# darshangm/dynamics-aware-diffusion

Measured on AMD Instinct MI355X. Metric: trajectory plans/sec (H=32, T=100), higher is better.
Workload: dtype f32; 1 GPU; PointMaze umaze-v2 guided policy, H=32 dim=128 mults(1,2,4) T=100 batch=256/GPU; arch=pointmaze, batch_per_gpu=256, global_batch=256, horizon=32, denoise_steps=100, rng=in-kernel philox, conv_arithmetic=fp32 (exact fp32 MFMA), hipgraph=False, loops_in_flight=1

## Files before the change

### dynamics_aware_diffusion_amd/_engine.py

```python
from __future__ import annotations

import ctypes as C
import math
import os
from typing import Dict, Mapping, Optional, Sequence

import torch

_HERE = os.path.dirname(os.path.abspath(__file__))
LIB_PATH = os.environ.get("DAD_LIB") or os.path.join(_HERE, "libdad_hip.so")

DAD_MAX_LEVELS = 8


class DadCfg(C.Structure):
    _fields_ = [
        ("transition_dim", C.c_int32), ("dim", C.c_int32), ("time_dim", C.c_int32),
        ("n_levels", C.c_int32), ("channels", C.c_int32 * DAD_MAX_LEVELS),
        ("kernel_size", C.c_int32), ("horizon", C.c_int32), ("n_timesteps", C.c_int32),
        ("predict_epsilon", C.c_int32), ("clip_denoised", C.c_int32),
    ]


class DadStepArgs(C.Structure):
    _fields_ = [
        ("noise", C.c_void_p), ("seed", C.c_uint64), ("row_offset", C.c_uint64),
        ("draw", C.c_uint64), ("cond0", C.c_void_p), ("cond_per_row", C.c_int32),
        ("guide_grad", C.c_void_p), ("guide_weight", C.c_float),
        ("mean_out", C.c_void_p), ("eps_out", C.c_void_p),
    ]


class DadProjectArgs(C.Structure):
    _fields_ = [
        ("P", C.c_void_p), ("obs_mean", C.c_void_p), ("obs_std", C.c_void_p),
        ("act_mean", C.c_void_p), ("act_std", C.c_void_p),
        ("state_dim", C.c_int32), ("observation_dim", C.c_int32), ("action_dim", C.c_int32),
        ("scratch", C.c_void_p), ("scratch_bytes", C.c_size_t),
    ]


ABI = {
    "dad_last_error": (C.c_char_p, []),
    "dad_version": (C.c_char_p, []),
    "dad_model_create": (C.c_int, [C.POINTER(DadCfg), C.POINTER(C.c_void_p)]),
    "dad_model_destroy": (None, [C.c_void_p]),
    "dad_model_load_weight": (C.c_int, [C.c_void_p, C.c_char_p, C.c_void_p,
                                        C.POINTER(C.c_int64), C.c_int32]),
    "dad_model_load_schedule": (C.c_int, [C.c_void_p] + [C.c_void_p] * 5),
    "dad_model_load_time_embedding": (C.c_int, [C.c_void_p, C.c_void_p, C.c_int32, C.c_int32]),
    "dad_model_set_precision": (C.c_int, [C.c_void_p, C.c_int32]),
    "dad_model_set_group_channels": (C.c_int, [C.c_void_p, C.POINTER(C.c_int32), C.c_int32]),
    "dad_model_set_horizon": (C.c_int, [C.c_void_p, C.c_int32]),
    "dad_model_finalize": (C.c_int, [C.c_void_p, C.c_void_p]),
    "dad_workspace_bytes": (C.c_int, [C.c_void_p, C.c_int32, C.POINTER(C.c_size_t)]),
    "dad_unet_forward": (C.c_int, [C.c_void_p, C.c_void_p, C.c_int32, C.c_void_p, C.c_int32,
                                   C.c_void_p, C.c_size_t, C.c_void_p]),
    "dad_unet_forward_rows": (C.c_int, [C.c_void_p, C.c_void_p, C.c_void_p, C.c_void_p, C.c_int32,
                                        C.c_void_p, C.c_size_t, C.c_void_p]),
    "dad_projection_violation": (C.c_int, [C.POINTER(DadProjectArgs), C.c_void_p, C.c_void_p, C.c_int32,
                                           C.c_int32, C.c_void_p]),
    "dad_denoise_step": (C.c_int, [C.c_void_p, C.c_void_p, C.c_int32, C.c_int32,
                                   C.POINTER(DadStepArgs), C.c_int32, C.c_void_p, C.c_size_t,
                                   C.c_void_p]),
    "dad_sample_loop": (C.c_int, [C.c_void_p, C.c_void_p, C.c_int32, C.c_int32, C.c_void_p,
                                  C.c_uint64, C.c_uint64, C.c_void_p, C.c_int32,
                                  C.POINTER(DadProjectArgs), C.c_void_p, C.c_int32, C.c_void_p,
                                  C.c_size_t, C.c_void_p]),
    "dad_project": (C.c_int, [C.POINTER(DadProjectArgs), C.c_float, C.c_void_p, C.c_int32,
                              C.c_int32, C.c_void_p]),
    "dad_fill_normal": (C.c_int, [C.c_void_p, C.c_int32, C.c_int32, C.c_uint64, C.c_uint64,
                                  C.c_uint64, C.c_void_p]),
    "dad_debug_set_tile": (C.c_int, [C.c_void_p, C.c_int32]),
    "dad_debug_set_option": (C.c_int, [C.c_void_p, C.c_char_p, C.c_int32]),
    "dad_debug_read_table": (C.c_int, [C.c_void_p, C.c_int32, C.c_int32, C.c_void_p, C.c_int32,
                                       C.POINTER(C.c_int32)]),
    "dad_debug_mish": (C.c_int, [C.c_void_p, C.c_void_p, C.c_int64, C.c_void_p]),
    "dad_debug_kernel_table_consistent": (C.c_int, []),
    "dad_debug_small_batch_plan": (C.c_int, [C.c_void_p, C.c_int32, C.POINTER(C.c_int32),
                                             C.POINTER(C.c_int32)]),
    "dad_debug_backward_plan": (C.c_int, [C.c_void_p, C.c_int32, C.POINTER(C.c_int32), C.c_int32,
                                          C.POINTER(C.c_int32)]),
    "dad_model_set_training": (C.c_int, [C.c_void_p, C.c_int32]),
    "dad_model_refresh_weights": (C.c_int, [C.c_void_p, C.c_int32, C.POINTER(C.c_char_p), C.POINTER(C.c_void_p),
                                            C.c_void_p]),
    "dad_train_grad_count": (C.c_int, [C.c_void_p, C.POINTER(C.c_int32), C.POINTER(C.c_int64)]),
    "dad_train_grad_info": (C.c_int, [C.c_void_p, C.c_int32, C.POINTER(C.c_char_p), C.POINTER(C.c_int64),
                                      C.POINTER(C.c_int64)]),
    "dad_train_workspace_bytes": (C.c_int, [C.c_void_p, C.c_int32, C.POINTER(C.c_size_t),
                                            C.POINTER(C.c_size_t)]),
    "dad_unet_forward_train": (C.c_int, [C.c_void_p, C.c_void_p, C.c_void_p, C.c_void_p, C.c_void_p,
                                         C.c_int32, C.c_void_p, C.c_size_t, C.c_void_p]),
    "dad_unet_backward": (C.c_int, [C.c_void_p, C.c_void_p, C.c_void_p, C.c_void_p, C.c_void_p,
                                    C.POINTER(C.c_void_p), C.c_int32,
                                    C.c_int32, C.c_void_p, C.c_size_t, C.c_void_p, C.c_size_t, C.c_void_p]),
    "dad_profile_enable": (C.c_int, [C.c_void_p, C.c_int32]),
    "dad_profile_read": (C.c_int, [C.c_void_p, C.POINTER(C.c_double), C.POINTER(C.c_int64),
                                   C.POINTER(C.c_double)]),
}

_lib = None


def load_library() -> C.CDLL:
    global _lib
    if _lib is not None:
        return _lib
    if not os.path.exists(LIB_PATH):
        raise RuntimeError(
            f"{LIB_PATH} not found: build it with dynamics_aware_diffusion_amd/csrc/build.sh "
            "(or __graft_entry__.build()).  There is no CPU fallback.")
    lib = C.CDLL(LIB_PATH)
    for name, (restype, argtypes) in ABI.items():
        if os.environ.get("DAD_LIB") and not hasattr(lib, name):
            continue
        fn = getattr(lib, name)
        fn.restype = restype
        fn.argtypes = argtypes
    _lib = lib
    return lib


class DadError(RuntimeError):
    def __init__(self, code: int, message: str):
        super().__init__(f"libdad_hip error {code}: {message}")
        self.code = code


def _check(lib, rc: int) -> None:
    if rc != 0:
        raise DadError(rc, lib.dad_last_error().decode("utf-8", "replace"))


def _ptr(t: Optional[torch.Tensor]) -> Optional[int]:
    return None if t is None else t.data_ptr()


def _require_device(t: torch.Tensor, name: str) -> None:
    if not t.is_cuda:
        raise RuntimeError(f"{name} must live on a ROCm device (got {t.device}); the HIP engine "
                           "has no CPU path")
    if t.dtype != torch.float32 or not t.is_contiguous():
        raise RuntimeError(f"{name} must be contiguous float32 (got {t.dtype}, "
                           f"contiguous={t.is_contiguous()})")


PRECISIONS = {"fp32": 0, "f16x3": 1}
TABLES = {"sinusoid": 0, "time_mlp": 1, "blocks": 2}


def sinusoid_table(n_timesteps: int, dim: int) -> torch.Tensor:
    half = dim // 2
    scale = math.log(10000) / (half - 1)
    freqs = torch.exp(torch.arange(half) * -scale)
    arg = torch.arange(n_timesteps)[:, None] * freqs[None, :]
    return torch.cat((arg.sin(), arg.cos()), dim=-1).contiguous()

SCHEDULE_KEYS = ("sqrt_recip_alphas_cumprod", "sqrt_recipm1_alphas_cumprod",
                 "posterior_mean_coef1", "posterior_mean_coef2",
                 "posterior_log_variance_clipped")


class HipEngine:

    def __init__(self, *, transition_dim: int, dim: int, channels: Sequence[int], horizon: int,
                 n_timesteps: int, time_dim: Optional[int] = None, kernel_size: int = 5,
                 predict_epsilon: bool = True, clip_denoised: bool = True,
                 device: torch.device | str = "cuda", precision: str = "fp32", training: bool = False):
        if precision not in PRECISIONS:
            raise ValueError(f"precision must be one of {sorted(PRECISIONS)}, got {precision!r}")
        self.precision = precision
        self.lib = load_library()
        self.device = torch.device(device)
        if self.device.type != "cuda":
            raise RuntimeError("HipEngine needs a ROCm device; there is no CPU path")
        from .utils import padding
        self.real_dim, self.real_channels = int(dim), [int(c) for c in channels]
        padded = [padding.padded_width(c) for c in self.real_channels]
        self.padded = padded != self.real_channels
        if self.padded:
            if self.real_channels[0] != self.real_dim:
                raise NotImplementedError("zero-padded widths need dim_mults[0] == 1")
            if transition_dim == self.real_dim:
                raise NotImplementedError(
                    f"transition_dim == dim == {dim} makes the first block's residual the trajectory itself; "
                    "with zero-padded GroupNorm groups that identity has no kernel")
        horizon = int(horizon)
        levels = len(self.real_channels)
        self.padded_horizon = max(1 << max(horizon - 1, 0).bit_length(), 4 << (levels - 1))
        self.rows_padded = self.padded_horizon != horizon
        if self.rows_padded:
            if horizon % (1 << (levels - 1)) != 0:
                raise ValueError(f"horizon {horizon} cannot be halved {levels - 1} times (the reference's U-Net needs "
                                 f"H % 2^(levels-1) == 0, temporal_unet.py:35-54)")
            if transition_dim == self.real_dim:
                raise NotImplementedError("transition_dim == dim with a zero-padded horizon has no kernel")
        self.padded = self.padded or self.rows_padded
        cfg = DadCfg()
        cfg.transition_dim = transition_dim
        cfg.dim = padded[0] if padded != self.real_channels else dim
        cfg.time_dim = time_dim or dim
        cfg.n_levels = len(channels)
        for i, ch in enumerate(padded):
            cfg.channels[i] = int(ch)
        cfg.kernel_size = kernel_size
        cfg.horizon = self.padded_horizon
        cfg.n_timesteps = n_timesteps
        cfg.predict_epsilon = int(predict_epsilon)
        cfg.clip_denoised = int(clip_denoised)
        self.cfg = cfg
        self.horizon = horizon
        self.transition_dim = transition_dim
        self.n_timesteps = n_timesteps
        handle = C.c_void_p()
        _check(self.lib, self.lib.dad_model_create(C.byref(cfg), C.byref(handle)))
        self._h = handle
        _check(self.lib, self.lib.dad_model_set_precision(self._h, PRECISIONS[precision]))
        self.widths_padded = padded != self.real_channels
        if self.widths_padded:
            real = (C.c_int32 * len(self.real_channels))(*self.real_channels)
            _check(self.lib, self.lib.dad_model_set_group_channels(self._h, real, len(self.real_channels)))
        if self.rows_padded:
            _check(self.lib, self.lib.dad_model_set_horizon(self._h, horizon))
        self.training = bool(training)
        if self.training:
            _check(self.lib, self.lib.dad_model_set_training(self._h, 1))
        self._ws: Dict[int, torch.Tensor] = {}
        self._pinned: Dict[tuple, torch.Tensor] = {}
        self.ready = False

    def __del__(self):
        h = getattr(self, "_h", None)
        if h:
# ... 138 lines not shown
            projection._check_x(x)
            pa = C.byref(projection.args)
            alphas = (C.c_float * self.n_timesteps)(*[float(a) for a in proj_alphas])
        ws = self.workspace(B)
        with torch.cuda.device(self.device):
            _check(self.lib, self.lib.dad_sample_loop(
                self._h, x.data_ptr(), int(n_steps), B, _ptr(noise_stack), int(seed),
                int(row_offset), cond_ptr, per_row, pa, alphas, int(use_graph), ws.data_ptr(),
                ws.numel() * 4, self._stream()))

    def fill_normal(self, x: torch.Tensor, seed: int, row_offset: int = 0, draw: int = 0) -> None:
        _require_device(x, "x")
        B = int(x.shape[0])
        with torch.cuda.device(self.device):
            _check(self.lib, self.lib.dad_fill_normal(
                x.data_ptr(), B, x.numel() // B, int(seed), int(row_offset), int(draw),
                self._stream()))

    def refresh(self, unet_state: Mapping[str, torch.Tensor]) -> None:
        keys, ptrs, keep = [], [], []
        if self.widths_padded:
            with torch.no_grad():
                names = list(unet_state.keys())
                fp = self.flat_padding(names, [tuple(unet_state[k].shape) for k in names])
                wide = fp.pad_flat([unet_state[k].detach().to(self.device) for k in names])
            base, n = wide.data_ptr(), len(names)
            with torch.cuda.device(self.device):
                _check(self.lib, self.lib.dad_model_refresh_weights(
                    self._h, n, (C.c_char_p * n)(*[k.encode() for k in names]),
                    (C.c_void_p * n)(*[base + 4 * o for o in fp.offsets]), self._stream()))
            self._refresh_keep = [wide]
            return
        for key, t in unet_state.items():
            d = t.detach()
            if d.device != self.device or d.dtype != torch.float32 or not d.is_contiguous():
                d = d.to(self.device, torch.float32).contiguous()
            keep.append(d)
            keys.append(key.encode())
            ptrs.append(d.data_ptr())
        n = len(keys)
        with torch.cuda.device(self.device):
            _check(self.lib, self.lib.dad_model_refresh_weights(
                self._h, n, (C.c_char_p * n)(*keys), (C.c_void_p * n)(*ptrs), self._stream()))
        self._refresh_keep = keep

    def flat_padding(self, keys, shapes, offsets=None, total=None):
        from .utils import padding
        cache = self.__dict__.setdefault("_flat_paddings", {})
        sig = (tuple(keys), None if offsets is None else tuple(offsets))
        if sig not in cache:
            cache[sig] = padding.FlatPadding(keys, shapes, self._pad_plan, offsets, total)
        return cache[sig]

    def time_projection_index(self) -> torch.Tensor:
        from .utils import padding
        cached = getattr(self, "_temb_index", None)
        if cached is None:
            n = len(self.real_channels)
            widths = [c for c in self.real_channels for _ in (0, 1)] + [self.real_channels[-1]] * 2
            for j in range(n - 1):
                widths += [self.real_channels[n - 2 - j]] * 2
            index, off = [], 0
            for c in widths:
                index.append(padding.channel_index(c) + off)
                off += padding.padded_width(c)
            cached = self._temb_index = (torch.cat(index).to(self.device), off)
        return cached

    def grad_layout(self):
        cached = getattr(self, "_grad_layout", None)
        if cached is not None:
            return cached
        n, total = C.c_int32(), C.c_int64()
        _check(self.lib, self.lib.dad_train_grad_count(self._h, C.byref(n), C.byref(total)))
        out = []
        for i in range(n.value):
            key, off, numel = C.c_char_p(), C.c_int64(), C.c_int64()
            _check(self.lib, self.lib.dad_train_grad_info(self._h, i, C.byref(key), C.byref(off), C.byref(numel)))
            out.append((key.value.decode(), off.value, numel.value))
        self._grad_layout = (out, total.value)
        return self._grad_layout

    def train_forward(self, x: torch.Tensor, temb_rows: torch.Tensor):
        B = self._traj(x)
        _require_device(temb_rows, "temb_rows")
        if temb_rows.dim() != 2 or temb_rows.shape[0] != B:
            raise RuntimeError(f"temb_rows must be (B, temb_width), got {tuple(temb_rows.shape)}")
        sv, sc = C.c_size_t(), C.c_size_t()
        _check(self.lib, self.lib.dad_train_workspace_bytes(self._h, B, C.byref(sv), C.byref(sc)))
        saved = torch.empty(max(sv.value, 4) // 4 + 4, dtype=torch.float32, device=self.device)
        rows = torch.arange(B, dtype=torch.int32, device=self.device)
        out = torch.empty_like(x)
        with torch.cuda.device(self.device):
            _check(self.lib, self.lib.dad_unet_forward_train(
                self._h, x.data_ptr(), rows.data_ptr(), temb_rows.data_ptr(), out.data_ptr(), B,
                saved.data_ptr(), saved.numel() * 4, self._stream()))
        return out, saved

    def train_backward(self, x: torch.Tensor, d_out: torch.Tensor, saved: torch.Tensor, temb_width: int, shapes):
        B = self._traj(x)
        if self._traj(d_out, "d_out") != B:
            raise RuntimeError("d_out batch mismatch")
        sv, sc = C.c_size_t(), C.c_size_t()
        _check(self.lib, self.lib.dad_train_workspace_bytes(self._h, B, C.byref(sv), C.byref(sc)))
        scratch = torch.empty(max(sc.value, 4) // 4 + 4, dtype=torch.float32, device=self.device)
        layout, total = self.grad_layout()
        if len(shapes) != len(layout):
            raise RuntimeError(f"{len(shapes)} parameter shapes for {len(layout)} gradient tensors")
        real = None
        if self.widths_padded:
            real = self.flat_padding([k for k, _, _ in layout], shapes, [o for _, o, _ in layout], total)
            shapes = real.padded_shapes
            for (key, _, numel), n in zip(layout, real.sizes):
                if n != numel:
                    raise RuntimeError(f"{key}: {n} padded elements, the library expects {numel}")
        flat = torch.empty(total, dtype=torch.float32, device=self.device)
        base = flat.data_ptr()
        spans = [layout[i + 1][1] - layout[i][1] for i in range(len(layout) - 1)] + [total - layout[-1][1]]
        pieces = flat.split_with_sizes(spans)
        grads = [(pc if pc.numel() == numel else pc[:numel]).view(tuple(shape))
                 for pc, (_, _, numel), shape in zip(pieces, layout, shapes)]
        ptrs = (C.c_void_p * len(grads))(*[base + 4 * offset for _, offset, _ in layout])
        d_x = torch.empty_like(x)
        d_temb = torch.empty(B, temb_width, dtype=torch.float32, device=self.device)
        with torch.cuda.device(self.device):
            _check(self.lib, self.lib.dad_unet_backward(
                self._h, x.data_ptr(), d_out.data_ptr(), d_x.data_ptr(), d_temb.data_ptr(), ptrs, len(grads), B,
                saved.data_ptr(), saved.numel() * 4, scratch.data_ptr(), scratch.numel() * 4, self._stream()))
        if real is not None:
            grads = real.gather(flat)
        return d_x, d_temb, grads

    def debug_set_tile(self, cfg: int) -> None:
        with torch.cuda.device(self.device):
            _check(self.lib, self.lib.dad_debug_set_tile(self._h, int(cfg)))

    def debug_set_option(self, name: str, value: int) -> None:
        with torch.cuda.device(self.device):
            _check(self.lib, self.lib.dad_debug_set_option(self._h, name.encode(), int(value)))

    def read_table(self, which: str, t: int) -> torch.Tensor:
        out = torch.empty(1 << 16, dtype=torch.float32)
        width = C.c_int32()
        with torch.cuda.device(self.device):
            _check(self.lib, self.lib.dad_debug_read_table(self._h, TABLES[which], int(t),
                                                           out.data_ptr(), out.numel(), C.byref(width)))
        return out[:width.value].clone()

    def small_batch_plan(self, batch: int):
        n, w = C.c_int32(), C.c_int32()
        _check(self.lib, self.lib.dad_debug_small_batch_plan(self._h, int(batch), C.byref(n), C.byref(w)))
        return n.value, w.value

    def backward_plan(self, batch: int) -> dict:
        need = C.c_int32()
        _check(self.lib, self.lib.dad_debug_backward_plan(self._h, int(batch), None, 0, C.byref(need)))
        buf = (C.c_int32 * need.value)()
        _check(self.lib, self.lib.dad_debug_backward_plan(self._h, int(batch), buf, need.value, C.byref(need)))
        r = list(buf)
        fields = ("taps", "tile", "windowed", "samples", "spc", "sps", "ksplit", "chunks", "last_chunks")
        assert r[71] == len(fields) and (len(r) - 72) == r[0] * r[71]
        hist = lambda at: {(cfg, bool(s)): r[at + 2 * cfg + s] for cfg in range(10) for s in (0, 1) if r[at + 2 * cfg + s]}
        return {
            "wgrads": r[0], "multi": r[1], "max_chunks": r[2], "max_ksplit": r[3], "part": r[4], "part_multi": r[5],
            "windowed": r[6], "tile": r[7:11],
            "taps_tile": {(taps, tile): r[11 + 4 * i + tile] for i, taps in enumerate((1, 3, 4, 5, 7)) for tile in range(4)
                          if r[11 + 4 * i + tile]},
            "fwd": hist(31), "dgrad": hist(51),
            "launches": [dict(zip(fields, r[at:at + len(fields)])) for at in range(72, len(r), len(fields))],
        }

    def mish(self, x: torch.Tensor) -> torch.Tensor:
        _require_device(x, "x")
        out = torch.empty_like(x)
        with torch.cuda.device(self.device):
            _check(self.lib, self.lib.dad_debug_mish(x.data_ptr(), out.data_ptr(), x.numel(),
                                                     self._stream()))
        return out

    def profile_enable(self, on: bool) -> None:
        _check(self.lib, self.lib.dad_profile_enable(self._h, int(on)))

    def profile_read(self):
        ms, n, fl = C.c_double(), C.c_int64(), C.c_double()
        _check(self.lib, self.lib.dad_profile_read(self._h, C.byref(ms), C.byref(n), C.byref(fl)))
        return ms.value, n.value, fl.value


class ProjectionState:

    def __init__(self, P: torch.Tensor, obs_mean, obs_std, act_mean, act_std, state_dim: int,
                 observation_dim: int, action_dim: int, device):
        dev = torch.device(device)
        if dev.type != "cuda":
            raise RuntimeError("projection kernel needs a ROCm device; there is no CPU path")

        def put(v):
            return torch.as_tensor(v, dtype=torch.float32).contiguous().to(dev)

        self.P = put(P)
        self.obs_mean, self.obs_std = put(obs_mean), put(obs_std)
        self.act_mean, self.act_std = put(act_mean), put(act_std)
        a = DadProjectArgs()
        a.P = self.P.data_ptr()
        a.obs_mean, a.obs_std = self.obs_mean.data_ptr(), self.obs_std.data_ptr()
        a.act_mean, a.act_std = self.act_mean.data_ptr(), self.act_std.data_ptr()
        a.state_dim, a.observation_dim, a.action_dim = state_dim, observation_dim, action_dim
        self.args = a
        self.device = dev
        self._scratch = None
        self.gemm = True
        self.D = int(self.P.shape[0])
        if self.P.dim() != 2 or self.P.shape[1] != self.D:
            raise ValueError(f"projection matrix must be square, got {tuple(self.P.shape)}")
        if self.obs_mean.numel() != observation_dim or self.obs_std.numel() != observation_dim \
                or self.act_mean.numel() != action_dim or self.act_std.numel() != action_dim:
            raise ValueError("normaliser statistics do not match observation_dim / action_dim")

    def _check_x(self, x: torch.Tensor) -> None:
        _require_device(x, "x")
        a = self.args
        if x.dim() != 3 or x.shape[2] != a.observation_dim + a.action_dim:
            raise RuntimeError(f"x must be (B, H, {a.observation_dim + a.action_dim}), got {tuple(x.shape)}")
        D = (int(x.shape[1]) + 1) * a.state_dim + int(x.shape[1]) * a.action_dim
        if D != self.D:
            raise RuntimeError(f"mat1 and mat2 shapes cannot be multiplied ({x.shape[0]}x{D} and "
                               f"{self.D}x{self.D}): the projector was built for another horizon")
        if x.device != self.P.device:
            raise RuntimeError(f"x is on {x.device}, the projector on {self.P.device}")
        if self.gemm and (self._scratch is None or self._scratch.numel() < x.numel()):
            self._scratch = torch.empty(x.numel(), dtype=torch.float32, device=self.device)
            self.args.scratch = self._scratch.data_ptr()
            self.args.scratch_bytes = self._scratch.numel() * 4

    def violation(self, x: torch.Tensor) -> torch.Tensor:
        self._check_x(x)
        out = torch.empty(int(x.shape[0]), dtype=torch.float32, device=x.device)
        lib = load_library()
        with torch.cuda.device(self.device):
            _check(lib, lib.dad_projection_violation(C.byref(self.args), x.data_ptr(), out.data_ptr(),
                                                     int(x.shape[0]), int(x.shape[1]),
                                                     torch.cuda.current_stream(self.device).cuda_stream))
        return out

    def apply(self, x: torch.Tensor, alpha: float) -> None:
        self._check_x(x)
        lib = load_library()
        with torch.cuda.device(self.device):
            _check(lib, lib.dad_project(C.byref(self.args), float(alpha), x.data_ptr(),
                                        int(x.shape[0]), int(x.shape[1]),
                                        torch.cuda.current_stream(self.device).cuda_stream))
```

### dynamics_aware_diffusion_amd/csrc/conv_gemm.hpp

```cpp
#pragma once
#include <hip/hip_runtime.h>
#include <stdint.h>

#include "conv_shapes.hpp"

namespace dad {

#define DAD_LBID (blockIdx.x + gridDim.x * (blockIdx.y + gridDim.y * blockIdx.z))
#ifdef DAD_STAMPS
#define DAD_STAMP(i) do { if (p.stamps != nullptr && threadIdx.x == 0 && DAD_LBID < 4096) p.stamps[DAD_LBID * 8 + (i)] = __builtin_amdgcn_s_memrealtime(); } while (0)
#else
#define DAD_STAMP(i) do {} while (0)
#endif
#ifdef DAD_STAMPS
#define DAD_CLOCK(i) do { if (p.stamps != nullptr && threadIdx.x == 0 && DAD_LBID < 4096) p.stamps[DAD_LBID * 8 + (i)] = __builtin_amdgcn_s_memtime(); } while (0)
#else
#define DAD_CLOCK(i) do {} while (0)
#endif
#ifdef DAD_STAMPS_PROLOGUE
#define DAD_PSTAMP(i) do { if (p.stamps != nullptr && threadIdx.x == 0 && DAD_LBID < 4096) p.stamps[DAD_LBID * 8 + (i)] = __builtin_amdgcn_s_memrealtime(); } while (0)
#undef DAD_STAMP
#define DAD_STAMP(i) do { if ((i) == 0) DAD_PSTAMP(0); } while (0)
#undef DAD_CLOCK
#define DAD_CLOCK(i) do {} while (0)
#else
#define DAD_PSTAMP(i) do {} while (0)
#endif

typedef float f32x16 __attribute__((ext_vector_type(16)));
typedef _Float16 f16x8 __attribute__((ext_vector_type(8)));

__device__ __forceinline__ void split_f16(float v, _Float16& hi, _Float16& lo) {
    const float c = __builtin_fminf(__builtin_fmaxf(v, -65504.0f), 65504.0f);
    hi = (_Float16)c;
    lo = (_Float16)((c - (float)hi) * 2048.0f);
}
__device__ __forceinline__ void split_f16x4(const float4 v, float2& hi, float2& lo) {
    typedef _Float16 f16x4 __attribute__((ext_vector_type(4)));
    f16x4 h, l;
    _Float16 a, b;
    split_f16(v.x, a, b); h[0] = a; l[0] = b;
    split_f16(v.y, a, b); h[1] = a; l[1] = b;
    split_f16(v.z, a, b); h[2] = a; l[2] = b;
    split_f16(v.w, a, b); h[3] = a; l[3] = b;
    hi = __builtin_bit_cast(float2, h);
    lo = __builtin_bit_cast(float2, l);
}

struct ConvParams {
    const float* src0;
    const float* src1;
    const float* w;
    const float* bias;
    const float* gamma;
    const float* beta;
    const float* temb;
    const int32_t* trow;
    int32_t temb_stride;
    const float* res;
    float* dst;
    int32_t cin0, cin1;
    int32_t cin_pad;
    int32_t M;
    int32_t cpg;
    int32_t lreal;
    int32_t src_len;
    int32_t cpg_real;
    int32_t B;
    int32_t Lin, Lout;
    int32_t lshift;
    int32_t lshift_in;
    int32_t interleave;
    int32_t ntiles_n;
    int32_t xcd_gn;
    int32_t xcd_mts;
    int32_t xcd_ntn;
    int32_t kslices;
    int32_t chunks_per_slice;
    float c1, c2;
    uint64_t xswz;
    int32_t wtaps;
    const float* rbias;
    float* rdst;
    float* pre;
    float* stats;
    float* slab;
    unsigned* counters;
#ifdef DAD_STAMPS
    unsigned long long* stamps;
#endif
};

__device__ __forceinline__ float mish_f32(float y) {
    if (y > 20.0f) return y;
    const float n = expf(y);
    const float w = n * (n + 2.0f);
    return y * (w / (w + 2.0f));
}

__device__ __forceinline__ float mish_fast_f32(float y) {
    if (y > 20.0f) return y;
    const float L2E_HI = 1.44269502162933349609375f;
    const float L2E_LO = 1.92596299112661746e-08f;
    const float t = y * L2E_HI;
    const float tl = fmaf(y, L2E_HI, -t) + y * L2E_LO;
    const float n = __builtin_amdgcn_exp2f(t) * (1.0f + 0.693147180559945f * tl);
    const float w = n * (n + 2.0f);
    return y * (w * __builtin_amdgcn_rcpf(w + 2.0f));
}

template <int CTRL>
__device__ __forceinline__ float dpp_f32(float v) {
    return __builtin_bit_cast(float, __builtin_amdgcn_update_dpp(0, __builtin_bit_cast(int, v), CTRL,
                                                                 0xF, 0xF, true));
}
__device__ __forceinline__ float rows_sum(float v, int width, int lane) {
    const int iv = __builtin_bit_cast(int, v);
    const float r0 = __builtin_bit_cast(float, __builtin_amdgcn_readlane(iv, 0));
    const float r1 = __builtin_bit_cast(float, __builtin_amdgcn_readlane(iv, 16));
    const float r2 = __builtin_bit_cast(float, __builtin_amdgcn_readlane(iv, 32));
    const float r3 = __builtin_bit_cast(float, __builtin_amdgcn_readlane(iv, 48));
    const float lo = r0 + r1, hi = r2 + r3;
    if (width >= 64) return lo + hi;
    return lane < 32 ? lo : hi;
}

__device__ __forceinline__ float4 ldg4(const float* p) {
    typedef float __attribute__((ext_vector_type(4))) f4;
    const f4 v = *reinterpret_cast<const __attribute__((address_space(1))) f4*>(
        (const __attribute__((address_space(1))) float*)p);
    return make_float4(v.x, v.y, v.z, v.w);
}

__device__ __forceinline__ void store_f4_sc1(float* p, const float4 v) {
    typedef float __attribute__((ext_vector_type(4))) f4;
    const f4 x = {v.x, v.y, v.z, v.w};
    asm volatile("global_store_dwordx4 %0, %1, off sc1" ::"v"(p), "v"(x) : "memory");
}

template <int BM, int BN, int SK, int KC, int TAPS, int STRIDE, bool RAGGED, bool X3 = false, bool BDIR = false,
          bool RES = false, bool PADDED = false, bool WIN = false>
__global__ __launch_bounds__(64 * (BM / 32) * (BN / 32) * SK) void conv_gemm_f32(const ConvParams p) {
    constexpr int TMW = BM / 32;
    constexpr int TNW = BN / 32;
    constexpr int WT = TMW * TNW;
    constexpr int NT = 64 * WT * SK;
    constexpr int PAD = TAPS / 2;
    constexpr int WTAPS = TAPS + (RES ? 1 : 0);
    constexpr int KP = KC + 4;
    constexpr int KU = X3 ? 16 : 8;
    constexpr int G = KC / KU;
    constexpr int GW = G / SK;
    constexpr int KG = KC < 16 ? KC : 16;
    constexpr int NSUB = KC / KG;
    static_assert(KC % KU == 0 && G % SK == 0 && GW >= 1, "K chunk must split evenly over the SK waves");
    static_assert(!BDIR || (BN == 32 && SK == 1 && !RAGGED && KC >= 16), "direct-B tiles");
    static_assert(!RES || (!X3 && !BDIR && (TAPS & 1) == 1 && TAPS >= 3 && STRIDE == 1), "the residual ride exists for fp32 stride-1 convs of the net's kernel size");
    static_assert(!WIN || (PADDED && !X3 && !BDIR && !RES), "windowed tiles: fp32, LDS-staged, no ride");
    constexpr int BN_SH = BN == 32 ? 5 : BN == 64 ? 6 : 7;
    static_assert((1 << BN_SH) == BN, "BN is 32, 64 or 128");

    extern __shared__ __attribute__((aligned(16))) float smem[];
    float4* const smem4 = reinterpret_cast<float4*>(smem);
    float2* const smem2 = reinterpret_cast<float2*>(smem);
#ifdef DAD_ABLATE_NULL
    if (p.B > 0) return;
#endif

    DAD_STAMP(0);
    const int tid = threadIdx.x;
    const int lane = tid & 63;
    const int wave = __builtin_amdgcn_readfirstlane(tid >> 6);
    const int wt = wave % WT;
    const int ks = wave / WT;
    const int tn = wt / TMW;
    const int tm = wt % TMW;
    const int l32 = lane & 31;
    const int h = lane >> 5;

    const int kb = blockIdx.x;
    int mt = blockIdx.y;
    int nt = blockIdx.z;
    if (p.xcd_gn > 0) {
        const int wg = blockIdx.y, c = wg & 7, j = wg >> 3;
        const int im = c / p.xcd_gn, in = c - im * p.xcd_gn;
        mt = (im << p.xcd_mts) + (j & ((1 << p.xcd_mts) - 1));
        nt = in * p.xcd_ntn + (j >> p.xcd_mts);
    }
    const int tile = mt * p.ntiles_n + nt;

    const int Lin = p.Lin, Lout = p.Lout;
    const int SPT = WIN ? 1 : BN >> p.lshift;
    const int SEG = WIN ? BN * STRIDE + 2 * PAD : Lin + 2 * PAD;
    const int XROWS = SPT * SEG;
    const int wsh = WIN ? p.lshift - BN_SH : 0;
    const int s0 = WIN ? nt >> wsh : nt * SPT;
    const int w0 = WIN ? (nt & ((1 << wsh) - 1)) << BN_SH : 0;
    const int m0 = mt * BM;
    const int M = p.M;
    const int nvalid = min(SPT, p.B - s0);

    const int XF = XROWS * KP + kXSwzPad;
    const int STAGE = XF + (BDIR ? 0 : WTAPS * BM * KP);
    const int STAGE4 = STAGE >> 2;


    const int n_loc = tn * 32 + l32;
    const int phase_shift = (TAPS == 2 && p.interleave && m0 >= (p.M >> 1)) ? 1 : 0;
    const int arow = WIN ? (n_loc * STRIDE + phase_shift) * KP + 4 * h
                         : ((n_loc >> p.lshift) * SEG + (n_loc & (Lout - 1)) * STRIDE + phase_shift) * KP + 4 * h +
                               (int)((p.xswz >> (4 * (n_loc >> p.lshift))) & 15) * 4;
    const int brow = XF + (tm * 32 + l32) * KP + 4 * h;

    f32x16 acc, acc2, acc3, acc4;
    f32x16 accr, accr2;
#pragma unroll
    for (int r = 0; r < 16; ++r) { acc[r] = 0.0f; acc2[r] = 0.0f; acc3[r] = 0.0f; acc4[r] = 0.0f; accr[r] = 0.0f; accr2[r] = 0.0f; }

    const int cin = p.cin0 + p.cin1;
    const int c_begin = kb * p.chunks_per_slice;
#ifdef DAD_ABLATE_NOLOOP
    const int nchunks = c_begin + 1;
#else
    const int nchunks = min((p.cin0 + p.cin1 + KC - 1) / KC, c_begin + p.chunks_per_slice);
#endif

    constexpr int W_F4 = WTAPS * BM * KC / 4;
    constexpr int W_PER_T = BDIR ? 0 : (W_F4 + NT - 1) / NT;
    constexpr int W_ARR = W_PER_T ? W_PER_T : 1;
    constexpr int KQ = KC / 4;
    constexpr int X_F4_MAX = (BN * STRIDE + (WIN ? 2 * PAD : 0)) * KQ;
    constexpr int X_PER_T = (X_F4_MAX + NT - 1) / NT;
    const int xrows_real = WIN ? SEG : SPT * Lin;
    float4 wreg[W_ARR];
    float4 xreg[X_PER_T];
    int w_goff[W_ARR], w_loff[W_ARR];
    int x_grow[X_PER_T], x_q4[X_PER_T], x_loff[X_PER_T];
    constexpr int GQ = KG / 4;
#pragma unroll
    for (int i = 0; i < W_PER_T; ++i) {
        const int e = tid + i * NT;
        const int row = e / KQ;
        const int q = e - row * KQ;
        const int tap = row / BM;
        const int mm = row - tap * BM;
        const int sub = q / GQ;
        w_goff[i] = ((sub * p.wtaps + tap) * M + m0 + mm) * KG + (q - sub * GQ) * 4;
        w_loff[i] = (XF + row * KP + q * 4) >> 2;
    }
#pragma unroll
    for (int i = 0; i < X_PER_T; ++i) {
        const int e = tid + i * NT;
        const int row = e / KQ;
        const int q = e - row * KQ;
        const int s = WIN ? 0 : row >> p.lshift_in;
        int l = row - (s << p.lshift_in);
        if constexpr (WIN) l = w0 * STRIDE - PAD + row;
        const bool ok = e < xrows_real * KQ && s < nvalid && (!WIN || (l >= 0 && l < Lin));
        x_grow[i] = ok ? (WIN ? s0 * Lin + l : s0 * Lin + row) : -1;
        if constexpr (PADDED)
            if (p.src_len > 0)
                x_grow[i] = (ok && l < p.src_len) ? (s0 + s) * p.src_len + l : -1;
        x_q4[i] = q * 4;
        const int qoff = X3 ? (q >> 2) * 16 + (q & 3) * 2 : q * 4;
        const int xo = WIN ? row * KP + qoff : (s * SEG + PAD + l) * KP + qoff + (int)((p.xswz >> (4 * s)) & 15) * 4;
        x_loff[i] = e < xrows_real * KQ ? (X3 ? xo >> 1 : xo >> 2) : -1;
    }
    DAD_PSTAMP(6);
    const long w_chunk_stride = (long)NSUB * p.wtaps * M * KG;
    constexpr int NLD = W_PER_T + X_PER_T;
    auto item_store = [&](int k, int stage) {
        const int base4 = stage * STAGE4;
        if (k < W_PER_T) {
            if (W_F4 % NT == 0 || tid + k * NT < W_F4)
                smem4[base4 + w_loff[k]] = wreg[k];
        } else {
            const int i = k - W_PER_T;
            if (x_loff[i] >= 0) {
                float4 v = xreg[i];
                if (!RAGGED && x_grow[i] < 0) v = make_float4(0.f, 0.f, 0.f, 0.f);
                if constexpr (X3) {
                    float2 hi, lo;
                    split_f16x4(v, hi, lo);
                    smem2[base4 * 2 + x_loff[i]] = hi;
                    smem2[base4 * 2 + x_loff[i] + 4] = lo;
                } else {
                    smem4[base4 + x_loff[i]] = v;
                }
            }
        }
    };
    auto item_load = [&](int k, int chunk) {
        if (k < W_PER_T) {
            float4 v = make_float4(0.f, 0.f, 0.f, 0.f);
            if (W_F4 % NT == 0 || tid + k * NT < W_F4)
                v = *reinterpret_cast<const float4*>(p.w + chunk * w_chunk_stride + w_goff[k]);
            wreg[k] = v;
        } else {
            const int i = k - W_PER_T;
            const int c0 = chunk * KC;
            float4 v = make_float4(0.f, 0.f, 0.f, 0.f);
            if constexpr (!RAGGED) {
                const bool second = c0 >= p.cin0;
                const float* xsrc = second ? p.src1 : p.src0;
                const int cs = second ? p.cin1 : p.cin0;
                const int cb = second ? c0 - p.cin0 : c0;
                v = *reinterpret_cast<const float4*>(xsrc + (long)max(x_grow[i], 0) * cs + cb + x_q4[i]);
            } else {
                const int cc = c0 + x_q4[i];
                if (x_grow[i] >= 0 && cc < cin) {
                    const bool second = cc >= p.cin0;
                    const int cs = second ? p.cin1 : p.cin0;
                    const int cl = second ? cc - p.cin0 : cc;
                    const float* g = (second ? p.src1 : p.src0) + (long)x_grow[i] * cs + cl;
                    const int left = cs - cl;
                    if ((cs & 3) == 0) {
                        v = *reinterpret_cast<const float4*>(g);
                    } else {
                        if (left > 0) v.x = g[0];
                        if (left > 1) v.y = g[1];
                        if (left > 2) v.z = g[2];
                        if (left > 3) v.w = g[3];
                    }
                }
            }
            xreg[i] = v;
        }
    };

    constexpr int UW = WTAPS * GW;
    const int koff = ks * (GW * KU);
    const int afrag4 = (arow + koff) >> 2;
    const int bfrag4 = (brow + koff) >> 2;
    auto frag_a = [&](int stage, int u, int lo) -> float4 {
        const int wtap = u / GW, gw = u - wtap * GW;
        const int tap = (RES && wtap == TAPS) ? PAD : wtap;
        return smem4[stage * STAGE4 + afrag4 + tap * (KP / 4) + gw * (KU / 4) + lo / 4];
    };
    auto frag_b = [&](int stage, int u, int lo) -> float4 {
        const int tap = u / GW, gw = u - tap * GW;
        return smem4[stage * STAGE4 + bfrag4 + tap * (BM * KP / 4) + gw * (KU / 4) + lo / 4];
    };
    constexpr int BPU = X3 ? 2 : 1;
    float4 breg[BDIR ? BPU * UW : 1];
    const float* bsrc = p.w + ((long)(m0 + tm * 32 + l32) * 16 + 4 * h);
    auto bload = [&](int u, int chunk) {
        const int tap = u / GW, gw = u - tap * GW;
        if constexpr (X3) {
            const float* q = bsrc + (long)chunk * w_chunk_stride + (long)((gw * p.wtaps + tap) * M) * 16;
            breg[2 * u] = ldg4(q);
            breg[2 * u + 1] = ldg4(q + 8);
        } else {
            const float* q = bsrc + (long)chunk * w_chunk_stride +
                             (long)(((gw >> 1) * p.wtaps + tap) * M) * 16 + (gw & 1) * 8;
            breg[u] = ldg4(q);
        }
    };

#pragma unroll
    for (int k = 0; k < NLD; ++k) item_load(k, c_begin);
    if constexpr (BDIR) {
#pragma unroll
        for (int u = 0; u < UW; ++u) bload(u, c_begin);
    }

    constexpr int ES = BM + 4;
    constexpr int ECOPY = BN * ES;
    constexpr int F4PL = (BN * BM / 4) / NT;
    static_assert(F4PL >= 1 && (BN * BM / 4) % NT == 0, "epilogue mapping");
#ifdef DAD_ABLATE_GN
    const bool has_gn = false;
#else
    const bool has_gn = !WIN && p.gamma != nullptr;
#endif
    const int cpg = has_gn ? p.cpg : BM;
    const int cq = cpg >> 2;
    const int cnt4 = has_gn ? (Lout * cq) : (BN * cq);
    static_assert((F4PL & (F4PL - 1)) == 0, "F4PL is a power of two");
    const int lpp = cnt4 >> (F4PL == 1 ? 0 : F4PL == 2 ? 1 : F4PL == 4 ? 2 : 3);
    const int lpp_sh = 31 - __clz(lpp);
    const int cq_sh = 31 - __clz(cq);
    const int gpt_sh = 31 - __clz(BM) - (31 - __clz(cpg));
    const int pr = tid >> lpp_sh;
    const int lp = tid & (lpp - 1);
    const int ps = has_gn ? pr >> gpt_sh : 0;
    const int pg = has_gn ? pr & ((1 << gpt_sh) - 1) : 0;
    int erow[F4PL], ecol[F4PL];
    int eoff[F4PL];
    float4 bias4[F4PL], gam4[F4PL], bet4[F4PL], temb4[F4PL], res4[F4PL];
#pragma unroll
    for (int k = 0; k < F4PL; ++k) {
        const int j = lp + k * lpp;
        const int r = j >> cq_sh;
        erow[k] = ps * Lout + r;
        ecol[k] = pg * cpg + (j & (cq - 1)) * 4;
        const int s = erow[k] >> p.lshift;
        const int l = w0 + (erow[k] & (Lout - 1));
        const int em = m0 + ecol[k];
        if (!p.interleave) {
            eoff[k] = ((s0 + s) * Lout + l) * M + em;
        } else {
            const int half = M >> 1;
            const int phase = em >= half;
            eoff[k] = ((s0 + s) * (2 * Lout) + 2 * l + phase) * half + (em - phase * half);
        }
        if (s >= nvalid) eoff[k] = -1;
    }
    constexpr bool EARLY_PARAMS = F4PL <= 2;
#define DAD_FETCH_PARAMS()                                                                       \
    _Pragma("unroll") for (int k = 0; k < F4PL; ++k) {                                           \
        const int em = m0 + ecol[k];                                                             \
        long toff = 0;                                                                           \
        if (p.trow != nullptr)            \
            toff = (long)p.trow[min(s0 + (erow[k] >> p.lshift), p.B - 1)] * p.temb_stride;       \
        bias4[k] = ldg4(p.bias + em);                                                            \
        gam4[k] = ldg4(gptr + em);                                                               \
        bet4[k] = ldg4(bptr + em);                                                               \
        temb4[k] = ldg4(tptr + toff + em);                                                       \
        res4[k] = ldg4(has_res ? p.res + max(eoff[k], 0) : p.bias + em);                         \
    }
    const float* const gptr = has_gn ? p.gamma : p.bias;
    const float* const bptr = has_gn ? p.beta : p.bias;
    const float* const tptr = p.temb != nullptr ? p.temb : p.bias;
    const bool has_res = p.res != nullptr && !p.interleave;
    const bool has_temb = p.temb != nullptr;
    DAD_PSTAMP(7);
    if (EARLY_PARAMS) { DAD_FETCH_PARAMS() }
    DAD_PSTAMP(1);
    if constexpr (PAD > 0 && !WIN) {
        constexpr int KP4 = KP / 4;
        const int nz = SPT * (2 * PAD) * KP4;
        for (int i = tid; i < nz; i += NT) {
            const int hr = i / KP4, c4 = i - hr * KP4;
            const int s = hr / (2 * PAD), j = hr - s * (2 * PAD);
            const int row = s * SEG + (j < PAD ? j : Lin + j);
            const int at = row * KP + c4 * 4 + (int)((p.xswz >> (4 * s)) & 15) * 4;
            smem4[at >> 2] = make_float4(0.f, 0.f, 0.f, 0.f);
            smem4[STAGE4 + (at >> 2)] = make_float4(0.f, 0.f, 0.f, 0.f);
        }
    }
    DAD_PSTAMP(2);
#pragma unroll
    for (int k = 0; k < NLD; ++k) item_store(k, 0);
    DAD_PSTAMP(3);
    if (c_begin + 1 < nchunks) {
#pragma unroll
        for (int k = 0; k < NLD; ++k) item_load(k, c_begin + 1);
    }
    DAD_PSTAMP(4);
    __syncthreads();
    DAD_PSTAMP(5);

    float4 ah = frag_a(0, 0, 0), bh = ah;
    if constexpr (!BDIR) bh = frag_b(0, 0, 0);
    float4 al = ah, bl = bh;
    if constexpr (X3) {
        al = frag_a(0, 0, 8);
        if constexpr (!BDIR) bl = frag_b(0, 0, 8);
    }
    DAD_STAMP(1);
    DAD_CLOCK(6);
#ifndef DAD_ABLATE_STAGE
#define DAD_ROLL(STORE, LOAD)                                                                    \
    _Pragma("unroll") for (int k = 0; k < NLD; ++k) {                                            \
        if ((BDIR ? UW - 1 : (k * UW) / NLD) != u) continue;       \
        if (STORE) item_store(k, cur ^ 1);                                                       \
        if (LOAD) item_load(k, ch + 2);                                                          \
    }
#else
#define DAD_ROLL(STORE, LOAD)
#endif
#ifndef DAD_ABLATE_BARRIER
#define DAD_SYNC() __syncthreads();
#else
#define DAD_SYNC()
#endif
#ifndef DAD_ABLATE_LDSREAD
#define DAD_READ(ST, U)                                                                          \
    nah = frag_a(ST, U, 0);                                                                      \
    if constexpr (X3) nal = frag_a(ST, U, 8);                                                    \
    if constexpr (!BDIR) {                                                                       \
        nbh = frag_b(ST, U, 0);                                                                  \
        if constexpr (X3) nbl = frag_b(ST, U, 8);                                                \
    }
#else
#define DAD_READ(ST, U)
#endif
#ifndef DAD_ABLATE_MFMA
#define DAD_MFMA()                                                                               \
    if constexpr (BDIR && X3) { bh = breg[2 * u]; bl = breg[2 * u + 1]; }                        \
    if constexpr (BDIR && !X3) bh = breg[u];                                                     \
    if constexpr (X3) {                                                                          \
        acc = __builtin_amdgcn_mfma_f32_32x32x16_f16(__builtin_bit_cast(f16x8, ah),              \
                                                     __builtin_bit_cast(f16x8, bh), acc, 0, 0, 0);  \
        acc2 = __builtin_amdgcn_mfma_f32_32x32x16_f16(__builtin_bit_cast(f16x8, ah),             \
                                                      __builtin_bit_cast(f16x8, bl), acc2, 0, 0, 0); \
        acc3 = __builtin_amdgcn_mfma_f32_32x32x16_f16(__builtin_bit_cast(f16x8, al),             \
                                                      __builtin_bit_cast(f16x8, bh), acc3, 0, 0, 0); \
    } else if (RES && u / GW == TAPS) {                                                          \
        accr = __builtin_amdgcn_mfma_f32_32x32x2f32(ah.x, bh.x, accr, 0, 0, 0);                  \
        accr2 = __builtin_amdgcn_mfma_f32_32x32x2f32(ah.y, bh.y, accr2, 0, 0, 0);                \
        accr = __builtin_amdgcn_mfma_f32_32x32x2f32(ah.z, bh.z, accr, 0, 0, 0);                  \
        accr2 = __builtin_amdgcn_mfma_f32_32x32x2f32(ah.w, bh.w, accr2, 0, 0, 0);                \
    } else {                                                                                     \
        acc = __builtin_amdgcn_mfma_f32_32x32x2f32(ah.x, bh.x, acc, 0, 0, 0);                    \
        acc2 = __builtin_amdgcn_mfma_f32_32x32x2f32(ah.y, bh.y, acc2, 0, 0, 0);                  \
        acc3 = __builtin_amdgcn_mfma_f32_32x32x2f32(ah.z, bh.z, acc3, 0, 0, 0);                  \
        acc4 = __builtin_amdgcn_mfma_f32_32x32x2f32(ah.w, bh.w, acc4, 0, 0, 0);                  \
    }
#else
#define DAD_MFMA() acc[0] += ah.x * bh.x + al.y * bl.y;
#endif
#define DAD_CHUNK(STORE, LOAD)                                                                   \
    {                                                                                            \
        const int cur = (ch - c_begin) & 1;                                                      \
        _Pragma("unroll") for (int u = 0; u < UW; ++u) {                                         \
            float4 nah = ah, nal = al, nbh = bh, nbl = bl;                                       \
            DAD_ROLL(STORE, LOAD)                                                                \
            if (u + 1 < UW) {                                                                    \
                DAD_READ(cur, u + 1)                                                             \
            } else {                                                                             \
                DAD_SYNC()                                                                       \
                if (STORE) { DAD_READ(cur ^ 1, 0) }                                              \
            }                                                                                    \
            __builtin_amdgcn_sched_barrier(0);                                                   \
            DAD_MFMA()                                                                           \
            __builtin_amdgcn_sched_barrier(0);                                                   \
            if constexpr (BDIR) { if (STORE) bload(u, ch + 1); }                                 \
            ah = nah; al = nal; bh = nbh; bl = nbl;                                              \
        }                                                                                        \
    }
    int ch = c_begin;
    for (; ch + 2 < nchunks; ++ch) DAD_CHUNK(true, true)
    if (ch + 1 < nchunks) { DAD_CHUNK(true, false) ++ch; }
    if (ch < nchunks) DAD_CHUNK(false, false)
#undef DAD_CHUNK
#undef DAD_ROLL
#undef DAD_SYNC
#undef DAD_READ
#undef DAD_MFMA
#pragma unroll
    for (int r = 0; r < 16; ++r) {
        if constexpr (X3) acc[r] = acc[r] * p.c1 + (acc2[r] + acc3[r]) * p.c2;
        else acc[r] = (acc[r] + acc2[r]) + (acc3[r] + acc4[r]);
    }
    __syncthreads();
    DAD_STAMP(2);
    DAD_CLOCK(7);

    float* E = smem;
    float* red = smem + SK * ECOPY;
#ifdef DAD_ABLATE_NOEPI
    if (p.B > 0) { if (acc[0] == 123.456f) p.dst[0] = acc[1]; return; }
#endif
#pragma unroll
    for (int r = 0; r < 16; ++r) {
        const int row = tn * 32 + (r & 3) + 8 * (r >> 2) + 4 * h;
        const int col = tm * 32 + l32;
        E[ks * ECOPY + row * ES + col] = acc[r];
    }
    __syncthreads();
    DAD_STAMP(3);
    if (!EARLY_PARAMS) { DAD_FETCH_PARAMS() }
#undef DAD_FETCH_PARAMS

    float y[F4PL][4];
#pragma unroll
    for (int k = 0; k < F4PL; ++k) {
        const float* q = E + erow[k] * ES + ecol[k];
        float4 v = *reinterpret_cast<const float4*>(q);
#pragma unroll
        for (int c = 1; c < SK; ++c) {
            const float4 u = *reinterpret_cast<const float4*>(q + c * ECOPY);
            v.x += u.x; v.y += u.y; v.z += u.z; v.w += u.w;
        }
        y[k][0] = v.x; y[k][1] = v.y; y[k][2] = v.z; y[k][3] = v.w;
    }

    if constexpr (RES) {
        __syncthreads();
#pragma unroll
        for (int r = 0; r < 16; ++r) {
            const int row = tn * 32 + (r & 3) + 8 * (r >> 2) + 4 * h;
            const int col = tm * 32 + l32;
            E[ks * ECOPY + row * ES + col] = accr[r] + accr2[r];
        }
        __syncthreads();
#pragma unroll
        for (int k = 0; k < F4PL; ++k) {
            const float* q = E + erow[k] * ES + ecol[k];
            float4 v = *reinterpret_cast<const float4*>(q);
#pragma unroll
            for (int c = 1; c < SK; ++c) {
                const float4 u = *reinterpret_cast<const float4*>(q + c * ECOPY);
                v.x += u.x; v.y += u.y; v.z += u.z; v.w += u.w;
            }
            const float4 rb = ldg4(p.rbias + m0 + ecol[k]);
            if (eoff[k] >= 0)
                store_f4_sc1(p.rdst + eoff[k], make_float4(v.x + rb.x, v.y + rb.y, v.z + rb.z, v.w + rb.w));
        }
    }

    if (p.kslices > 1) {
        const int KS = p.kslices;
        float* mine = p.slab + ((long)tile * KS + kb) * (BN * BM);
#pragma unroll
        for (int k = 0; k < F4PL; ++k)
            if (eoff[k] >= 0)
                store_f4_sc1(mine + erow[k] * BM + ecol[k], make_float4(y[k][0], y[k][1], y[k][2], y[k][3]));
        asm volatile("s_waitcnt vmcnt(0)" ::: "memory");
        __syncthreads();
        unsigned* flag = reinterpret_cast<unsigned*>(smem + SK * ECOPY + 32);
        if (tid == 0) {
            const unsigned ticket = __hip_atomic_fetch_add(p.counters + tile, 1u, __ATOMIC_RELAXED,
                                                           __HIP_MEMORY_SCOPE_AGENT);
            const unsigned last = ticket == (unsigned)(KS - 1);
            if (last) {
                __builtin_amdgcn_fence(__ATOMIC_ACQUIRE, "agent");
                asm volatile("s_waitcnt vmcnt(0)" ::: "memory");
// ... 118 lines not shown
```

### dynamics_aware_diffusion_amd/csrc/dad_lib.hip

```cpp
#include <hip/hip_runtime.h>

#include <algorithm>
#include <cmath>
#include <cstdarg>
#include <cstdio>
#include <cstring>
#include <cstdlib>
#include <functional>
#include <map>
#include <memory>
#include <string>
#include <vector>

#include <mutex>
#include <set>
#include <tuple>
#include <utility>

#include "../../include/dad.h"
#include "host_plan.hpp"
#include "conv_gemm.hpp"
#include "conv_gn_pass.hpp"
#include "pointwise.hpp"
#include "conv_cc.hpp"
#include "conv_ccw.hpp"
#include "train_bwd.hpp"

using namespace dadhost;

namespace {

#ifdef DAD_STAMPS
unsigned long long* g_stamps = nullptr;
#endif

#define HIP_TRY(expr)                                                                   \
    do {                                                                                \
        hipError_t e_ = (expr);                                                         \
        if (e_ != hipSuccess)                                                           \
            return fail(DAD_E_HIP, "%s failed: %s (%s:%d)", #expr, hipGetErrorString(e_), \
                        __FILE__, __LINE__);                                            \
    } while (0)

struct GraphKey {
    const void* x; const void* noise; const void* cond; const void* ws;
    const void* P; const void* obs_mean; const void* obs_std; const void* act_mean; const void* act_std;
    const void* proj_scratch;
    int n_steps, batch, cond_per_row, state_dim, observation_dim, action_dim;
    int force_tile, flags;
    uint64_t row_offset;
    uint64_t alpha_hash;
    bool operator<(const GraphKey& o) const {
        return std::memcmp(this, &o, sizeof(GraphKey)) < 0;
    }
};

}

struct dad_model : HostModel {
    bool finalized = false;
    int device = -1;
    std::vector<float> sched[5];
    bool have_sched = false;
    std::vector<float> emb_override;
    float* d_emb = nullptr;
    float* d_temb = nullptr;
    float* d_temb_table = nullptr;
    float* d_final_w = nullptr;
    float* d_final_b = nullptr;
    uint64_t* d_rng = nullptr;
    unsigned* d_counters = nullptr;
    float* d_zero = nullptr;
    std::map<std::string, float*> d_time;
    std::vector<WeightEntry> weights;
    float* d_h1 = nullptr;
    std::vector<void*> owned;
    void* d_repack = nullptr;
    size_t repack_cap = 0;
    std::vector<char> repack_host;
    bool tables_stale = false;
    char* arena = nullptr;
    size_t arena_cap = 0, arena_used = 0;
    bool profile = false;
    std::vector<std::pair<hipEvent_t, hipEvent_t>> ev_pool;
    size_t ev_used = 0;
    double prof_flops = 0;
    int64_t prof_launches = 0;
    std::map<GraphKey, hipGraphExec_t> graphs;
    hipStream_t cap_stream = nullptr;
};

namespace {

using dad::ConvParams;

int arena_alloc(dad_model* m, size_t bytes, void** out) {
    const size_t aligned = (bytes + 255) / 256 * 256;
    if (m->arena_used + aligned > m->arena_cap)
        return fail(DAD_E_STATE, "parameter arena exhausted (%zu + %zu > %zu)", m->arena_used, aligned,
                    m->arena_cap);
    *out = m->arena + m->arena_used;
    m->arena_used += aligned;
    return DAD_OK;
}

int upload(dad_model* m, const std::vector<float>& host, float** dev) {
    void* p = nullptr;
    const int rc = arena_alloc(m, std::max<size_t>(host.size(), 1) * sizeof(float), &p);
    if (rc != DAD_OK) return rc;
    HIP_TRY(hipMemcpy(p, host.data(), host.size() * sizeof(float), hipMemcpyHostToDevice));
    *dev = (float*)p;
    return DAD_OK;
}

float*& weight_ptr(dad_model* m, const WeightEntry& e) {
    switch (e.to) {
        case WT_W: return m->plan.convs[e.conv].d_w;
        case WT_BIAS: return m->plan.convs[e.conv].d_bias;
        case WT_RBIAS: return m->plan.convs[e.conv].d_rbias;
        case WT_GAMMA: return m->plan.convs[e.conv].d_gamma;
        case WT_BETA: return m->plan.convs[e.conv].d_beta;
        case WT_BWD_W: return m->bconvs[e.conv].op[e.sub].d_w;
        case WT_BFINAL_W: return m->bfinal.d_w;
        case WT_FINAL_W: return m->d_final_w;
        case WT_FINAL_B: return m->d_final_b;
        case WT_TIME: break;
    }
    return m->d_time[e.key];
}

void free_device(dad_model* m) {
    for (auto& kv : m->graphs) (void)hipGraphExecDestroy(kv.second);
    m->graphs.clear();
    for (void* p : m->owned) (void)hipFree(p);
    m->owned.clear();
    m->d_repack = nullptr; m->repack_cap = 0; m->repack_host.clear(); m->tables_stale = false;
    m->arena = nullptr;
    m->arena_cap = m->arena_used = 0;
    m->d_emb = m->d_temb = m->d_temb_table = nullptr;
    m->d_final_w = m->d_final_b = nullptr;
    m->d_rng = nullptr;
    m->d_counters = nullptr;
    m->d_zero = nullptr;
    m->weights.clear(); m->d_time.clear();
    for (Plan* plan : {&m->plan, &m->tplan})
        for (auto& op : plan->convs) op.d_w = op.d_bias = op.d_gamma = op.d_beta = op.d_rbias = nullptr;
    for (auto& b : m->bconvs) for (int k = 0; k < b.n; ++k) b.op[k].d_w = b.op[k].d_bias = nullptr;
    m->bfinal.d_w = m->bfinal.d_bias = nullptr;
}

using KernFn = void (*)(const ConvParams);
using KernKey = std::tuple<int, int, int, bool, bool, bool, bool, bool, bool>;
using KernTable = std::map<KernKey, KernFn>;

template <int CFG, int TAPS, int STRIDE, int F>
void reg_kernel(KernTable& t) {
    if constexpr (kernel_registered_f(CFG, TAPS, STRIDE, F)) {
        constexpr TileCfg T = kTiles[CFG];
        constexpr bool X3 = F & 1, BDIR = F & 2, RAGGED = F & 4, RES = F & 8, PADDED = F & 16, WIN = F & 32;
        t[KernKey(CFG, TAPS, STRIDE, X3, BDIR, RAGGED, RES, PADDED, WIN)] =
            dad::conv_gemm_f32<T.BM, T.BN, T.SK, tile_kc(CFG, TAPS, X3, BDIR), TAPS, STRIDE, RAGGED, X3, BDIR, RES, PADDED, WIN>;
    }
}
template <int CFG, int TAPS, size_t... F>
void reg_flags(KernTable& t, std::index_sequence<F...>) {
    (reg_kernel<CFG, TAPS, 1, (int)F>(t), ...);
    (reg_kernel<CFG, TAPS, 2, (int)F>(t), ...);
}
template <int CFG, size_t... TAPS>
void reg_taps(KernTable& t, std::index_sequence<TAPS...>) {
    (reg_flags<CFG, (int)TAPS + 1>(t, std::make_index_sequence<(1 << kRegFlags)>()), ...);
}
template <size_t... CFG>
void reg_tiles(KernTable& t, std::index_sequence<CFG...>) {
    (reg_taps<(int)CFG>(t, std::make_index_sequence<kRegMaxTaps>()), ...);
}
const KernTable& kernel_table() {
    static const KernTable table = [] {
        KernTable t;
        reg_tiles(t, std::make_index_sequence<kNumTiles>());
        return t;
    }();
    return table;
}

struct FamilyKernel { int key[5]; const void* fn; };
using FamilyList = std::vector<FamilyKernel>;
const void* find_kernel(const FamilyList& list, int k0, int k1, int k2, int k3 = 0, int k4 = 0) {
    for (const FamilyKernel& k : list)
        if (k.key[0] == k0 && k.key[1] == k1 && k.key[2] == k2 && k.key[3] == k3 && k.key[4] == k4) return k.fn;
    return nullptr;
}

template <bool BIG, int NR>
void add_cc(FamilyList& v) {
    v.push_back({{5, 0, BIG, NR, 0}, (const void*)dad::conv_cc<5, 1, false, BIG, NR>});
    v.push_back({{5, 1, BIG, NR, 0}, (const void*)dad::conv_cc<5, 1, true, BIG, NR>});
    v.push_back({{3, 0, BIG, NR, 0}, (const void*)dad::conv_cc<3, 2, false, BIG, NR>});
    v.push_back({{2, 0, BIG, NR, 0}, (const void*)dad::conv_cc<2, 1, false, BIG, NR>});
}
const FamilyList& cc_kernels() {
    static const FamilyList list = [] {
        FamilyList v;
        add_cc<false, 16>(v); add_cc<false, 32>(v); add_cc<true, 16>(v); add_cc<true, 32>(v);
        v.push_back({{5, 0, 0, 32, 1}, (const void*)dad::conv_cc<5, 1, false, false, 32, 6, true>});
        v.push_back({{5, 1, 0, 32, 1}, (const void*)dad::conv_cc<5, 1, true, false, 32, 6, true>});
        return v;
    }();
    return list;
}
const void* cc_kernel(int taps, bool ride, bool big, int rows, bool windowed) {
    return find_kernel(cc_kernels(), taps, ride, big, rows, windowed);
}

template <bool RIDE, int NR>
void add_ccw(FamilyList& v) {
    v.push_back({{5, 0, RIDE, NR}, (const void*)dad::conv_ccw<5, 1, false, RIDE, NR>});
    v.push_back({{5, 1, RIDE, NR}, (const void*)dad::conv_ccw<5, 1, true, RIDE, NR>});
    v.push_back({{3, 0, RIDE, NR}, (const void*)dad::conv_ccw<3, 2, false, RIDE, NR>});
    v.push_back({{2, 0, RIDE, NR}, (const void*)dad::conv_ccw<2, 1, false, RIDE, NR>});
    v.push_back({{1, 0, RIDE, NR}, (const void*)dad::conv_ccw<1, 1, false, RIDE, NR>});
}
const FamilyList& ccw_kernels() {
    static const FamilyList list = [] {
        FamilyList v;
        add_ccw<false, 16>(v); add_ccw<false, 32>(v); add_ccw<true, 16>(v); add_ccw<true, 32>(v);
        return v;
    }();
    return list;
}
const void* ccw_kernel(int taps, bool res, bool ride_in, int rows) {
    return find_kernel(ccw_kernels(), taps, res, ride_in, rows);
}

template <int TAPS, bool WIN>
void add_wgrad(FamilyList& v) {
    v.push_back({{TAPS, 0, WIN}, (const void*)dad::conv_wgrad<TAPS, 2, 2, true, WIN>});
    v.push_back({{TAPS, 1, WIN}, (const void*)dad::conv_wgrad<TAPS, 2, 1, true, WIN>});
    v.push_back({{TAPS, 2, WIN}, (const void*)dad::conv_wgrad<TAPS, 1, 1, true, WIN>});
    v.push_back({{TAPS, 3, WIN}, (const void*)dad::conv_wgrad<TAPS, 1, 1, false, WIN>});
}
template <size_t... I>
void add_wgrad_taps(FamilyList& v, std::index_sequence<I...>) {
    ((add_wgrad<kWgradTaps[I], false>(v), add_wgrad<kWgradTaps[I], true>(v)), ...);
}
const FamilyList& wgrad_kernels() {
    static const FamilyList list = [] {
        FamilyList v;
        add_wgrad_taps(v, std::make_index_sequence<std::size(kWgradTaps)>());
        return v;
    }();
    return list;
}
const void* wgrad_kernel(int taps, int tile, bool win) { return find_kernel(wgrad_kernels(), taps, tile, win); }

int configure_kernels() {
    static std::mutex lock;
    static std::set<int> done;
    int dev = -1;
    HIP_TRY(hipGetDevice(&dev));
    std::lock_guard<std::mutex> hold(lock);
    if (done.count(dev)) return DAD_OK;
    std::vector<const void*> fns = {(const void*)dad::final_posterior_kernel, (const void*)dad::final_cc_kernel,
                                    (const void*)dad::project_kernel<4, 16>, (const void*)dad::project_kernel<1, 16>};
    for (const auto& kv : kernel_table()) fns.push_back((const void*)kv.second);
    for (const FamilyList* list : {&cc_kernels(), &ccw_kernels(), &wgrad_kernels()})
        for (const FamilyKernel& k : *list) fns.push_back(k.fn);
    for (const void* fn : fns)
        HIP_TRY(hipFuncSetAttribute(fn, hipFuncAttributeMaxDynamicSharedMemorySize, (int)dad::kLdsBytes));
    done.insert(dev);
    return DAD_OK;
}

struct ConvIO {
    const float* src0 = nullptr; const float* src1 = nullptr;
    float* dst = nullptr; const float* res = nullptr; float* rdst = nullptr;
    const float* temb = nullptr; const int32_t* trow = nullptr;
    float* pre = nullptr; float* stats = nullptr;
    float* slab = nullptr;
};
int launch_conv(dad_model* m, const ConvOp& op, const LaunchGeom& g, int batch, const ConvIO& io, hipStream_t st);

int run_conv(dad_model* m, const FwdPlan& f, const FwdLaunch& l, const float* xext, float* ws, int t, hipStream_t st,
             const int32_t* trow, const float* temb_rows) {
    const Plan& plan = f.train ? m->tplan : m->plan;
    const ConvOp& op = plan.convs[l.conv];
    const int batch = f.batch;
    auto buf = [&](int id) -> float* {
        return id >= 0 ? ws + plan.bufs[id].offset * (long)batch : nullptr;
    };
    if (op.cat0 >= 0) {
        const long rows = (long)batch * op.Lout;
        const long n4 = rows * ((op.cat_c0 + op.cat_c1) / 4);
        hipLaunchKernelGGL(dad::concat_rows_kernel, dim3((unsigned)((n4 + 255) / 256)), dim3(256), 0, st,
                           buf(op.res), buf(op.cat0), buf(op.cat1), rows, op.cat_c0, op.cat_c1);
        HIP_TRY(hipGetLastError());
    }
    ConvIO io;
    io.src0 = op.src0 == -2 ? xext : buf(op.src0);
    io.src1 = buf(op.src1);
    if (op.temb_off >= 0)
        io.temb = temb_rows != nullptr ? temb_rows + op.temb_off
                                       : m->d_temb_table + (trow ? 0L : (long)t * m->plan.temb_width) + op.temb_off;
    io.trow = io.temb != nullptr ? trow : nullptr;
    io.res = op.res == -2 ? xext : buf(op.res);
    io.dst = buf(op.dst);
    io.rdst = buf(op.rdst);
    io.pre = buf(op.pre); io.stats = buf(op.stats);
    io.slab = ws + plan.floats_per_sample * (long)batch;
    return launch_conv(m, op, l.g, batch, io, st);
}

int launch_gn_pass(dad_model* m, const ConvOp& op, int npt, int batch, const ConvIO& io, hipStream_t st) {
    dad::GnPassParams q{};
    q.src = io.pre != nullptr ? io.pre : io.dst;
    q.dst = io.dst;
    q.gamma = op.d_gamma; q.beta = op.d_beta;
    q.temb = io.temb; q.trow = io.trow; q.temb_stride = m->plan.temb_width;
    q.res = io.res; q.stats = io.stats;
    q.C = op.cout; q.L = op.Lout; q.cpg = op.cout / 8; q.lreal = op.lreal; q.cpg_real = op.gn_real;
    const dim3 grid(8, (unsigned)batch), block(dad::GNP_THREADS);
    static_assert(dad::kGnPassMaxNpt == 32, "one case per power of two up to kGnPassMaxNpt");
    switch (npt) {
        case 1: hipLaunchKernelGGL(dad::gn_pass_kernel<1>, grid, block, 0, st, q); break;
        case 2: hipLaunchKernelGGL(dad::gn_pass_kernel<2>, grid, block, 0, st, q); break;
        case 4: hipLaunchKernelGGL(dad::gn_pass_kernel<4>, grid, block, 0, st, q); break;
        case 8: hipLaunchKernelGGL(dad::gn_pass_kernel<8>, grid, block, 0, st, q); break;
        case 16: hipLaunchKernelGGL(dad::gn_pass_kernel<16>, grid, block, 0, st, q); break;
        default: hipLaunchKernelGGL(dad::gn_pass_kernel<32>, grid, block, 0, st, q);
    }
    HIP_TRY(hipGetLastError());
    return DAD_OK;
}

int launch_conv(dad_model* m, const ConvOp& op, const LaunchGeom& g, int batch, const ConvIO& io, hipStream_t st) {
    const bool gn_pass = g.gn_npt > 0;
    ConvParams p{};
    p.src0 = io.src0;
    p.src1 = io.src1;
    p.w = op.d_w; p.bias = op.d_bias; p.gamma = op.d_gamma; p.beta = op.d_beta;
    p.temb = io.temb;
    p.trow = io.trow; p.temb_stride = m->plan.temb_width;
    p.res = io.res;
    p.dst = io.dst;
    p.pre = io.pre; p.stats = io.stats;
    if (gn_pass) {
        p.gamma = p.beta = p.temb = p.res = nullptr;
        p.trow = nullptr;
        p.pre = nullptr; p.stats = nullptr;
        if (io.pre != nullptr) p.dst = io.pre;
    }
    p.cin0 = op.cin0; p.cin1 = op.cin1; p.cin_pad = op.cin_pad;
    p.M = op.M; p.cpg = op.norm.empty() ? 0 : op.cout / 8; p.cpg_real = op.gn_real;
    p.lreal = op.lreal; p.src_len = op.src_len;
    p.B = batch; p.Lin = op.Lin; p.Lout = op.Lout; p.lshift = ilog2(op.Lout);
    p.lshift_in = ilog2(op.Lin);
    p.interleave = op.kind == CONV_UP;
    p.ntiles_n = g.ntiles_n;
    p.xcd_gn = g.xcd_gn; p.xcd_mts = g.xcd_mts; p.xcd_ntn = g.xcd_ntn;
    p.kslices = g.split.kslices;
    p.chunks_per_slice = g.split.chunks_per_slice;
    p.slab = io.slab;
    p.counters = m->d_counters;
    p.c1 = op.c1; p.c2 = op.c2;
    p.xswz = g.xswz;
    p.wtaps = op.wtaps();
    p.rbias = g.fused ? op.d_rbias : nullptr;
    p.rdst = g.fused ? io.rdst : nullptr;
    if (g.split.kslices > 1 && io.slab == nullptr)
        return fail(DAD_E_WORKSPACE, "%s: split-K launch without scratch", op.name.c_str());
    static const bool trace = getenv("DAD_TRACE_TILES") != nullptr;
    if (trace)
        fprintf(stderr, "[dad] %-34s B=%d M=%d K=%dx%d L=%d tile=%d (%dx%d SK%d) kslices=%d%s\n", op.name.c_str(),
                batch, op.M, op.taps, op.cin0 + op.cin1, op.Lout, g.cfg, kTiles[g.cfg].BM, kTiles[g.cfg].BN,
                kTiles[g.cfg].SK, g.split.kslices, g.fused ? " +res1x1" : "");
#ifdef DAD_STAMPS
    p.stamps = (g_stamps && &op >= &m->plan.convs[0] && &op < &m->plan.convs[0] + m->plan.convs.size())
                   ? g_stamps + (size_t)(&op - &m->plan.convs[0]) * 4096 * 8 : nullptr;
#endif
    const auto& table = kernel_table();
    const auto it = table.find(KernKey(g.cfg, op.taps, op.stride, op.x3, op.bdir, g.ragged, g.fused, g.padded, g.windowed));
    if (it == table.end())
        return fail(DAD_E_INVALID, "no kernel for %s (tile %d taps=%d stride=%d x3=%d bdir=%d ragged=%d res=%d)",
                    op.name.c_str(), g.cfg, op.taps, op.stride, (int)op.x3, (int)op.bdir, (int)g.ragged, (int)g.fused);
    void* args[] = {&p};
    HIP_TRY(hipLaunchKernel((const void*)it->second, dim3(g.gx, g.gy, g.gz), dim3(g.threads), args,
                            g.lds_bytes, st));
    if (gn_pass) return launch_gn_pass(m, op, g.gn_npt, batch, io, st);
    return DAD_OK;
}

int build_time_tables(dad_model* m, hipStream_t st);
int ensure_tables(dad_model* m, hipStream_t st) {
    if (!m->tables_stale) return DAD_OK;
    const int rc = build_time_tables(m, st);
    if (rc == DAD_OK) m->tables_stale = false;
    return rc;
}

int check_ready(const dad_model* m, int batch, int t, size_t ws_bytes, bool small_ok, FwdPlan& f) {
    if (!m) return fail(DAD_E_INVALID, "null model");
    if (!m->finalized) return fail(DAD_E_STATE, "dad_model_finalize has not been called");
    if (batch <= 0) return fail(DAD_E_INVALID, "batch must be positive (got %d)", batch);
    if (t < 0 || t >= m->cfg.n_timesteps)
        return fail(DAD_E_RANGE, "index %d is out of bounds for the schedule of size %d", t,
                    m->cfg.n_timesteps);
    const int rc = plan_forward(*m, false, batch, small_ok, f);
    if (ws_bytes < f.bytes)
        return fail(DAD_E_WORKSPACE, "workspace has %zu bytes, batch %d needs %zu", ws_bytes, batch,
                    f.bytes);
    return rc;
}

dad::CcSrc cc_source(dad_model* m, const CcPlan& cc, const CcInput& in, int channels, const float* xext,
                     float* ws, int batch, int t) {
    dad::CcSrc s{};
    auto buf = [&](int id) -> float* { return ws + m->plan.bufs[id].offset * (long)batch; };
    float* slabs = ws + m->plan.floats_per_sample * (long)batch;
    s.C = channels;
    if (in.kind == 1) { s.data = xext; s.rows = batch * m->cfg.horizon; return s; }
    if (in.kind == 2) { s.data = buf(in.buf); return s; }
    const ConvOp& q = m->plan.convs[in.producer];
    const CcOp& qo = cc.ops[in.producer];
    s.data = slabs + qo.oslab;
    s.nsl = qo.kslices;
    s.C = qo.out_cols;
    s.rows = qo.out_rows;
    s.bias = q.d_bias;
    if (!q.norm.empty()) { s.gamma = q.d_gamma; s.beta = q.d_beta; s.cpg = q.cout / 8; }
    if (q.temb_off >= 0) s.temb = m->d_temb_table + (long)t * m->plan.temb_width + q.temb_off;
    if (qo.res_kind == 1) s.res = xext;
    else if (qo.res_kind == 2) s.res = buf(qo.res_buf);
    else if (qo.res_kind == 3) {
        const CcOp& r = cc.ops[qo.res_ride];
        s.rslab = slabs + r.orslab; s.nrs = r.kslices; s.rbias = m->plan.convs[qo.res_ride].d_rbias;
    } else if (qo.res_kind == 4) {
        const CcOp& r = cc.ops[qo.res_ride];
        s.rslab = slabs + r.oslab; s.nrs = r.kslices; s.rbias = m->plan.convs[qo.res_ride].d_bias;
    }
    s.mat = buf(in.buf);
    return s;
}

int run_conv_cc(dad_model* m, const CcPlan& cc, int i, const float* xext, float* ws, int batch, int t,
                hipStream_t st) {
    const ConvOp& op = m->plan.convs[i];
    const CcOp& o = cc.ops[i];
    dad::CcParams p{};
    p.src0 = cc_source(m, cc, o.in0, op.cin0, xext, ws, batch, t);
    if (o.in1.kind != 0) p.src1 = cc_source(m, cc, o.in1, op.cin1, xext, ws, batch, t);
    p.w = op.d_w; p.wtaps = op.wtaps();
    p.cin0 = op.cin0; p.cin1 = op.cin1; p.M = op.M;
    p.B = batch; p.Lin = op.Lin; p.Lout = op.Lout;
    p.lshift = ilog2(op.Lout); p.lshift_in = ilog2(op.Lin);
    p.interleave = op.kind == CONV_UP;
    p.slice_ch = o.slice_ch;
    float* slabs = ws + m->plan.floats_per_sample * (long)batch;
    p.oslab = slabs + o.oslab;
    p.orslab = o.orslab >= 0 ? slabs + o.orslab : nullptr;
    p.out_rows = o.out_rows;
    const void* kern = o.wide ? ccw_kernel(op.taps, op.ride, o.ride_in, o.tile_rows)
                              : cc_kernel(op.taps, op.ride, o.big, o.tile_rows, op.Lout > 32);
    if (!kern) return fail(DAD_E_INVALID, "no small-batch kernel for %s (taps=%d stride=%d)", op.name.c_str(), op.taps, op.stride);
    static const bool trace = getenv("DAD_TRACE_TILES") != nullptr;
    if (trace)
        fprintf(stderr, "[dad] %-34s B=%d M=%d K=%dx%d L=%d cc slice=%d kslices=%d ntiles=%d%s\n", op.name.c_str(), batch,
                op.M, op.taps, op.cin0 + op.cin1, op.Lout, o.slice_ch, o.kslices, o.ntiles, op.ride ? " +res1x1" : "");
    if (trace && o.wide) fprintf(stderr, "[dad]   (wide: %d-row tiles, %zu B LDS)\n", o.tile_rows, o.lds_bytes);
#ifdef DAD_STAMPS
    p.stamps = g_stamps ? g_stamps + (size_t)i * 16 : nullptr;
#endif
    void* args[] = {&p};
    HIP_TRY(hipLaunchKernel(kern, dim3(o.kslices, op.M / 32, o.ntiles), dim3(dad::CC_THREADS), args, o.lds_bytes, st));
    return DAD_OK;
}

int run_unet(dad_model* m, const FwdPlan& f, const float* x, int t, float* ws, hipStream_t st,
             const int32_t* trow = nullptr, const float* temb_rows = nullptr) {
    hipEvent_t e0 = nullptr, e1 = nullptr;
    if (m->profile) {
        if (m->ev_used == m->ev_pool.size()) {
            hipEvent_t a, b;
            HIP_TRY(hipEventCreate(&a));
            HIP_TRY(hipEventCreate(&b));
            m->ev_pool.push_back({a, b});
        }
        e0 = m->ev_pool[m->ev_used].first;
        e1 = m->ev_pool[m->ev_used].second;
        ++m->ev_used;
        HIP_TRY(hipEventRecord(e0, st));
    }
    for (size_t i = 0; f.cc.ok && i < f.cc.ops.size(); ++i) {
        if (!f.cc.ops[i].launched) continue;
        const int rc = run_conv_cc(m, f.cc, (int)i, x, ws, f.batch, t, st);
        if (rc != DAD_OK) return rc;
    }
    for (const FwdLaunch& l : f.launches) {
        const int rc = run_conv(m, f, l, x, ws, t, st, trow, temb_rows);
        if (rc != DAD_OK) return rc;
    }
    if (m->profile) {
        for (const ConvOp& op : m->plan.convs) m->prof_flops += op.flops_per_sample * f.batch;
        for (const CcOp& o : f.cc.ops) m->prof_launches += o.launched;
        m->prof_launches += (int64_t)f.launches.size();
        HIP_TRY(hipEventRecord(e1, st));
    }
    return DAD_OK;
}

int run_final(dad_model* m, const FwdPlan& f, float* x, const float* x_ro, int t, const dad_step_args* a,
              int x_out_disabled, float* eps_only, float* ws, hipStream_t st, bool seed_from_device = false) {
    const dad_cfg& c = m->cfg;
    const int batch = f.batch;
    dad::FinalParams p{};
    const Plan& plan = f.train ? m->tplan : m->plan;
    p.act = ws + plan.bufs[plan.final_act].offset * (long)batch;
    p.w = m->d_final_w; p.bias = m->d_final_b;
    p.dim = c.dim; p.td = c.transition_dim; p.B = batch; p.H = traj_horizon(*m); p.Hact = c.horizon;
    p.predict_epsilon = c.predict_epsilon; p.clip_denoised = c.clip_denoised;
    if (eps_only) {
        p.x = const_cast<float*>(x_ro);
        p.eps_out = eps_only;
        p.x_out_disabled = 1;
    } else {
        p.x = x;
        p.noise = a->noise; p.cond0 = a->cond0; p.cond_per_row = a->cond_per_row;
        p.guide = (a->guide_grad && a->guide_weight > 0.0f) ? a->guide_grad : nullptr;
        p.mean_out = a->mean_out; p.eps_out = a->eps_out;
        p.x_out_disabled = x_out_disabled;
        const float lv = m->sched[4][t];
        p.c_recip = m->sched[0][t]; p.c_recipm1 = m->sched[1][t];
        p.coef1 = m->sched[2][t]; p.coef2 = m->sched[3][t];
        p.sigma = t == 0 ? 0.0f : expf(0.5f * lv);
        p.guide_scale = a->guide_weight * expf(lv);
        p.seed = a->seed;
        p.elem_offset = a->row_offset * (uint64_t)traj_horizon(*m) * (uint64_t)c.transition_dim;
        p.draw = a->draw;
// ... 589 lines not shown
                      int32_t batch, void* saved_v, size_t saved_bytes, void* scratch_v, size_t scratch_bytes,
                      dad_stream_t stream) {
    int rc = check_train(m, batch);
    if (rc != DAD_OK) return rc;
    if (!x || !d_out || !d_temb_rows || !grad_tensors || !saved_v || !scratch_v) return fail(DAD_E_INVALID, "null pointer");
    if (n_grad_tensors != (int32_t)m->grad_slots.size())
        return fail(DAD_E_INVALID, "%d gradient tensors passed, the model has %zu (dad_train_grad_count)", n_grad_tensors,
                    m->grad_slots.size());
    for (int32_t i = 0; i < n_grad_tensors; ++i)
        if (!grad_tensors[i]) return fail(DAD_E_INVALID, "gradient tensor %d ('%s') is null", i, m->grad_slots[i].key.c_str());
    const int B = batch;
    FwdPlan fwd;
    plan_forward(*m, true, B, false, fwd);
    TrainScratch ts;
    const int geom_rc = train_scratch(*m, B, ts);
    if (saved_bytes < fwd.bytes || scratch_bytes < (size_t)ts.total * sizeof(float))
        return fail(DAD_E_WORKSPACE, "backward workspaces too small (saved %zu / %zu, scratch %zu / %zu bytes)", saved_bytes,
                    fwd.bytes, scratch_bytes, (size_t)ts.total * sizeof(float));
    if (m->bwd_rc != DAD_OK) return fail(m->bwd_rc, "%s", m->bwd_err.c_str());
    if (geom_rc != DAD_OK) return geom_rc;
    if (d_x != nullptr && !m->bdx) return fail(DAD_E_STATE, "backward: no gradient reached the trajectory");

    hipStream_t st = (hipStream_t)stream;
    const Plan& P = m->tplan;
    const int H = m->cfg.horizon, td = m->cfg.transition_dim, tdp = round_up(td, 32);
    float* const saved = (float*)saved_v;
    float* const mirror = (float*)scratch_v;
    float* const part = mirror + ts.mirror;
    float* const wslab = part + ts.part;
    float* const dxpad = wslab + ts.wslab;
    float* const tmp = dxpad + ts.dxpad;
    float* const bslab = tmp + ts.tmp;
    const int Hr = traj_horizon(*m);
    if (Hr != H) {
        float* const xpad = dxpad + (long)B * H * tdp;
        float* const dopad = xpad + (long)B * H * round_up(td, 4);
        const long n = (long)B * H * td;
        hipLaunchKernelGGL(dad::pad_rows_kernel, dim3((unsigned)((n + 255) / 256)), dim3(256), 0, st, xpad, x, (long)B, H, Hr, td);
        hipLaunchKernelGGL(dad::pad_rows_kernel, dim3((unsigned)((n + 255) / 256)), dim3(256), 0, st, dopad, d_out, (long)B, H, Hr, td);
        HIP_TRY(hipGetLastError());
        x = xpad; d_out = dopad;
    }
    auto ptr = [&](const BwdRef& r) -> float* {
        switch (r.sp) {
            case BSP_ACT: return saved + P.bufs[r.buf].offset * (long)B;
            case BSP_GRAD: return mirror + P.bufs[r.buf].offset * (long)B;
            case BSP_X: return const_cast<float*>(x);
            case BSP_DOUT: return const_cast<float*>(d_out);
            case BSP_DX: return dxpad;
            default: return nullptr;
        }
    };

    size_t nw = 0, nd = 0;
    for (const BwdStep& s : m->bsteps) {
        switch (s.kind) {
            case BK_BIAS:
                hipLaunchKernelGGL(dad::row_partial_sums_kernel, dim3(B), dim3(256), 0, st, part + s.part * B, ptr(s.in),
                                   s.rows, s.C, s.C);
                HIP_TRY(hipGetLastError());
                break;
            case BK_WGRAD:
                if ((rc = launch_wgrad(m, s, ts.wgrads[nw++], ptr(s.in), ptr(s.z0), ptr(s.z1), grad_tensors[s.slot], wslab, st)) != DAD_OK)
                    return rc;
                break;
            case BK_DGRAD: {
                ConvIO io;
                io.src0 = ptr(s.in); io.slab = bslab;
                io.dst = s.write == BW_STAGE ? tmp : ptr(s.out);
                io.res = s.write == BW_ADD ? io.dst : nullptr;
                if ((rc = launch_conv(m, bwd_op(*m, s), ts.dgrads[nd++].g, B, io, st)) != DAD_OK) return rc;
                if (s.write == BW_STAGE && (rc = accumulate(ptr(s.out), tmp, s.n * B, BW_ADD, st)) != DAD_OK) return rc;
                break;
            }
            case BK_GN: {
                const ConvOp& f = P.convs[s.conv];
                const long c4 = round_up(f.cout, 4);
                dad::GnBwdParams gp{};
                gp.dA = ptr(s.in); gp.h = saved + P.bufs[f.pre].offset * (long)B; gp.stats = saved + P.bufs[f.stats].offset * (long)B;
                gp.gamma = f.d_gamma; gp.beta = f.d_beta;
                gp.dH = ptr(s.out);
                gp.part_dgamma = part + s.part * B; gp.part_dbeta = gp.part_dgamma + c4 * B; gp.part_dbias = gp.part_dbeta + c4 * B;
                gp.dtemb = f.temb_off >= 0 ? d_temb_rows + f.temb_off : nullptr;
                gp.temb_stride = P.temb_width;
                gp.C = f.cout; gp.L = f.Lout; gp.cpg = f.cout / 8; gp.lreal = f.lreal; gp.cpg_real = f.gn_real;
                gp.B = B;
                const dim3 wgrid((unsigned)((B * 8 + 3) / 4));
                switch (s.nv) {
                    case 1: hipLaunchKernelGGL(dad::gn_mish_bwd_wave_kernel<1>, wgrid, dim3(256), 0, st, gp); break;
                    case 2: hipLaunchKernelGGL(dad::gn_mish_bwd_wave_kernel<2>, wgrid, dim3(256), 0, st, gp); break;
                    case 4: hipLaunchKernelGGL(dad::gn_mish_bwd_wave_kernel<4>, wgrid, dim3(256), 0, st, gp); break;
                    case 8: hipLaunchKernelGGL(dad::gn_mish_bwd_wave_kernel<8>, wgrid, dim3(256), 0, st, gp); break;
                    case 16: hipLaunchKernelGGL(dad::gn_mish_bwd_wave_kernel<16>, wgrid, dim3(256), 0, st, gp); break;
                    default: hipLaunchKernelGGL(dad::gn_mish_bwd_kernel, dim3(B, 8), dim3(dad::GNB_THREADS), 0, st, gp);
                }
                HIP_TRY(hipGetLastError());
                break;
            }
            case BK_RESID:
                if ((rc = accumulate(ptr(s.out), ptr(s.in), s.n * B, s.write, st)) != DAD_OK) return rc;
                break;
            case BK_COLS: {
                const long rows = (long)B * s.rows, n4 = rows * (s.C / 4);
                hipLaunchKernelGGL(dad::take_cols_kernel, dim3((unsigned)((n4 + 255) / 256)), dim3(256), 0, st,
                                   ptr(s.out), ptr(s.in), rows, s.C, s.ld, s.off, (int)(s.write == BW_ADD));
                HIP_TRY(hipGetLastError());
                break;
            }
        }
    }
    for (size_t at = 0; at < m->bsums.size(); at += dad::COLS_MAX) {
        dad::ColSumsMany cs{};
        const int n = (int)std::min<size_t>(dad::COLS_MAX, m->bsums.size() - at);
        int widest = 0;
        for (int k = 0; k < n; ++k) {
            const BwdSum& q = m->bsums[at + k];
            cs.out[k] = grad_tensors[q.slot]; cs.part[k] = part + q.part * B; cs.C[k] = q.C;
            widest = std::max(widest, q.C);
        }
        hipLaunchKernelGGL(dad::col_sums_many_kernel, dim3((unsigned)((widest + 31) / 32), (unsigned)n), dim3(256), 0, st, cs, B);
        HIP_TRY(hipGetLastError());
    }
    if (d_x != nullptr) {
        const long n = (long)B * Hr * td;
        if (Hr != H)
            hipLaunchKernelGGL(dad::slice_rows_cols_kernel, dim3((unsigned)((n + 255) / 256)), dim3(256), 0, st, d_x, dxpad, (long)B, H, Hr, td, tdp);
        else
            hipLaunchKernelGGL(dad::slice_cols_kernel, dim3((unsigned)((n + 255) / 256)), dim3(256), 0, st, d_x, dxpad, (long)B * H, td, tdp);
        HIP_TRY(hipGetLastError());
    }
    return DAD_OK;
}

int dad_fill_normal(float* x, int32_t batch, int32_t row_elems, uint64_t seed, uint64_t row_offset,
                    uint64_t draw, dad_stream_t stream) {
    if (!x || batch <= 0 || row_elems <= 0) return fail(DAD_E_INVALID, "bad argument");
    const long n = (long)batch * row_elems;
    hipLaunchKernelGGL(dad::fill_normal_kernel, dim3((unsigned)((n + 255) / 256)), dim3(256), 0,
                       (hipStream_t)stream, x, n, row_offset * (uint64_t)row_elems, draw, seed);
    HIP_TRY(hipGetLastError());
    return DAD_OK;
}

#ifdef DAD_STAMPS
int dad_debug_stamps(void* buf) { g_stamps = (unsigned long long*)buf; return DAD_OK; }
#endif
int dad_debug_kernel_table_consistent(void) {
    const KernTable& t = kernel_table();
    size_t hits = 0;
    for (int cfg = 0; cfg < kNumTiles; ++cfg)
        for (int taps = 1; taps <= kRegMaxTaps; ++taps)
            for (int stride = 1; stride <= 2; ++stride)
                for (int f = 0; f < (1 << kRegFlags); ++f) {
                    const bool x3 = f & 1, bdir = f & 2, ragged = f & 4, res = f & 8, padded = f & 16, win = f & 32;
                    const bool have = t.count(KernKey(cfg, taps, stride, x3, bdir, ragged, res, padded, win)) != 0;
                    if (have != kernel_registered_f(cfg, taps, stride, f)) {
                        fail(DAD_E_INVALID, "kernel table mismatch at tile %d taps=%d stride=%d x3=%d bdir=%d ragged=%d res=%d padded=%d windowed=%d (registry %d)",
                             cfg, taps, stride, (int)x3, (int)bdir, (int)ragged, (int)res, (int)padded, (int)win, (int)have);
                        return 0;
                    }
                    hits += have;
                }
    return hits == t.size() ? 1 : 0;
}

#ifdef DAD_WG_STAMPS
extern "C" int dad_debug_wgrad_stamps(unsigned long long* host32) {
    HIP_TRY(hipDeviceSynchronize());
    HIP_TRY(hipMemcpyFromSymbol(host32, HIP_SYMBOL(dad::g_wg_stamps), 32 * sizeof(unsigned long long)));
    return DAD_OK;
}
#endif

int dad_debug_set_tile(dad_model* m, int32_t cfg) {
    if (!m) return fail(DAD_E_INVALID, "null model");
    m->split_enabled = cfg < 99;
    m->force_tile = cfg >= 99 ? cfg - 100 : cfg;
    return DAD_OK;
}

int dad_debug_set_option(dad_model* m, const char* name, int32_t value) {
    if (!m || !name) return fail(DAD_E_INVALID, "null argument");
    const std::string key(name);
    if (key == "fuse_residual") m->fuse_residual = value != 0;
    else if (key == "xswz") m->xswz_enabled = value != 0;
    else if (key == "xcd_order") m->xcd_order = value != 0;
    else if (key == "split_target") m->split_target = std::max(1, (int)value);
    else if (key == "cc") m->cc_enabled = value != 0;
    else if (key == "cc_max_rows") m->cc_max_rows = std::max(0, (int)value);
    else if (key == "ccw_max_rows") m->ccw_max_rows = std::max(0, (int)value);
    else if (key == "ccw_min_blocks") m->ccw_min_blocks = std::max(1, (int)value);
    else if (key == "ccw_prefer16") m->ccw_prefer16 = value != 0;
    else if (key == "wgrad_blocks") m->wgrad_blocks = std::max(1, (int)value);
    else return fail(DAD_E_INVALID, "unknown option '%s'", name);
    if (!m->graphs.empty()) {
        HIP_TRY(hipDeviceSynchronize());
        for (auto& kv : m->graphs) (void)hipGraphExecDestroy(kv.second);
        m->graphs.clear();
    }
    return DAD_OK;
}

int dad_debug_read_table(dad_model* m, int32_t which, int32_t t, float* host_out, int32_t capacity,
                         int32_t* width_out) {
    if (!m || !host_out) return fail(DAD_E_INVALID, "null argument");
    if (!m->finalized) return fail(DAD_E_STATE, "dad_model_finalize has not been called");
    if (t < 0 || t >= m->cfg.n_timesteps)
        return fail(DAD_E_RANGE, "index %d is out of bounds for the schedule of size %d", t, m->cfg.n_timesteps);
    { const int rc = ensure_tables(m, nullptr); if (rc != DAD_OK) return rc; }
    const float* base = nullptr;
    int width = 0;
    switch (which) {
        case DAD_TABLE_SINUSOID: base = m->d_emb; width = m->cfg.dim; break;
        case DAD_TABLE_TIME_MLP: base = m->d_temb; width = m->cfg.time_dim; break;
        case DAD_TABLE_BLOCKS: base = m->d_temb_table; width = m->plan.temb_width; break;
        default: return fail(DAD_E_INVALID, "unknown table %d", which);
    }
    if (width_out) *width_out = width;
    if (capacity < width)
        return fail(DAD_E_INVALID, "table %d has rows of %d floats, the buffer holds %d", which, width, capacity);
    HIP_TRY(hipDeviceSynchronize());
    HIP_TRY(hipMemcpy(host_out, base + (size_t)t * width, (size_t)width * sizeof(float), hipMemcpyDeviceToHost));
    return DAD_OK;
}

int dad_debug_mish(const float* in, float* out, int64_t n, dad_stream_t stream) {
    if (!in || !out || n <= 0) return fail(DAD_E_INVALID, "bad argument");
    hipLaunchKernelGGL(dad::mish_probe_kernel, dim3((unsigned)((n + 255) / 256)), dim3(256), 0,
                       (hipStream_t)stream, in, out, (long)n);
    HIP_TRY(hipGetLastError());
    return DAD_OK;
}

int dad_debug_small_batch_plan(dad_model* m, int32_t batch, int32_t* launches_out, int32_t* wide_out) {
    if (!m || batch <= 0) return fail(DAD_E_INVALID, "bad argument");
    const CcPlan cc = cc_plan(*m, batch);
    int launches = 0, wide = 0;
    if (cc.ok)
        for (const CcOp& o : cc.ops) {
            launches += o.launched;
            wide += o.launched && o.wide;
        }
    static const bool trace = getenv("DAD_TRACE_TILES") != nullptr;
    if (trace && !cc.ok) fprintf(stderr, "[dad] batch %d: no small-batch plan (%s)\n", batch, cc.why.c_str());
    if (launches_out) *launches_out = launches;
    if (wide_out) *wide_out = wide;
    return DAD_OK;
}

int dad_debug_backward_plan(dad_model* m, int32_t batch, int32_t* out, int32_t capacity, int32_t* needed_out) {
    if (!m || batch <= 0 || capacity < 0 || (capacity > 0 && !out)) return fail(DAD_E_INVALID, "bad argument");
    if (!m->training) return fail(DAD_E_STATE, "dad_model_set_training(m, 1) has not been called");
    if (m->bwd_rc != DAD_OK) return fail(m->bwd_rc, "%s", m->bwd_err.c_str());
    std::vector<int32_t> r;
    const int rc = backward_plan_report(*m, batch, r);
    if (rc != DAD_OK) return rc;
    if (needed_out) *needed_out = (int32_t)r.size();
    std::copy(r.begin(), r.begin() + std::min<size_t>(r.size(), (size_t)capacity), out);
    return DAD_OK;
}

int dad_profile_enable(dad_model* m, int32_t on) {
    if (!m) return fail(DAD_E_INVALID, "null model");
    m->profile = on != 0;
    m->ev_used = 0;
    m->prof_flops = 0;
    m->prof_launches = 0;
    return DAD_OK;
}

int dad_profile_read(dad_model* m, double* conv_ms, int64_t* conv_launches, double* conv_flops) {
    if (!m) return fail(DAD_E_INVALID, "null model");
    double ms = 0;
    for (size_t i = 0; i < m->ev_used; ++i) {
        HIP_TRY(hipEventSynchronize(m->ev_pool[i].second));
        float d = 0;
        HIP_TRY(hipEventElapsedTime(&d, m->ev_pool[i].first, m->ev_pool[i].second));
        ms += d;
    }
    if (conv_ms) *conv_ms = ms;
    if (conv_launches) *conv_launches = m->prof_launches;
    if (conv_flops) *conv_flops = m->prof_flops;
    m->ev_used = 0;
    m->prof_flops = 0;
    m->prof_launches = 0;
    return DAD_OK;
}

}
```

### dynamics_aware_diffusion_amd/csrc/host_plan.hpp

```cpp
#pragma once
#include <algorithm>
#include <array>
#include <cmath>
#include <cstdarg>
#include <cstdint>
#include <cstdio>
#include <cstdlib>
#include <cstring>
#include <functional>
#include <iterator>
#include <map>
#include <string>
#include <vector>

#include "../../include/dad.h"
#include "conv_shapes.hpp"
#include "weight_image.hpp"

namespace dadhost {

inline thread_local char g_err[1024] = "";

inline int fail(int code, const char* fmt, ...) {
    va_list ap;
    va_start(ap, fmt);
    vsnprintf(g_err, sizeof(g_err), fmt, ap);
    va_end(ap);
    return code;
}

struct HostTensor {
    std::vector<float> data;
    std::vector<int64_t> shape;
};

enum ConvKind { CONV_K5 = 0, CONV_1X1 = 1, CONV_DOWN = 2, CONV_UP = 3 };

struct ConvOp {
    std::string name;
    std::string norm;
    ConvKind kind;
    int taps, stride;
    int cin0, cin1, cin_pad;
    int cout;
    int M;
    int Lin, Lout;
    int src0, src1, dst, res;
    int temb_off;
    int kc = 16;
    bool x3 = false;
    bool bdir = false;
    int cat0 = -1, cat1 = -1, cat_c0 = 0, cat_c1 = 0;
    std::string rname;
    int rdst = -1;
    bool ride = false;
    int rider_of = -1;
    float c1 = 1.0f, c2 = 0.0f;
    int pre = -1, stats = -1;
    bool net_padded = false;
    int gn_real = 0;
    int lreal = 0;
    int src_len = 0;
    int real_in = 0, real_out = 0;
    float* d_w = nullptr;
    float* d_bias = nullptr;
    float* d_gamma = nullptr;
    float* d_beta = nullptr;
    float* d_rbias = nullptr;
    double flops_per_sample = 0;
    int wtaps() const { return taps + (ride ? 1 : 0); }
    bool padded() const { return gn_real > 0 || lreal > 0 || src_len > 0; }
};

struct Buf {
    long per_sample;
    long offset;
};

struct Plan {
    std::vector<ConvOp> convs;
    std::vector<Buf> bufs;
    long floats_per_sample = 0;
    int final_act = -1;
    int temb_width = 0;
};

constexpr int kMaxSplitTiles = 4096;
struct TileCfg { int BM, BN, SK, KC; };
constexpr int kNumTiles = 10;
constexpr TileCfg kTiles[kNumTiles] = {
    {32, 64, 4, 32},
    {64, 64, 2, 32},
    {128, 64, 1, 16},
    {256, 32, 1, 8},
    {64, 64, 1, 16},
    {32, 64, 2, 16},
    {32, 64, 1, 16},
    {64, 64, 2, 16},
    {32, 128, 2, 32},
    {64, 128, 1, 16},
};
constexpr int kMaxTileBN = 128;
constexpr bool kWinTiles[kNumTiles] = {true, true, true, false, false, false, false, false, false, false};
constexpr bool kPaddedTiles[kNumTiles] = {true, true, true, true, true, false, false, false, true, true};
constexpr int kGnPassMaxPair = dad::GNP_THREADS * 4 * dad::kGnPassMaxNpt;
inline bool windowed_layer(const ConvOp& op) { return op.Lout > kMaxTileBN; }
inline long tiles_n(const ConvOp& op, int BN, int batch) {
    if (op.Lout > BN) return (long)batch * (op.Lout / BN);
    const int spt = BN / op.Lout;
    return (batch + spt - 1) / spt;
}

constexpr int eff_kc(int cfg_kc, int bm, int taps, int sk = 1, bool x3 = false, bool bd = false, int bn = 64) {
    return bd                          ? 32
           : (taps == 1 && cfg_kc >= 16) ? (bn >= 128 ? 32 : bm >= 128 ? 64 : 128)
           : (x3 && cfg_kc < 16 * sk)  ? 16 * sk
                                       : cfg_kc;
}
constexpr int tile_kc(int cfg, int taps, bool x3, bool bdir) {
    return eff_kc(kTiles[cfg].KC, kTiles[cfg].BM, taps, kTiles[cfg].SK, x3, bdir, kTiles[cfg].BN);
}

enum BwdSpace : int8_t { BSP_NONE, BSP_ACT, BSP_GRAD, BSP_X, BSP_DOUT, BSP_DX };
struct BwdRef { BwdSpace sp = BSP_NONE; int buf = -1; };
enum BwdKind : int8_t {
    BK_BIAS,
    BK_WGRAD,
    BK_DGRAD,
    BK_GN,
    BK_RESID,
    BK_COLS,
};
enum BwdWrite : int8_t { BW_SET, BW_ADD, BW_STAGE };
struct BwdStep {
    BwdKind kind;
    BwdWrite write = BW_SET;
    int conv = -1;
    int sub = 0;
    BwdRef in, out;
    BwdRef z0, z1;
    int slot = -1;
    long part = 0;
    long n = 0;
    int rows = 0, C = 0;
    int off = 0, ld = 0;
    int M = 0, C0 = 0, C1 = 0, taps = 0, stride = 0, pad = 0, Lg = 0, Lz = 0;
    int nv = 0;
};
struct BwdSum { int slot; long part; int C; };

struct HostModel {
    dad_cfg cfg{};
    std::map<std::string, HostTensor> raw;
    std::map<std::string, std::vector<int64_t>> expected;
    Plan plan;
    Plan tplan;
    int precision = DAD_PREC_FP32;
    int force_tile = -1;
    bool split_enabled = true;
    bool fuse_residual = true;
    bool xswz_enabled = true;
    bool xcd_order = true;
    int split_target = 256;
    bool cc_enabled = true;
    int cc_max_rows = 512;
    int ccw_max_rows = 128;
    int ccw_min_blocks = 256;
    int real_channels[DAD_MAX_LEVELS] = {0};
    int real_horizon = 0;
    int wgrad_blocks = 256;
    bool ccw_prefer16 = true;
    mutable std::map<std::array<int, 5>, uint64_t> xswz_cache;
    bool training = false;
    struct BwdConv {
        int n = 0;
        ConvOp op[2];
        int c_lo[2] = {0, 0};
        int c_n[2] = {0, 0};
    };
    std::vector<BwdConv> bconvs;
    ConvOp bfinal;
    struct GradSlot { std::string key; long offset, numel; };
    std::vector<GradSlot> grad_slots;
    long grad_numel = 0;
    std::vector<BwdStep> bsteps;
    std::vector<BwdSum> bsums;
    long bpart = 0;
    bool bdx = false;
    int bwd_rc = DAD_OK;
    std::string bwd_err;
    int max_cout = 0;
    int max_bwd_m = 0;
};

inline int ilog2(int v) { int s = 0; while ((1 << s) < v) ++s; return s; }
inline bool is_pow2(int v) { return v > 0 && (v & (v - 1)) == 0; }

inline int check_cfg(const dad_cfg* cfg) {
    if (!cfg) return fail(DAD_E_INVALID, "null argument");
    if (cfg->kernel_size != 3 && cfg->kernel_size != 5 && cfg->kernel_size != 7)
        return fail(DAD_E_INVALID, "kernel_size %d unsupported (3, 5 or 7)", cfg->kernel_size);
    if (cfg->n_levels < 1 || cfg->n_levels > DAD_MAX_LEVELS)
        return fail(DAD_E_INVALID, "n_levels %d out of range", cfg->n_levels);
    if (cfg->transition_dim < 1 || cfg->dim < 4 || (cfg->dim & 1) || cfg->time_dim < 1)
        return fail(DAD_E_INVALID, "bad transition_dim/dim/time_dim");
    if (!is_pow2(cfg->horizon) || (cfg->horizon >> (cfg->n_levels - 1)) < 4)
        return fail(DAD_E_INVALID, "horizon %d must be a power of two with horizon / 2^(levels-1) >= 4",
                    cfg->horizon);
    if (cfg->n_timesteps < 1) return fail(DAD_E_INVALID, "n_timesteps must be positive");
    for (int i = 0; i < cfg->n_levels; ++i) {
        const int ch = cfg->channels[i];
        if (ch < 32 || ch % 32 != 0 || !is_pow2(ch / 8))
            return fail(DAD_E_INVALID, "level %d has %d channels: need a multiple of 32 with C/8 a power of two",
                        i, ch);
    }
    if (cfg->dim % 32 != 0) return fail(DAD_E_INVALID, "dim %d must be a multiple of 32", cfg->dim);
    return DAD_OK;
}

struct Allocator {
    std::vector<Buf>& bufs;
    std::vector<bool> in_use;
    bool retain;
    explicit Allocator(std::vector<Buf>& b, bool keep = false) : bufs(b), retain(keep) {}
    int get(long per_sample) {
        int best = -1;
        for (size_t i = 0; i < bufs.size() && !retain; ++i)
            if (!in_use[i] && bufs[i].per_sample >= per_sample &&
                (best < 0 || bufs[i].per_sample < bufs[best].per_sample))
                best = (int)i;
        if (best < 0) {
            bufs.push_back({per_sample, 0});
            in_use.push_back(false);
            best = (int)bufs.size() - 1;
        }
        in_use[best] = true;
        return best;
    }
    void put(int id) { if (id >= 0) in_use[id] = false; }
};

inline void expect(HostModel* m, const std::string& key, std::vector<int64_t> shape) {
    m->expected[key] = std::move(shape);
}

inline void decide_kernel_families(HostModel* m) {
    bool padded_net = m->real_horizon > 0 && m->real_horizon != m->cfg.horizon;
    for (int i = 0; i < m->cfg.n_levels; ++i) padded_net = padded_net || (m->real_channels[i] > 0 && m->real_channels[i] != m->cfg.channels[i]);
    for (Plan* plan : {&m->plan, &m->tplan})
    for (ConvOp& op : plan->convs) {
        const int cin_all = op.cin0 + op.cin1;
        op.bdir = op.kc == 8 && op.kind == CONV_K5 &&
                  (op.cin0 % 32) == 0 && (cin_all % 32) == 0 && op.cin_pad == cin_all;
        const bool win = windowed_layer(op);
        op.ride = !op.rname.empty() && !op.bdir && m->precision == DAD_PREC_FP32 && !padded_net && !win;
        op.x3 = !padded_net && !win && ((op.bdir && m->precision == DAD_PREC_F16X3) ||
                (m->precision == DAD_PREC_F16X3 && op.kc == 16 &&
                 ((op.kind == CONV_K5 && op.taps == 5) || op.kind == CONV_1X1 ||
                  ((op.kind == CONV_DOWN || op.kind == CONV_UP) && (op.cin0 & 63) == 0 && (cin_all & 63) == 0))));
        op.net_padded = padded_net;
    }
}

inline int build_plan_into(HostModel* m, Plan& P, bool retain) {
    const dad_cfg& c = m->cfg;
    P = Plan();
    Allocator A(P.bufs, retain);
    const int k = c.kernel_size;
    const int tdm = c.time_dim;
    int temb_off = 0;

    int level_now = 0;
    const bool rows_padded = m->real_horizon > 0 && m->real_horizon != c.horizon;
// ... 200 lines not shown
        const ConvOp& f = convs[i];
        HostModel::BwdConv& b = m->bconvs[i];
        const int cin = f.cin0 + f.cin1;
        switch (f.kind) {
            case CONV_K5: case CONV_1X1:
                b.n = f.cin1 > 0 ? 2 : 1;
                for (int s = 0; s < b.n; ++s) {
                    b.c_lo[s] = s == 0 ? 0 : f.cin0;
                    b.c_n[s] = s == 0 ? f.cin0 : f.cin1;
                    b.op[s] = make_bwd_op(f, s == 0 ? ".dgrad0" : ".dgrad1", f.kind, f.taps, 1, f.cout, b.c_n[s], f.Lin, f.Lin);
                }
                wslot[i] = slot(f.name + ".weight", (long)f.cout * cin * f.taps);
                break;
            case CONV_DOWN:
                b.n = 1; b.c_lo[0] = 0; b.c_n[0] = cin;
                b.op[0] = make_bwd_op(f, ".dgrad0", CONV_UP, 2, 1, f.cout, cin, f.Lout, f.Lout);
                wslot[i] = slot(f.name + ".weight", (long)f.cout * cin * 3);
                break;
            case CONV_UP:
                b.n = 1; b.c_lo[0] = 0; b.c_n[0] = cin;
                b.op[0] = make_bwd_op(f, ".dgrad0", CONV_DOWN, 5, 2, f.cout, cin, 2 * f.Lin, f.Lin);
                wslot[i] = slot(f.name + ".weight", (long)cin * f.cout * 4);
                break;
        }
        for (int s = 0; s < b.n; ++s) {
            const int real_rows = f.kind == CONV_DOWN ? f.real_out : f.real_in;
            const int rows = f.kind == CONV_DOWN ? f.Lout : f.Lin;
            b.op[s].lreal = (real_rows > 0 && real_rows != rows) ? real_rows : 0;
            b.op[s].net_padded = f.net_padded;
        }
        bslot[i] = slot(f.name + ".bias", f.cout);
        if (!f.norm.empty()) { gslot[i] = slot(f.norm + ".weight", f.cout); slot(f.norm + ".bias", f.cout); }
        m->max_cout = std::max(m->max_cout, f.cout);
        for (int s = 0; s < b.n; ++s) m->max_bwd_m = std::max(m->max_bwd_m, b.op[s].M);
    }
    {
        ConvOp f;
        f.name = "final_conv.1";
        m->bfinal = make_bwd_op(f, ".dgrad0", CONV_1X1, 1, 1, c.transition_dim, c.dim, c.horizon, c.horizon);
        if (m->real_horizon > 0 && m->real_horizon != c.horizon) { m->bfinal.lreal = m->real_horizon; m->bfinal.net_padded = true; }
    }
    const int fw = slot("final_conv.1.weight", (long)c.transition_dim * c.dim);
    const int fb = slot("final_conv.1.bias", c.transition_dim);

    std::vector<BwdStep>& S = m->bsteps;
    S.clear(); m->bsums.clear(); m->bpart = 0;
    m->bwd_rc = DAD_OK; m->bwd_err.clear();
    std::vector<int> alias(P.bufs.size(), -1), owner(P.bufs.size(), -1);
    std::vector<char> written(P.bufs.size(), 0);
    char dx = 0;
    for (size_t i = 0; i < convs.size(); ++i) owner[convs[i].dst] = (int)i;
    auto resolve = [&](int id) { while (alias[id] >= 0) id = alias[id]; return id; };
    auto grad = [&](int id) { return BwdRef{BSP_GRAD, resolve(id)}; };
    auto act = [&](int id) { return id == -2 ? BwdRef{BSP_X, -1} : id >= 0 ? BwdRef{BSP_ACT, id} : BwdRef{}; };
    auto write = [&](BwdStep& s, int id) {
        char& w = id == -2 ? dx : written[resolve(id)];
        s.out = id == -2 ? BwdRef{BSP_DX, -1} : grad(id);
        s.write = w ? BW_ADD : BW_SET;
        w = 1;
    };
    auto part_take = [&](int C) { const long q = m->bpart; m->bpart += round_up(C, 4); return q; };
    auto bias = [&](BwdRef in, int rows, int C, int slot_) {
        BwdStep s{BK_BIAS};
        s.in = in; s.rows = rows; s.C = C; s.part = part_take(C);
        S.push_back(s);
        m->bsums.push_back({slot_, s.part, C});
    };
    auto wgrad = [&](BwdRef G, int M, BwdRef z0, int C0, BwdRef z1, int C1, int slot_, int taps, int stride, int pad,
                     int Lg, int Lz) {
        BwdStep s{BK_WGRAD};
        s.in = G; s.M = M; s.z0 = z0; s.C0 = C0; s.z1 = z1; s.C1 = C1; s.slot = slot_;
        s.taps = taps; s.stride = stride; s.pad = pad; s.Lg = Lg; s.Lz = Lz;
        S.push_back(s);
    };
    auto dgrad = [&](int conv, int sub, BwdRef dH, int target, long per_sample) {
        BwdStep s{BK_DGRAD};
        s.conv = conv; s.sub = sub; s.in = dH; s.n = per_sample;
        write(s, target);
        const ConvOp& op = conv < 0 ? m->bfinal : m->bconvs[conv].op[sub];
        if (op.kind == CONV_UP && s.write == BW_ADD) s.write = BW_STAGE;
        S.push_back(s);
    };

    const int H = c.horizon, td = c.transition_dim;
    const BwdRef dout{BSP_DOUT, -1};
    bias(dout, H, td, fb);
    wgrad(dout, td, act(P.final_act), c.dim, BwdRef{}, 0, fw, 1, 1, 0, H, H);
    dgrad(-1, 0, dout, P.final_act, (long)H * c.dim);
    for (int i = (int)convs.size() - 1; i >= 0; --i) {
        const ConvOp& f = convs[i];
        if (!written[resolve(f.dst)] && m->bwd_rc == DAD_OK) {
            m->bwd_rc = fail(DAD_E_STATE, "backward: no gradient reached the output of %s", f.name.c_str());
            m->bwd_err = g_err;
        }
        const BwdRef gout = grad(f.dst);
        const int out_rows = f.kind == CONV_UP ? 2 * f.Lout : f.Lout;
        BwdRef dH = gout;
        if (!f.norm.empty()) {
            auto resid = [&](int target) {
                BwdStep s{BK_RESID};
                s.in = gout; s.n = (long)out_rows * f.cout;
                write(s, target);
                S.push_back(s);
            };
            if (f.res == -2) {
                resid(-2);
            } else if (f.cat0 >= 0) {
                const int ids[2] = {f.cat0, f.cat1}, cs[2] = {f.cat_c0, f.cat_c1};
                for (int k = 0, off = 0; k < 2; off += cs[k], ++k) {
                    BwdStep s{BK_COLS};
                    s.in = gout; s.rows = out_rows; s.C = cs[k]; s.off = off; s.ld = f.cout;
                    write(s, ids[k]);
                    S.push_back(s);
                }
            } else if (f.res >= 0) {
                const int q = owner[f.res];
                if (q >= 0 && convs[q].kind == CONV_1X1 && convs[q].norm.empty()) alias[f.res] = resolve(f.dst);
                else resid(f.res);
            }
            BwdStep s{BK_GN};
            s.conv = i; s.in = gout; s.out = BwdRef{BSP_GRAD, f.pre};
            s.part = part_take(f.cout); part_take(f.cout); part_take(f.cout);
            const int f4 = f.cout / 8 / 4 * f.Lout;
            s.nv = f4 <= 64 ? 1 : f4 <= 128 ? 2 : f4 <= 256 ? 4 : f4 <= 512 ? 8 : f4 <= 1024 ? 16 : 0;
            S.push_back(s);
            const long c4 = round_up(f.cout, 4);
            m->bsums.push_back({gslot[i], s.part, f.cout});
            m->bsums.push_back({gslot[i] + 1, s.part + c4, f.cout});
            m->bsums.push_back({bslot[i], s.part + 2 * c4, f.cout});
            dH = s.out;
        } else {
            bias(dH, out_rows, f.cout, bslot[i]);
        }
        switch (f.kind) {
            case CONV_K5: case CONV_1X1:
                wgrad(dH, f.cout, act(f.src0), f.cin0, act(f.src1), f.cin1, wslot[i], f.taps, 1, f.taps / 2, f.Lin, f.Lin); break;
            case CONV_DOWN:
                wgrad(dH, f.cout, act(f.src0), f.cin0, BwdRef{}, 0, wslot[i], 3, 2, 1, f.Lout, f.Lin); break;
            case CONV_UP:
                wgrad(act(f.src0), f.cin0, dH, f.cout, BwdRef{}, 0, wslot[i], 4, 2, 1, f.Lin, 2 * f.Lin); break;
        }
        const HostModel::BwdConv& b = m->bconvs[i];
        for (int k = 0; k < b.n; ++k) dgrad(i, k, dH, k == 0 ? f.src0 : f.src1, (long)f.Lin * b.c_n[k]);
    }
    m->bdx = dx != 0;
    return DAD_OK;
}
inline const char* training_refusal(const HostModel& m) {
    if (m.precision != DAD_PREC_FP32) return "the backward pass exists for the fp32 arithmetic only";
    return nullptr;
}

inline bool tile_valid(const ConvOp& op, int cfg);
inline int check_tiles(const HostModel& m) {
    for (const ConvOp& op : m.plan.convs) {
        bool any = false;
        for (int cfg = 0; cfg < kNumTiles && !any; ++cfg) any = tile_valid(op, cfg);
        if (!any)
            return fail(DAD_E_INVALID, "no tile configuration for %s (M=%d, C/8=%d, L=%d, %d taps)",
                        op.name.c_str(), op.M, op.cout / 8, op.Lout, op.taps);
    }
    return DAD_OK;
}
inline int build_plan(HostModel* m) {
    m->expected.clear();
    int rc = build_plan_into(m, m->plan, false);
    if (rc == DAD_OK) rc = build_plan_into(m, m->tplan, true);
    if (rc == DAD_OK) decide_kernel_families(m);
    if (rc == DAD_OK) rc = check_tiles(*m);
    if (rc == DAD_OK) rc = build_backward_plan(m);
    return rc;
}

inline uint16_t f16_bits(float v) {
    const _Float16 h = (_Float16)v;
    uint16_t b;
    std::memcpy(&b, &h, 2);
    return b;
}
inline int split_f16_image(std::vector<float>& packed) {
    float amax = 0.0f;
    for (float v : packed) amax = std::max(amax, std::fabs(v));
    int s = 0;
    if (amax > 0.0f && std::isfinite(amax)) {
        int e;
        std::frexp(amax, &e);
        s = 10 - e;
    }
    s = std::max(-100, std::min(100, s));
    const float up = std::ldexp(1.0f, s);
    for (size_t g = 0; g + 16 <= packed.size(); g += 16) {
        uint16_t hi[16], lo[16];
        for (int j = 0; j < 16; ++j) {
            const float v = packed[g + j] * up;
            const _Float16 h = (_Float16)v;
            hi[j] = f16_bits(v);
            lo[j] = f16_bits((v - (float)h) * 2048.0f);
        }
        std::memcpy(&packed[g], hi, 32);
        std::memcpy(&packed[g + 8], lo, 32);
    }
    return s;
}

inline dad::ImageDesc image_desc(const ConvOp& op, int mode, int CO, int CI, int K, int c_lo = 0, int c_n = 0) {
    dad::ImageDesc p{};
    p.mode = mode;
    p.kg = op.bdir ? 16 : op.kc;
    p.wtaps = op.wtaps(); p.M = op.M;
    p.n = (long)op.cin_pad * p.wtaps * op.M;
    p.CO = CO; p.CI = CI; p.K = K; p.c_lo = c_lo; p.c_n = c_n;
    return p;
}
inline dad::ImageDesc fwd_image(const ConvOp& op) {
    const int cin = op.cin0 + op.cin1;
    return op.kind == CONV_UP ? image_desc(op, dad::IMG_FWD_UP, op.cout, cin, 4) : image_desc(op, dad::IMG_FWD, op.cout, cin, op.taps);
}
inline dad::ImageDesc bwd_image(const ConvOp& f, const HostModel::BwdConv& b, int k) {
    const int mode = f.kind == CONV_DOWN ? dad::IMG_BWD_DOWN : f.kind == CONV_UP ? dad::IMG_BWD_UP : dad::IMG_BWD_CONV;
    return image_desc(b.op[k], mode, f.cout, f.cin0 + f.cin1, f.taps, b.c_lo[k], b.c_n[k]);
}
inline dad::ImageDesc bfinal_image(const HostModel& m) {
    return image_desc(m.bfinal, dad::IMG_BWD_FINAL, m.cfg.transition_dim, m.cfg.dim, 1);
}

enum WeightTarget { WT_W, WT_BIAS, WT_RBIAS, WT_GAMMA, WT_BETA, WT_BWD_W, WT_BFINAL_W, WT_FINAL_W, WT_FINAL_B, WT_TIME };
struct WeightEntry {
    WeightTarget to;
    int conv, sub;
    std::string key, key2;
    dad::ImageDesc img;
    long floats = 0;
    int reps = 1;
    float* dev = nullptr;
    size_t size() const { return img.n > 0 ? (size_t)img.n : (size_t)floats * reps; }
};
inline std::vector<WeightEntry> weight_table(const HostModel& m) {
    std::vector<WeightEntry> t;
    auto copy = [&](WeightTarget to, int conv, const std::string& key, long floats, int reps = 1) {
        t.push_back({to, conv, 0, key, "", dad::ImageDesc{}, floats, reps});
    };
    for (const auto& kv : m.expected)
        if (kv.first.find("time_mlp.") != std::string::npos) {
            long n = 1;
            for (int64_t d : kv.second) n *= (long)d;
            copy(WT_TIME, -1, kv.first, n);
        }
    for (int i = 0; i < (int)m.plan.convs.size(); ++i) {
        const ConvOp& op = m.plan.convs[i];
        t.push_back({WT_W, i, 0, op.name + ".weight", op.ride ? op.rname + ".weight" : "", fwd_image(op)});
        for (int k = 0; m.training && k < m.bconvs[i].n; ++k)
            t.push_back({WT_BWD_W, i, k, op.name + ".weight", "", bwd_image(m.tplan.convs[i], m.bconvs[i], k)});
        copy(WT_BIAS, i, op.name + ".bias", op.cout, op.kind == CONV_UP ? 2 : 1);
        if (op.ride) copy(WT_RBIAS, i, op.rname + ".bias", op.cout);
        if (!op.norm.empty()) { copy(WT_GAMMA, i, op.norm + ".weight", op.cout); copy(WT_BETA, i, op.norm + ".bias", op.cout); }
    }
    copy(WT_FINAL_W, -1, "final_conv.1.weight", (long)m.cfg.transition_dim * m.cfg.dim);
    if (m.training) t.push_back({WT_BFINAL_W, -1, 0, "final_conv.1.weight", "", bfinal_image(m)});
    copy(WT_FINAL_B, -1, "final_conv.1.bias", m.cfg.transition_dim);
    return t;
}

inline void pack_image(const dad::ImageDesc& p, float* out) {
    const long chunks = p.n / ((long)p.wtaps * p.M * p.kg);
    for (long c = 0; c < chunks; ++c)
        for (int slot = 0; slot < p.wtaps; ++slot)
            for (int o = 0; o < p.M; ++o)
                for (int j = 0; j < p.kg; ++j) *out++ = dad::image_value(p, (int)c * p.kg + j, slot, o);
}
inline int pack_entry(HostModel* m, const WeightEntry& e, std::vector<float>& out) {
    auto src = [&](const std::string& key) -> const float* {
        auto it = m->raw.find(key);
        return it == m->raw.end() ? nullptr : it->second.data.data();
    };
    const float* w = src(e.key);
    const float* ride = e.key2.empty() ? nullptr : src(e.key2);
    if (!w || (!e.key2.empty() && !ride)) return fail(DAD_E_KEY, "missing key '%s'", (w ? e.key2 : e.key).c_str());
    out.resize(e.size());
    if (e.img.n == 0) {
        for (int r = 0; r < e.reps; ++r) std::copy(w, w + e.floats, out.begin() + r * e.floats);
        return DAD_OK;
    }
    dad::ImageDesc p = e.img;
    p.w = w; p.ride = ride;
    pack_image(p, out.data());
    if (e.to == WT_W) {
        ConvOp& op = m->plan.convs[e.conv];
        op.c1 = 1.0f; op.c2 = 0.0f;
        if (op.x3) {
            const int sh = split_f16_image(out);
            op.c1 = std::ldexp(1.0f, -sh);
            op.c2 = std::ldexp(1.0f, -sh - 11);
        }
    }
    return DAD_OK;
}

inline bool tile_valid(const ConvOp& op, int cfg) {
    const TileCfg& t = kTiles[cfg];
    if (windowed_layer(op)) {
        if (!kWinTiles[cfg] || op.x3 || op.bdir || op.kc != 16 || op.Lout % t.BN != 0) return false;
        if ((op.kind == CONV_UP ? op.M / 2 : op.M) % t.BM != 0) return false;
        if (!op.norm.empty() && (long)(op.cout / 8) * op.Lout > kGnPassMaxPair) return false;
        const int kc = tile_kc(cfg, op.taps, false, false);
        return dad::conv_lds_floats(t.BM, t.BN, kc, op.taps, op.Lin, op.Lout, t.SK, false, op.taps) * sizeof(float) <=
               dad::kLdsBytes;
    }
    if (op.net_padded && !kPaddedTiles[cfg]) return false;
    const int Mrows = op.kind == CONV_UP ? op.M / 2 : op.M;
    const int cpg = op.norm.empty() ? 1 : op.cout / 8;
    if ((t.KC == 8) != (op.kc == 8)) return false;
    if (Mrows % t.BM != 0) return false;
    if (!op.norm.empty() && (t.BM % cpg != 0)) return false;
    if (t.BN % op.Lout != 0) return false;
    const int nthreads = 64 * (t.BM / 32) * (t.BN / 32) * t.SK;
    const int f4pl = t.BM * t.BN / 4 / nthreads;
    if (!op.norm.empty() && op.Lout * cpg / 4 < f4pl) return false;
    const int kc = tile_kc(cfg, op.taps, op.x3, op.bdir);
    if (dad::conv_lds_floats(t.BM, t.BN, kc, op.taps, op.Lin, op.Lout, t.SK, op.bdir, op.taps) * sizeof(float) > dad::kLdsBytes)
        return false;
    return true;
}
inline int choose_tile(const HostModel& m, const ConvOp& op, int batch) {
    auto valid = [&](int cfg) { return tile_valid(op, cfg); };
    auto blocks = [&](int cfg) {
        const TileCfg& t = kTiles[cfg];
        return tiles_n(op, t.BN, batch) * (op.M / t.BM);
    };
    if (op.kc == 8) return valid(3) ? 3 : -1;
    if (m.force_tile >= 0 && m.force_tile < kNumTiles && valid(m.force_tile)) return m.force_tile;
    if (valid(2) && blocks(2) >= 512) return 2;
    if (valid(1) && blocks(1) >= 224) return 1;
    if (valid(0)) return 0;
    if (valid(1)) return 1;
    if (valid(2)) return 2;
    if (valid(4)) return 4;
    if (valid(8)) return 8;
    if (valid(9)) return 9;
    return -1;
}

inline uint64_t find_xswz(const HostModel& m, int L, int stride, int pad, int kp4, int BN) {
    if (L >= 32 || pad == 0 || BN / L > 16) return 0;
    const std::array<int, 5> key{L, stride, pad, kp4, BN};
    auto it = m.xswz_cache.find(key);
    if (it != m.xswz_cache.end()) return it->second;
    static const int groups[2][16] = {{0, 1, 2, 3, 12, 13, 14, 15, 20, 21, 22, 23, 24, 25, 26, 27},
                                      {4, 5, 6, 7, 8, 9, 10, 11, 16, 17, 18, 19, 28, 29, 30, 31}};
    const int S = BN / L, seg = L * stride + 2 * pad, per = 32 / L;
    std::vector<int> d(S, 0);
    auto ok_prefix = [&](int upto) {
        for (int tn = 0; tn * per < upto; ++tn)
            for (const auto& g : groups) {
                unsigned seen = 0;
                for (int lane : g) {
                    const int n = tn * 32 + lane, sm = n / L, l = n % L;
                    if (sm >= upto) continue;
                    const unsigned bit = 1u << (((sm * seg + l * stride) * kp4 + d[sm]) & 15);
                    if (seen & bit) return false;
                    seen |= bit;
                }
            }
        return true;
    };
    long budget = 300000;
    std::function<bool(int)> place = [&](int sm) -> bool {
        if (sm == S) return true;
        for (int v = 0; v < 16; ++v) {
            if (--budget < 0) return false;
            if (sm > 0 && d[sm - 1] - v > pad * kp4) continue;
            d[sm] = v;
            if (ok_prefix(sm + 1) && place(sm + 1)) return true;
        }
        d[sm] = 0;
        return false;
    };
    uint64_t packed = 0;
    if (place(0))
        for (int sm = 0; sm < S; ++sm) packed |= (uint64_t)d[sm] << (4 * sm);
    m.xswz_cache[key] = packed;
    return packed;
}

struct SplitPlan { int kslices, chunks_per_slice; long slab_floats; };
inline SplitPlan plan_split(const HostModel& m, const ConvOp& op, int cfg, int batch) {
    const TileCfg& t = kTiles[cfg];
    const long tiles = tiles_n(op, t.BN, batch) * (op.M / t.BM);
    const int kc = tile_kc(cfg, op.taps, op.x3, op.bdir);
    const int nchunks = (op.cin0 + op.cin1 + kc - 1) / kc;
    SplitPlan sp{1, nchunks, 0};
    if (!m.split_enabled) return sp;
    if (tiles >= 160 || nchunks < 2 || tiles > kMaxSplitTiles) return sp;
    int want = tiles * 2 <= m.split_target ? (int)(m.split_target / tiles) : (int)((m.split_target + tiles - 1) / tiles);
    if (want > nchunks) want = nchunks;
    if (want < 2) return sp;
    sp.chunks_per_slice = (nchunks + want - 1) / want;
    sp.kslices = (nchunks + sp.chunks_per_slice - 1) / sp.chunks_per_slice;
    sp.slab_floats = tiles * sp.kslices * (long)t.BN * t.BM;
    return sp;
}

struct LaunchGeom {
    int cfg = -1;
    int kc = 0;
    bool ragged = false;
    int threads = 0;
    size_t lds_bytes = 0;
    int ntiles_n = 0, mtiles = 0;
    unsigned gx = 1, gy = 1, gz = 1;
    int xcd_gn = 0, xcd_mts = 0, xcd_ntn = 0;
    bool fused = false;
    bool padded = false;
    bool windowed = false;
    int gn_npt = 0;
    SplitPlan split{1, 0, 0};
    uint64_t xswz = 0;
};

inline bool fused_at(const HostModel& m, const ConvOp& op, const LaunchGeom& g) {
    if (!op.ride || !m.fuse_residual || g.cfg < 0) return false;
    const TileCfg& t = kTiles[g.cfg];
    if (t.KC < 16 || g.split.kslices != 1) return false;
    return dad::conv_lds_floats(t.BM, t.BN, g.kc, op.taps, op.Lin, op.Lout, t.SK, false, op.taps + 1) *
               sizeof(float) <= dad::kLdsBytes;
}
inline void choose_launch(const HostModel& m, const ConvOp& op, int batch, LaunchGeom& g) {
    g = LaunchGeom();
    g.cfg = choose_tile(m, op, batch);
    if (g.cfg < 0) return;
    g.kc = tile_kc(g.cfg, op.taps, op.x3, op.bdir);
    g.split = plan_split(m, op, g.cfg, batch);
    g.fused = fused_at(m, op, g);
}

constexpr int kRegMaxTaps = 7;
constexpr int kRegFlags = 6;
constexpr bool kernel_registered(int cfg, int taps, int stride, bool x3, bool bdir, bool ragged, bool res, bool padded = false,
                                 bool windowed = false) {
    if (cfg < 0 || cfg >= kNumTiles) return false;
    if (windowed) {
        if (!kWinTiles[cfg] || !padded || x3 || bdir || res) return false;
        const bool odd = taps == 3 || taps == 5 || taps == 7 || taps == 1;
        if (ragged) return stride == 1 && odd;
        return (stride == 1 && (odd || taps == 2)) || (stride == 2 && (taps == 3 || (taps == 5 && kTiles[cfg].KC >= 16)));
    }
    if (padded && (!kPaddedTiles[cfg] || x3 || res)) return false;
    const bool kc16 = kTiles[cfg].KC >= 16;
    const bool k357 = taps == 3 || taps == 5 || taps == 7;
    if (ragged && !(stride == 1 && (k357 || taps == 1) && !bdir)) return false;
    if (bdir) return !kc16 && !res && !ragged && stride == 1 && k357;
    if (res) return kc16 && !x3 && stride == 1 && k357;
    if (x3) return kc16 && ((taps == 5 && stride == 1) || (taps == 3 && stride == 2) || (taps == 2 && stride == 1) ||
                            (taps == 1 && stride == 1));
    if (stride == 2) return taps == 3 || (taps == 5 && kc16);
    return stride == 1 && (taps == 1 || taps == 2 || k357);
}
constexpr bool kernel_registered_f(int cfg, int taps, int stride, int f) {
    return kernel_registered(cfg, taps, stride, f & 1, f & 2, f & 4, f & 8, f & 16, f & 32);
}
constexpr int count_registered() {
    int n = 0;
    for (int cfg = 0; cfg < kNumTiles; ++cfg)
        for (int taps = 1; taps <= kRegMaxTaps; ++taps)
            for (int stride = 1; stride <= 2; ++stride)
                for (int f = 0; f < (1 << kRegFlags); ++f) n += kernel_registered_f(cfg, taps, stride, f);
    return n;
}
static_assert(count_registered() == 335, "the set of conv-GEMM kernels changed: kernel_registered");

inline int plan_launch(const HostModel& m, const ConvOp& op, int batch, LaunchGeom& g) {
    choose_launch(m, op, batch, g);
    if ((long)batch * op.Lout * op.M >= (1L << 31) ||
        (long)batch * op.Lin * (op.cin0 + op.cin1) >= (1L << 31))
        return fail(DAD_E_INVALID, "batch %d too large: a layer's activation tensor exceeds 2^31 elements", batch);
    if (g.cfg < 0)
        return fail(DAD_E_INVALID, "no tile configuration for %s (M=%d, C/8=%d, L=%d)",
                    op.name.c_str(), op.M, op.cout / 8, op.Lout);
    const TileCfg& t = kTiles[g.cfg];
    const int cin = op.cin0 + op.cin1;
    g.ragged = (op.cin0 & 3) != 0 || (op.cin1 & 3) != 0 || op.cin0 % g.kc != 0 || cin % g.kc != 0;
    if (g.ragged && !(op.stride == 1 && (op.taps & 1) == 1))
        return fail(DAD_E_INVALID, "channel count %d+%d needs the general staging path, which exists "
                    "for stride-1 k-tap and 1x1 convs only", op.cin0, op.cin1);
    if (op.bdir && g.ragged)
        return fail(DAD_E_INVALID, "the direct-B kernel needs whole 32-channel chunks (%d+%d)", op.cin0, op.cin1);
    if (op.bdir && !(t.KC == 8 && op.kind == CONV_K5 && op.stride == 1))
        return fail(DAD_E_INVALID, "no direct-B kernel for tile %d taps=%d stride=%d", g.cfg, op.taps, op.stride);
    if (op.x3 && !op.bdir && t.KC < 16)
        return fail(DAD_E_INVALID, "no split-f16 kernel for tile %d taps=%d stride=%d", g.cfg, op.taps, op.stride);
    if (g.fused && (op.x3 || op.bdir || op.kind != CONV_K5 || op.stride != 1))
        return fail(DAD_E_INVALID, "no fused-residual kernel for %s on tile %d", op.name.c_str(), g.cfg);
    if (op.cin_pad % g.kc != 0 && !g.ragged)
        return fail(DAD_E_INVALID, "%s: padded channel count %d is not a multiple of the K chunk %d",
                    op.name.c_str(), op.cin_pad, g.kc);
    g.windowed = op.Lout > t.BN;
    g.padded = op.net_padded || g.windowed;
    if (!kernel_registered(g.cfg, op.taps, op.stride, op.x3, op.bdir, g.ragged, g.fused, g.padded, g.windowed))
        return fail(DAD_E_INVALID, "no kernel for %s (tile %d taps=%d stride=%d x3=%d bdir=%d ragged=%d res=%d padded=%d windowed=%d)",
                    op.name.c_str(), g.cfg, op.taps, op.stride, (int)op.x3, (int)op.bdir, (int)g.ragged, (int)g.fused, (int)g.padded,
                    (int)g.windowed);
    if (g.windowed && !op.norm.empty() && (long)(op.cout / 8) * op.Lout > kGnPassMaxPair)
        return fail(DAD_E_INVALID, "%s: GroupNorm pair of %ld elements (the pass holds %d)", op.name.c_str(),
                    (long)(op.cout / 8) * op.Lout, kGnPassMaxPair);
    if (g.windowed && !op.norm.empty()) {
        const long elems = (long)(op.cout / 8) * op.Lout, per = dad::GNP_THREADS * 4L;
        if (op.kind != CONV_K5 || (op.cout / 8) % 4 != 0)
            return fail(DAD_E_INVALID, "%s: no GroupNorm pass for %ld-element pairs", op.name.c_str(), elems);
        for (g.gn_npt = 1; elems > g.gn_npt * per; g.gn_npt *= 2) {}
    }
    g.threads = 64 * (t.BM / 32) * (t.BN / 32) * t.SK;
    g.lds_bytes = dad::conv_lds_floats(t.BM, t.BN, g.kc, op.taps, op.Lin, op.Lout, t.SK, op.bdir,
                                       op.taps + (g.fused ? 1 : 0)) * sizeof(float);
    if (g.lds_bytes > dad::kLdsBytes)
        return fail(DAD_E_INVALID, "%s: tile %d needs %zu bytes of LDS", op.name.c_str(), g.cfg, g.lds_bytes);
    const long ntn = tiles_n(op, t.BN, batch);
    if (ntn > 65535) return fail(DAD_E_INVALID, "batch too large for one launch (%ld N tiles)", ntn);
    g.ntiles_n = (int)ntn;
    g.mtiles = op.M / t.BM;
    if (g.split.kslices > 1 && (long)g.mtiles * g.ntiles_n > kMaxSplitTiles)
        return fail(DAD_E_INVALID, "%s: %ld tiles exceed the split-K ticket table", op.name.c_str(),
                    (long)g.mtiles * g.ntiles_n);
    const int MT = g.mtiles, NTn = g.ntiles_n;
    g.gx = (unsigned)g.split.kslices; g.gy = (unsigned)MT; g.gz = (unsigned)NTn;
    g.xcd_gn = 0;
    if (m.xcd_order && g.split.kslices == 1 && (MT & (MT - 1)) == 0 && (long)MT * NTn <= 65535 &&
        ((long)MT * NTn) % 8 == 0) {
        const double wbytes = (double)op.M * op.taps * cin;
        const double xbytes = (double)batch * op.Lin * cin;
        double best = -1;
        for (int gm = 1; gm <= 8; gm *= 2) {
            const int gn = 8 / gm;
            if (MT % gm != 0 || NTn % gn != 0) continue;
            const double cost = gn * wbytes + gm * xbytes;
            if (best < 0 || cost < best) {
                best = cost;
                g.xcd_gn = gn; g.xcd_mts = ilog2(MT / gm); g.xcd_ntn = NTn / gn;
            }
        }
        if (g.xcd_gn > 0) { g.gy = (unsigned)(MT * NTn); g.gz = 1; }
    }
    g.xswz = m.xswz_enabled ? find_xswz(m, op.Lout, op.stride, op.taps / 2, (g.kc + 4) / 4, t.BN) : 0;
    return DAD_OK;
}

constexpr int kCcMaxSlabs = 16;
constexpr int kCcMaxSlice = 64;
constexpr int kCcwMaxSlabs = 8;
using dad::kCcwMaxPairs;
constexpr int kCcwMaxPair = 8192;
struct CcInput {
    int kind = 0;
    int buf = -1;
    int producer = -1;
};
struct CcOp {
    bool launched = false;
    bool wide = false;
    int slice_ch = 0, kslices = 0, ntiles = 0;
    int tile_rows = 32;
    bool big = false;
    bool ride_in = false;
    long oslab = 0, orslab = -1;
    int out_rows = 0, out_cols = 0;
    size_t lds_bytes = 0;
    CcInput in0, in1;
    int res_kind = 0;
    int res_buf = -1, res_ride = -1;
};
struct CcPlan {
    bool ok = false;
    std::vector<CcOp> ops;
    long slab_floats = 0;
    int final_producer = -1;
    std::string why;
};
inline CcPlan& refuse(CcPlan& P, const char* why) { P.why = why; return P; }
constexpr bool cc_kernel_exists(int taps, int stride, bool ride, bool wide, bool big, int rows, bool windowed) {
    if ((rows != 16 && rows != 32) || (ride && !(taps == 5 && stride == 1))) return false;
    const bool shape_ok = (taps == 5 && stride == 1) || (taps == 3 && stride == 2) || (taps == 2 && stride == 1);
    if (wide) return !big && !windowed && (shape_ok || (taps == 1 && stride == 1));
    if (windowed) return taps == 5 && stride == 1 && !big && rows == 32;
    return shape_ok;
}

inline CcPlan cc_plan(const HostModel& m, int batch) {
    CcPlan P;
    const dad_cfg& c = m.cfg;
    const std::vector<ConvOp>& convs = m.plan.convs;
    if (m.precision != DAD_PREC_FP32 || !m.cc_enabled || c.horizon > 128 || c.kernel_size != 5 ||
        (long)batch * c.horizon > m.cc_max_rows)
        return refuse(P, "disabled, split-f16 arithmetic, horizon > 128, kernel_size != 5 or more than cc_max_rows rows");
    if (c.horizon > 32 && (long)batch * c.horizon > 256)
        return refuse(P, "horizon > 32 and more than 256 rows");
    for (const ConvOp& op : convs)
        if (op.gn_real > 0) return refuse(P, "zero-padded GroupNorm groups (dad_model_set_group_channels): batch kernels only");
    if (m.real_horizon > 0 && m.real_horizon != c.horizon) return refuse(P, "zero-padded horizon (dad_model_set_horizon): batch kernels only");
    for (const ConvOp& op : convs)
        if ((op.kc != 16 && !op.bdir) || op.cat0 >= 0 || op.x3 || (!op.rname.empty() && !op.ride)) return refuse(P, "a weight image not in 16-channel granules, or an identity residual over a concat");
    P.ops.resize(convs.size());
    std::vector<int> owner(m.plan.bufs.size(), -1);
    std::vector<char> materialised(convs.size(), 0);
    long off = 0;
    for (size_t i = 0; i < convs.size(); ++i) {
        const ConvOp& op = convs[i];
        CcOp& o = P.ops[i];
        if (op.rider_of >= 0) { owner[op.dst] = -2 - op.rider_of; continue; }
        o.launched = true;
        auto input = [&](int buf, CcInput& in) -> bool {
            if (buf == -1) { in.kind = 0; return true; }
            if (buf == -2) { in.kind = 1; return true; }
            const int q = owner[buf];
            if (q < 0) return false;
            in.buf = buf;
            if (materialised[q]) { in.kind = 2; return true; }
            in.kind = 3; in.producer = q; materialised[q] = 1;
            return true;
        };
        if (!input(op.src0, o.in0) || !input(op.src1, o.in1)) return refuse(P, "input with no known producer");
        const bool windowed = op.Lout > 32;
        if (op.M % 32 != 0 || (!windowed && 32 % op.Lout != 0) || (windowed && (op.Lout % 32 != 0 || op.kind != CONV_K5)))
            return refuse(P, "output columns not a multiple of 32, a length that does not divide 32, or a long layer that is not a stride-1 conv");
        const int cin = op.cin0 + op.cin1;
        int need = 32, max_slabs_in = 0;
        long max_pair = 0;
        for (const CcInput* in : {&o.in0, &o.in1})
            if (in->kind == 3) {
                const ConvOp& q = convs[in->producer];
                const CcOp& qo = P.ops[in->producer];
                max_slabs_in = std::max(max_slabs_in, qo.kslices);
                if (qo.res_kind >= 3) max_slabs_in = std::max(max_slabs_in, P.ops[qo.res_ride].kslices);
                o.ride_in = o.ride_in || qo.res_kind >= 3;
                if (!q.norm.empty()) {
                    need = std::max(need, q.cout / 8);
                    max_pair = std::max(max_pair, (long)(q.cout / 8) * op.Lin);
                    if (need % (q.cout / 8) != 0) return refuse(P, "inputs whose GroupNorm widths do not nest");
                }
            }
        int slice = need;
        while ((cin + slice - 1) / slice > 8 && slice < kCcMaxSlice) slice *= 2;
        while ((cin + slice - 1) / slice > kCcMaxSlabs) slice *= 2;
        o.wide = slice > kCcMaxSlice || max_pair > 1024 || op.bdir || op.kind == CONV_1X1;
        if (o.wide && (windowed || op.Lin > 32)) return refuse(P, "a wide layer (conv_ccw) of more than 32 positions");
        if (windowed && max_slabs_in > 8) return refuse(P, "a windowed layer fed more than 8 slabs");
        if (!o.wide) {
            if (slice % 32 != 0) return refuse(P, "K slice not a multiple of 32 channels");
            o.tile_rows = 32;
            if (op.Lout <= 16) {
                const int ks = (cin + slice - 1) / slice;
                const long blocks16 = (long)((batch + 16 / op.Lout - 1) / (16 / op.Lout)) * (op.M / 32) * ks;
                if (blocks16 <= 256) o.tile_rows = 16;
// ... 294 lines not shown
```

### dynamics_aware_diffusion_amd/csrc/pointwise.hpp

```cpp
#pragma once
#include <hip/hip_runtime.h>
#include <stdint.h>

#include "conv_gemm.hpp"

namespace dad {

__host__ __device__ inline void philox4x32_10(uint32_t c0, uint32_t c1, uint32_t c2, uint32_t c3,
                                              uint32_t k0, uint32_t k1, uint32_t out[4]) {
    const uint32_t M0 = 0xD2511F53u, M1 = 0xCD9E8D57u, W0 = 0x9E3779B9u, W1 = 0xBB67AE85u;
#pragma unroll
    for (int r = 0; r < 10; ++r) {
        const uint64_t p0 = (uint64_t)M0 * c0;
        const uint64_t p1 = (uint64_t)M1 * c2;
        const uint32_t n0 = (uint32_t)(p1 >> 32) ^ c1 ^ k0;
        const uint32_t n1 = (uint32_t)p1;
        const uint32_t n2 = (uint32_t)(p0 >> 32) ^ c3 ^ k1;
        const uint32_t n3 = (uint32_t)p0;
        c0 = n0; c1 = n1; c2 = n2; c3 = n3;
        k0 += W0; k1 += W1;
    }
    out[0] = c0; out[1] = c1; out[2] = c2; out[3] = c3;
}

__device__ __forceinline__ float philox_normal(uint64_t e, uint64_t draw, uint64_t seed) {
    uint32_t r[4];
    const uint64_t q = e >> 2;
    philox4x32_10((uint32_t)q, (uint32_t)(q >> 32), (uint32_t)draw, (uint32_t)(draw >> 32),
                  (uint32_t)seed, (uint32_t)(seed >> 32), r);
    const int pair = (int)((e >> 1) & 1);
    const uint32_t ra = r[2 * pair], rb = r[2 * pair + 1];
    const float u1 = ((float)(ra >> 9) + 0.5f) * (1.0f / 8388608.0f);
    const float u2 = (float)(rb >> 8) * (1.0f / 16777216.0f);
    const float rad = sqrtf(-2.0f * logf(u1));
    const float ang = 6.28318530717958647692f * u2;
    return (e & 1) ? rad * sinf(ang) : rad * cosf(ang);
}

__global__ void set_u64_kernel(unsigned long long* dst, unsigned long long v) { *dst = v; }

__global__ void fill_normal_kernel(float* x, long n_elems, uint64_t elem_offset, uint64_t draw,
                                   uint64_t seed) {
    const long i = (long)blockIdx.x * blockDim.x + threadIdx.x;
    if (i < n_elems) x[i] = philox_normal(elem_offset + (uint64_t)i, draw, seed);
}

__global__ void concat_rows_kernel(float* dst, const float* a, const float* b, long rows, int c0, int c1) {
    const int q = (c0 + c1) >> 2;
    const long i = (long)blockIdx.x * blockDim.x + threadIdx.x;
    if (i >= rows * q) return;
    const long r = i / q;
    const int c = (int)(i - r * q) * 4;
    const float4 v = c < c0 ? *reinterpret_cast<const float4*>(a + r * c0 + c)
                            : *reinterpret_cast<const float4*>(b + r * c1 + (c - c0));
    *reinterpret_cast<float4*>(dst + r * (c0 + c1) + c) = v;
}

struct FinalParams {
    const float* act;
    const float* w;
    const float* bias;
    float* x;
    const float* noise;
    const float* cond0;
    const float* guide;
    float* mean_out;
    float* eps_out;
    int32_t dim, td, B, H;
    int32_t Hact;
    int32_t cond_per_row;
    int32_t predict_epsilon, clip_denoised;
    int32_t x_out_disabled;
    float c_recip, c_recipm1, coef1, coef2;
    float sigma;
    float guide_scale;
    uint64_t seed, elem_offset, draw;
    const unsigned long long* seed_dev;
};


template <int K>
__device__ __forceinline__ void final_dots(const float* wrow0, const float* arow, int dim, int rstep, float* acc) {
    const float* wr[K];
    float a[K][4];
#pragma unroll
    for (int k = 0; k < K; ++k) {
        wr[k] = wrow0 + (long)k * rstep;
        a[k][0] = a[k][1] = a[k][2] = a[k][3] = 0.0f;
    }
    for (int c = 0; c < dim; c += 4) {
        const float4 av = *reinterpret_cast<const float4*>(arow + c);
#pragma unroll
        for (int k = 0; k < K; ++k) {
            const float4 wv = *reinterpret_cast<const float4*>(wr[k] + c);
            a[k][0] = fmaf(wv.x, av.x, a[k][0]); a[k][1] = fmaf(wv.y, av.y, a[k][1]);
            a[k][2] = fmaf(wv.z, av.z, a[k][2]); a[k][3] = fmaf(wv.w, av.w, a[k][3]);
        }
    }
#pragma unroll
    for (int k = 0; k < K; ++k) acc[k] = (a[k][0] + a[k][1]) + (a[k][2] + a[k][3]);
}

__global__ __launch_bounds__(256) void final_posterior_kernel(const FinalParams p) {
    extern __shared__ __attribute__((aligned(16))) float ws[];
    const int td = p.td, dim = p.dim;
    const int rs = dim + 4;
    constexpr int JG = 256 / FINAL_COLS;
    const int rows_local = final_rows_local(td, (int)gridDim.y);
    float* wl = ws;
    float* bl = wl + rows_local * dim;
    float* tile = bl + ((td + 3) & ~3);
    const long N = (long)p.B * p.H;
    const long n0 = (long)blockIdx.x * FINAL_COLS;
    const int dq = dim >> 2;
    for (int e = threadIdx.x; e < FINAL_COLS * dq; e += blockDim.x) {
        const int row = e / dq, q = e - row * dq;
        float4 v = make_float4(0.f, 0.f, 0.f, 0.f);
        if (n0 + row < N) {
            long ar = n0 + row;
            if (p.Hact != p.H) { const long sb = ar / p.H; ar = sb * p.Hact + (ar - sb * p.H); }
            v = *reinterpret_cast<const float4*>(p.act + ar * dim + q * 4);
        }
        *reinterpret_cast<float4*>(tile + row * rs + q * 4) = v;
    }
    for (int i = threadIdx.x; i < rows_local * dq; i += blockDim.x) {
        const int lr = i / dq, q = i - lr * dq;
        const int j = ((lr / JG) * (int)gridDim.y + (int)blockIdx.y) * JG + lr % JG;
        float4 v = make_float4(0.f, 0.f, 0.f, 0.f);
        if (j < td) v = *reinterpret_cast<const float4*>(p.w + (long)j * dim + q * 4);
        *reinterpret_cast<float4*>(wl + i * 4) = v;
    }
    for (int i = threadIdx.x; i < td; i += blockDim.x) bl[i] = p.bias[i];
    __syncthreads();

    const int col = threadIdx.x & (FINAL_COLS - 1);
    const int jg = threadIdx.x / FINAL_COLS;
    const long n = n0 + col;
    if (n >= N) return;
    const int b = (int)(n / p.H);
    const int l = (int)(n - (long)b * p.H);
    const float* arow = tile + col * rs;
    auto finish = [&](int j, float acc, float xv) {
        const long idx = n * td + j;
        const float out = acc + bl[j];
        if (p.eps_out != nullptr) p.eps_out[idx] = out;
        if (p.x_out_disabled && p.mean_out == nullptr) return;
        float x0 = p.predict_epsilon ? p.c_recip * xv - p.c_recipm1 * out : out;
        if (p.clip_denoised) x0 = fminf(fmaxf(x0, -1.0f), 1.0f);
        float mean = p.coef1 * x0 + p.coef2 * xv;
        if (p.guide != nullptr) mean = mean + p.guide_scale * p.guide[idx];
        if (p.mean_out != nullptr) p.mean_out[idx] = mean;
        if (p.x_out_disabled) return;
        const float z = (p.noise != nullptr)
                            ? p.noise[idx]
                            : philox_normal(p.elem_offset + (uint64_t)idx, p.draw,
                                            p.seed_dev != nullptr ? (uint64_t)*p.seed_dev : p.seed);
        float xn = mean + p.sigma * z;
        if (l == 0 && p.cond0 != nullptr) xn = p.cond0[(p.cond_per_row ? (long)b * td : 0) + j];
        p.x[idx] = xn;
    };
    constexpr int JB = 4;
    const int jstep = JG * (int)gridDim.y;
    for (int jb = (int)blockIdx.y * JG; jb < td; jb += JB * jstep) {
        const int j0 = jb + jg;
        const int live = min(JB, (td - 1 - jb) / jstep + 1);
        float acc[JB], xv[JB];
#pragma unroll
        for (int k = 0; k < JB; ++k) xv[k] = p.x[n * td + min(j0 + k * jstep, td - 1)];
        const float* wrow0 = wl + (long)(((jb / JG) / (int)gridDim.y) * JG + jg) * dim;
        switch (live) {
            case 1: final_dots<1>(wrow0, arow, dim, JG * dim, acc); break;
            case 2: final_dots<2>(wrow0, arow, dim, JG * dim, acc); break;
            case 3: final_dots<3>(wrow0, arow, dim, JG * dim, acc); break;
            default: final_dots<4>(wrow0, arow, dim, JG * dim, acc); break;
        }
#pragma unroll
        for (int k = 0; k < JB; ++k)
            if (k < live && j0 + k * jstep < td) finish(j0 + k * jstep, acc[k], xv[k]);
    }
}

struct ProjParams {
    const float* P;
    const float* obs_mean; const float* obs_std; const float* act_mean; const float* act_std;
    float* x;
    float* xout;
    int32_t B, H, n, od, m, D;
    float alpha, one_minus_alpha;
    float* violation;
};

template <int RB, int KP>
__global__ __launch_bounds__(64 * KP) void project_kernel(const ProjParams p) {
    extern __shared__ __attribute__((aligned(16))) float v[];
    const int D = p.D, H = p.H, n = p.n, m = p.m, td = p.od + p.m;
    float* part = v + RB * D;
    const int b0 = blockIdx.x * RB;
    const int nstate = (H + 1) * n;
    for (int e = threadIdx.x; e < RB * D; e += blockDim.x) {
        const int r = e / D, d = e - r * D;
        const int b = b0 + r;
        float val = 0.0f;
        if (b < p.B) {
            const float* xb = p.x + (long)b * H * td;
            if (d < nstate) {
                const int ts = d / n, k = d - ts * n;
                const int tsrc = ts < H ? ts : H - 1;
                val = xb[tsrc * td + k] * p.obs_std[k] + p.obs_mean[k];
            } else {
                const int dd = d - nstate;
                const int ts = dd / m, k = dd - ts * m;
                val = xb[ts * td + p.od + k] * p.act_std[k] + p.act_mean[k];
            }
        }
        v[e] = val;
    }
    __syncthreads();
    const int dl = threadIdx.x & 63, kp = threadIdx.x >> 6;
    const int kq = (D + KP - 1) / KP;
    const int k0 = kp * kq, k1 = min(D, k0 + kq);
    for (int d = dl; d < D; d += 64) {
        float acc[RB];
#pragma unroll
        for (int r = 0; r < RB; ++r) acc[r] = 0.0f;
        const float* pc = p.P + d;
#pragma unroll 8
        for (int k = k0; k < k1; ++k) {
            const float pk = pc[(long)k * D];
#pragma unroll
            for (int r = 0; r < RB; ++r) acc[r] = fmaf(v[r * D + k], pk, acc[r]);
        }
#pragma unroll
        for (int r = 0; r < RB; ++r) part[(kp * RB + r) * D + d] = acc[r];
    }
    __syncthreads();
    if (p.violation != nullptr) {
        if (threadIdx.x < 64) {
            for (int r = 0; r < RB; ++r) {
                float acc = 0.0f;
                for (int d = threadIdx.x; d < D; d += 64) {
                    float proj = 0.0f;
#pragma unroll
                    for (int q = 0; q < KP; ++q) proj += part[(q * RB + r) * D + d];
                    const float diff = v[r * D + d] - proj;
                    acc = fmaf(diff, diff, acc);
                }
                for (int o = 32; o > 0; o >>= 1) acc += __shfl_xor(acc, o, 64);
                if (threadIdx.x == 0 && b0 + r < p.B) p.violation[b0 + r] = acc;
            }
        }
        return;
    }
    for (int e = threadIdx.x; e < RB * D; e += blockDim.x) {
        const int r = e / D, d = e - r * D;
        const int b = b0 + r;
        if (b >= p.B) continue;
        float proj = 0.0f;
#pragma unroll
        for (int q = 0; q < KP; ++q) proj += part[(q * RB + r) * D + d];
        const float blended = p.alpha * proj + p.one_minus_alpha * v[r * D + d];
        float* xb = p.x + (long)b * H * td;
        if (d < nstate) {
            const int ts = d / n, k = d - ts * n;
            if (ts < H) xb[ts * td + k] = (blended - p.obs_mean[k]) / p.obs_std[k];
        } else {
            const int dd = d - nstate;
            const int ts = dd / m, k = dd - ts * m;
            xb[ts * td + p.od + k] = (blended - p.act_mean[k]) / p.act_std[k];
        }
    }
    if (p.od > n) {
        const int extra = p.od - n;
        for (int e = threadIdx.x; e < RB * H * extra; e += blockDim.x) {
            const int r = e / (H * extra);
            const int rem = e - r * H * extra;
            const int ts = rem / extra, k = rem - ts * extra;
            const int b = b0 + r;
            if (b < p.B) p.x[((long)b * H + ts) * td + n + k] = 0.0f;
        }
    }
}

constexpr int PG_THREADS = 256;
constexpr int PG_KC = 64;
constexpr int PG_AS = 33;
__host__ __device__ inline size_t project_gemm_lds_floats() { return (size_t)4 * PG_KC * PG_AS + 64; }

__device__ __forceinline__ float proj_gather(const ProjParams& p, const float* xb, int d, int nstate, int td) {
    if (d < nstate) {
        const int ts = d / p.n, k = d - ts * p.n;
        const int tsrc = ts < p.H ? ts : p.H - 1;
        return xb[tsrc * td + k] * p.obs_std[k] + p.obs_mean[k];
    }
    const int dd = d - nstate;
    const int ts = dd / p.m, k = dd - ts * p.m;
    return xb[ts * td + p.od + k] * p.act_std[k] + p.act_mean[k];
}

__global__ __launch_bounds__(PG_THREADS) void project_gemm_kernel(const ProjParams p) {
    extern __shared__ __attribute__((aligned(16))) float sm[];
    const int tid = threadIdx.x, lane = tid & 63;
    const int wave = __builtin_amdgcn_readfirstlane(tid >> 6);
    const int l32 = lane & 31, h = lane >> 5;
    const int D = p.D, H = p.H, td = p.od + p.m;
    const int nstate = (H + 1) * p.n;
    const int b0 = blockIdx.x * 32, d0 = blockIdx.y * 32;
    float* const As = sm + wave * (PG_KC * PG_AS);
    f32x16 acc;
#pragma unroll
    for (int r = 0; r < 16; ++r) acc[r] = 0.0f;
    const int nchunks = (D + PG_KC - 1) / PG_KC;
    const int dcol = min(d0 + l32, D - 1);
    for (int ch = wave; ch < nchunks; ch += 4) {
        const int k0 = ch * PG_KC;
        float bv[PG_KC / 2];
#pragma unroll
        for (int j = 0; j < PG_KC / 2; ++j) {
            const int k = min(k0 + 2 * j + h, D - 1);
            bv[j] = p.P[(long)k * D + dcol];
        }
        {
            const int k = k0 + lane;
            for (int r = 0; r < 32; ++r) {
                const int b = b0 + r;
                float v = 0.0f;
                if (k < D && b < p.B) v = proj_gather(p, p.x + (long)b * H * td, k, nstate, td);
                As[lane * PG_AS + r] = v;
            }
        }
        __builtin_amdgcn_fence(__ATOMIC_RELEASE, "wavefront");
#pragma unroll
// ... 62 lines not shown
```

### include/dad.h

```cpp
#ifndef DAD_H
#define DAD_H

#include <stddef.h>
#include <stdint.h>

#ifdef __cplusplus
extern "C" {
#endif

#define DAD_OK 0
#define DAD_E_INVALID (-1)
#define DAD_E_STATE (-2)
#define DAD_E_KEY (-3)
#define DAD_E_HIP (-4)
#define DAD_E_RANGE (-5)
#define DAD_E_WORKSPACE (-6)

#define DAD_MAX_LEVELS 8

#define DAD_PREC_FP32 0
#define DAD_PREC_F16X3 1

typedef struct dad_model dad_model;
typedef void* dad_stream_t;

typedef struct dad_cfg {
    int32_t transition_dim;
    int32_t dim;
    int32_t time_dim;
    int32_t n_levels;
    int32_t channels[DAD_MAX_LEVELS];
    int32_t kernel_size;
    int32_t horizon;
    int32_t n_timesteps;
    int32_t predict_epsilon;
    int32_t clip_denoised;
} dad_cfg;

const char* dad_last_error(void);
const char* dad_version(void);

int dad_model_create(const dad_cfg* cfg, dad_model** out);
void dad_model_destroy(dad_model* m);

int dad_model_load_weight(dad_model* m, const char* key, const float* data,
                          const int64_t* shape, int32_t ndim);

int dad_model_load_schedule(dad_model* m, const float* sqrt_recip, const float* sqrt_recipm1,
                            const float* coef1, const float* coef2, const float* log_var);

int dad_model_load_time_embedding(dad_model* m, const float* emb, int32_t n_timesteps, int32_t dim);

int dad_model_set_precision(dad_model* m, int32_t precision);

int dad_model_set_group_channels(dad_model* m, const int32_t* real_channels, int32_t n_levels);

int dad_model_set_horizon(dad_model* m, int32_t real_horizon);
int dad_model_finalize(dad_model* m, dad_stream_t stream);

int dad_workspace_bytes(const dad_model* m, int32_t batch, size_t* bytes);

int dad_unet_forward(dad_model* m, const float* x, int32_t t, float* out, int32_t batch,
                     void* workspace, size_t workspace_bytes, dad_stream_t stream);

int dad_unet_forward_rows(dad_model* m, const float* x, const int32_t* t_rows, float* out, int32_t batch,
                          void* workspace, size_t workspace_bytes, dad_stream_t stream);

int dad_model_set_training(dad_model* m, int32_t on);
int dad_model_refresh_weights(dad_model* m, int32_t n, const char* const* keys, const float* const* tensors,
                              dad_stream_t stream);
int dad_train_grad_count(const dad_model* m, int32_t* count, int64_t* total_floats);
int dad_train_grad_info(const dad_model* m, int32_t i, const char** key, int64_t* offset, int64_t* numel);
int dad_train_workspace_bytes(const dad_model* m, int32_t batch, size_t* saved_bytes, size_t* scratch_bytes);
int dad_unet_forward_train(dad_model* m, const float* x, const int32_t* row_index, const float* temb_rows,
                           float* out, int32_t batch, void* saved, size_t saved_bytes, dad_stream_t stream);
int dad_unet_backward(dad_model* m, const float* x, const float* d_out, float* d_x, float* d_temb_rows,
                      float* const* grad_tensors, int32_t n_grad_tensors, int32_t batch, void* saved,
                      size_t saved_bytes, void* scratch, size_t scratch_bytes, dad_stream_t stream);

typedef struct dad_step_args {
    const float* noise;
    uint64_t seed;
    uint64_t row_offset;
    uint64_t draw;
    const float* cond0;
    int32_t cond_per_row;
    const float* guide_grad;
    float guide_weight;
    float* mean_out;
    float* eps_out;
} dad_step_args;

int dad_denoise_step(dad_model* m, float* x, int32_t t, int32_t batch, const dad_step_args* args,
                     int32_t x_out_disabled, void* workspace, size_t workspace_bytes,
                     dad_stream_t stream);

typedef struct dad_project_args {
    const float* P;
    const float* obs_mean;
    const float* obs_std;
    const float* act_mean;
    const float* act_std;
    int32_t state_dim;
    int32_t observation_dim;
    int32_t action_dim;
    float* scratch;
    size_t scratch_bytes;
} dad_project_args;

int dad_sample_loop(dad_model* m, float* x, int32_t n_steps, int32_t batch,
                    const float* noise_stack, uint64_t seed, uint64_t row_offset,
                    const float* cond0, int32_t cond_per_row,
                    const dad_project_args* proj, const float* proj_alphas_host,
                    int32_t use_graph, void* workspace, size_t workspace_bytes,
                    dad_stream_t stream);

int dad_project(const dad_project_args* p, float alpha, float* x, int32_t batch,
                int32_t horizon, dad_stream_t stream);

int dad_projection_violation(const dad_project_args* p, const float* x, float* violation, int32_t batch,
                             int32_t horizon, dad_stream_t stream);

int dad_fill_normal(float* x, int32_t batch, int32_t row_elems, uint64_t seed,
                    uint64_t row_offset, uint64_t draw, dad_stream_t stream);

int dad_profile_enable(dad_model* m, int32_t on);
int dad_profile_read(dad_model* m, double* conv_ms, int64_t* conv_launches, double* conv_flops);

int dad_debug_set_tile(dad_model* m, int32_t cfg);
int dad_debug_set_option(dad_model* m, const char* name, int32_t value);

#define DAD_TABLE_SINUSOID 0
#define DAD_TABLE_TIME_MLP 1
#define DAD_TABLE_BLOCKS 2
int dad_debug_read_table(dad_model* m, int32_t which, int32_t t, float* host_out, int32_t capacity,
                         int32_t* width_out);
int dad_debug_mish(const float* in, float* out, int64_t n, dad_stream_t stream);
int dad_debug_kernel_table_consistent(void);
int dad_debug_small_batch_plan(dad_model* m, int32_t batch, int32_t* launches_out, int32_t* wide_out);
#define DAD_BP_WGRADS 0
#define DAD_BP_MULTI 1
#define DAD_BP_MAX_CHUNKS 2
#define DAD_BP_MAX_KSPLIT 3
#define DAD_BP_PART 4
#define DAD_BP_PART_MULTI 5
#define DAD_BP_WINDOWED 6
#define DAD_BP_TILE 7
#define DAD_BP_TAPS_TILE 11
#define DAD_BP_FWD 31
#define DAD_BP_DGRAD 51
#define DAD_BP_RECORD_INTS 71
#define DAD_BP_HEADER 72
#define DAD_BP_REC_TAPS 0
#define DAD_BP_REC_TILE 1
#define DAD_BP_REC_WINDOWED 2
#define DAD_BP_REC_SAMPLES 3
#define DAD_BP_REC_SPC 4
#define DAD_BP_REC_SPS 5
#define DAD_BP_REC_KSPLIT 6
#define DAD_BP_REC_CHUNKS 7
#define DAD_BP_REC_LAST_CHUNKS 8
#define DAD_BP_REC_INTS 9
int dad_debug_backward_plan(dad_model* m, int32_t batch, int32_t* out, int32_t capacity, int32_t* needed_out);

#ifdef __cplusplus
}
#endif
#endif
```

Baseline: 3454 plans/s.

## Add narrow-channel conv tile path and split final projection dot over K slices

```diff
diff --git a/dynamics_aware_diffusion_amd/_engine.py b/dynamics_aware_diffusion_amd/_engine.py
--- a/dynamics_aware_diffusion_amd/_engine.py
+++ b/dynamics_aware_diffusion_amd/_engine.py
@@ -79,6 +79,8 @@
     "dad_debug_kernel_table_consistent": (C.c_int, []),
     "dad_debug_small_batch_plan": (C.c_int, [C.c_void_p, C.c_int32, C.POINTER(C.c_int32),
                                              C.POINTER(C.c_int32)]),
+    "dad_debug_forward_plan": (C.c_int, [C.c_void_p, C.c_int32, C.POINTER(C.c_int32), C.c_int32,
+                                         C.POINTER(C.c_int32)]),
     "dad_debug_backward_plan": (C.c_int, [C.c_void_p, C.c_int32, C.POINTER(C.c_int32), C.c_int32,
                                           C.POINTER(C.c_int32)]),
     "dad_model_set_training": (C.c_int, [C.c_void_p, C.c_int32]),
@@ -523,6 +525,16 @@
         _check(self.lib, self.lib.dad_debug_small_batch_plan(self._h, int(batch), C.byref(n), C.byref(w)))
         return n.value, w.value
 
+    def forward_plan(self, batch: int) -> list:
+        need = C.c_int32()
+        _check(self.lib, self.lib.dad_debug_forward_plan(self._h, int(batch), None, 0, C.byref(need)))
+        buf = (C.c_int32 * need.value)()
+        _check(self.lib, self.lib.dad_debug_forward_plan(self._h, int(batch), buf, need.value, C.byref(need)))
+        r = list(buf)
+        fields = ("conv", "tile", "kc", "kslices", "fused", "ragged", "narrow", "blocks")
+        assert r[1] == len(fields) and len(r) == 2 + r[0] * r[1]
+        return [dict(zip(fields, r[at:at + len(fields)])) for at in range(2, len(r), len(fields))]
+
     def backward_plan(self, batch: int) -> dict:
         need = C.c_int32()
         _check(self.lib, self.lib.dad_debug_backward_plan(self._h, int(batch), None, 0, C.byref(need)))
diff --git a/dynamics_aware_diffusion_amd/csrc/conv_gemm.hpp b/dynamics_aware_diffusion_amd/csrc/conv_gemm.hpp
--- a/dynamics_aware_diffusion_amd/csrc/conv_gemm.hpp
+++ b/dynamics_aware_diffusion_amd/csrc/conv_gemm.hpp
@@ -132,6 +132,13 @@
     return make_float4(v.x, v.y, v.z, v.w);
 }
 
+__device__ __forceinline__ float4 ldg4u(const float* p) {
+    typedef float __attribute__((ext_vector_type(4), aligned(4))) f4u;
+    const f4u v = *reinterpret_cast<const __attribute__((address_space(1))) f4u*>(
+        (const __attribute__((address_space(1))) float*)p);
+    return make_float4(v.x, v.y, v.z, v.w);
+}
+
 __device__ __forceinline__ void store_f4_sc1(float* p, const float4 v) {
     typedef float __attribute__((ext_vector_type(4))) f4;
     const f4 x = {v.x, v.y, v.z, v.w};
@@ -151,10 +158,12 @@
     constexpr int KU = X3 ? 16 : 8;
     constexpr int G = KC / KU;
     constexpr int GW = G / SK;
-    constexpr int KG = KC < 16 ? KC : 16;
-    constexpr int NSUB = KC / KG;
+    constexpr int KG = (KC < 16 && BM == 256) ? KC : 16;
+    constexpr bool HALFG = KC < KG;
+    constexpr int NSUB = HALFG ? 1 : KC / KG;
     static_assert(KC % KU == 0 && G % SK == 0 && GW >= 1, "K chunk must split evenly over the SK waves");
     static_assert(!BDIR || (BN == 32 && SK == 1 && !RAGGED && KC >= 16), "direct-B tiles");
+    static_assert(!HALFG || (RAGGED && !X3 && !BDIR && !WIN && KC == 8), "half-granule chunks: narrow first layers");
     static_assert(!RES || (!X3 && !BDIR && (TAPS & 1) == 1 && TAPS >= 3 && STRIDE == 1), "the residual ride exists for fp32 stride-1 convs of the net's kernel size");
     static_assert(!WIN || (PADDED && !X3 && !BDIR && !RES), "windowed tiles: fp32, LDS-staged, no ride");
     constexpr int BN_SH = BN == 32 ? 5 : BN == 64 ? 6 : 7;
@@ -269,7 +278,20 @@
     DAD_PSTAMP(6);
     const long w_chunk_stride = (long)NSUB * p.wtaps * M * KG;
     constexpr int NLD = W_PER_T + X_PER_T;
-    auto item_store = [&](int k, int stage) {
+    const float* rag_src0 = p.src0;
+    const float* rag_src1 = p.src1;
+    constexpr bool RAGU = RAGGED && HALFG;
+    if constexpr (RAGU) asm volatile("" : "+s"(rag_src0), "+s"(rag_src1));
+    const int rag_rows = p.B * ((PADDED && p.src_len > 0) ? p.src_len : Lin);
+    auto rag_src = [&](int cc, int grow, bool& second, int& cs, int& cl, int& at, int& d) {
+        second = cc >= p.cin0 && p.cin1 > 0;
+        cs = second ? p.cin1 : p.cin0;
+        cl = second ? cc - p.cin0 : cc;
+        const int want = max(grow, 0) * cs + cl;
+        at = min(want, rag_rows * cs - 4);
+        d = want - at;
+    };
+    auto item_store = [&](int k, int stage, int chunk) {
         const int base4 = stage * STAGE4;
         if (k < W_PER_T) {
             if (W_F4 % NT == 0 || tid + k * NT < W_F4)
@@ -279,6 +301,17 @@
             if (x_loff[i] >= 0) {
                 float4 v = xreg[i];
                 if (!RAGGED && x_grow[i] < 0) v = make_float4(0.f, 0.f, 0.f, 0.f);
+                if constexpr (RAGU) {
+                    const int cc = chunk * KC + x_q4[i];
+                    bool second; int cs, cl, at, d;
+                    rag_src(cc, x_grow[i], second, cs, cl, at, d);
+                    const int left = (x_grow[i] >= 0 && cc < cin) ? cs - cl : 0;
+                    const float a1 = v.y, a2 = v.z, a3 = v.w;
+                    v.x = left > 0 ? (d == 0 ? v.x : d == 1 ? a1 : d == 2 ? a2 : a3) : 0.0f;
+                    v.y = left > 1 ? (d == 0 ? a1 : d == 1 ? a2 : a3) : 0.0f;
+                    v.z = left > 2 ? (d == 0 ? a2 : a3) : 0.0f;
+                    v.w = left > 3 ? a3 : 0.0f;
+                }
                 if constexpr (X3) {
                     float2 hi, lo;
                     split_f16x4(v, hi, lo);
@@ -294,7 +327,8 @@
         if (k < W_PER_T) {
             float4 v = make_float4(0.f, 0.f, 0.f, 0.f);
             if (W_F4 % NT == 0 || tid + k * NT < W_F4)
-                v = *reinterpret_cast<const float4*>(p.w + chunk * w_chunk_stride + w_goff[k]);
+                v = *reinterpret_cast<const float4*>(p.w + (HALFG ? (chunk >> 1) * w_chunk_stride + (chunk & 1) * KC
+                                                                   : chunk * w_chunk_stride) + w_goff[k]);
             wreg[k] = v;
         } else {
             const int i = k - W_PER_T;
@@ -306,6 +340,10 @@
                 const int cs = second ? p.cin1 : p.cin0;
                 const int cb = second ? c0 - p.cin0 : c0;
                 v = *reinterpret_cast<const float4*>(xsrc + (long)max(x_grow[i], 0) * cs + cb + x_q4[i]);
+            } else if constexpr (RAGU) {
+                bool second; int cs, cl, at, d;
+                rag_src(c0 + x_q4[i], x_grow[i], second, cs, cl, at, d);
+                v = ldg4u((second ? rag_src1 : rag_src0) + at);
             } else {
                 const int cc = c0 + x_q4[i];
                 if (x_grow[i] >= 0 && cc < cin) {
@@ -441,7 +479,7 @@
     }
     DAD_PSTAMP(2);
 #pragma unroll
-    for (int k = 0; k < NLD; ++k) item_store(k, 0);
+    for (int k = 0; k < NLD; ++k) item_store(k, 0, c_begin);
     DAD_PSTAMP(3);
     if (c_begin + 1 < nchunks) {
 #pragma unroll
@@ -464,7 +502,7 @@
 #define DAD_ROLL(STORE, LOAD)                                                                    \
     _Pragma("unroll") for (int k = 0; k < NLD; ++k) {                                            \
         if ((BDIR ? UW - 1 : (k * UW) / NLD) != u) continue;       \
-        if (STORE) item_store(k, cur ^ 1);                                                       \
+        if (STORE) item_store(k, cur ^ 1, ch + 1);                                               \
         if (LOAD) item_load(k, ch + 2);                                                          \
     }
 #else
diff --git a/dynamics_aware_diffusion_amd/csrc/dad_lib.hip b/dynamics_aware_diffusion_amd/csrc/dad_lib.hip
--- a/dynamics_aware_diffusion_amd/csrc/dad_lib.hip
+++ b/dynamics_aware_diffusion_amd/csrc/dad_lib.hip
@@ -150,16 +150,16 @@
 }
 
 using KernFn = void (*)(const ConvParams);
-using KernKey = std::tuple<int, int, int, bool, bool, bool, bool, bool, bool>;
+using KernKey = std::tuple<int, int, int, bool, bool, bool, bool, bool, bool, bool>;
 using KernTable = std::map<KernKey, KernFn>;
 
 template <int CFG, int TAPS, int STRIDE, int F>
 void reg_kernel(KernTable& t) {
     if constexpr (kernel_registered_f(CFG, TAPS, STRIDE, F)) {
         constexpr TileCfg T = kTiles[CFG];
-        constexpr bool X3 = F & 1, BDIR = F & 2, RAGGED = F & 4, RES = F & 8, PADDED = F & 16, WIN = F & 32;
-        t[KernKey(CFG, TAPS, STRIDE, X3, BDIR, RAGGED, RES, PADDED, WIN)] =
-            dad::conv_gemm_f32<T.BM, T.BN, T.SK, tile_kc(CFG, TAPS, X3, BDIR), TAPS, STRIDE, RAGGED, X3, BDIR, RES, PADDED, WIN>;
+        constexpr bool X3 = F & 1, BDIR = F & 2, RAGGED = F & 4, RES = F & 8, PADDED = F & 16, WIN = F & 32, NARROW = F & 64;
+        t[KernKey(CFG, TAPS, STRIDE, X3, BDIR, RAGGED, RES, PADDED, WIN, NARROW)] =
+            dad::conv_gemm_f32<T.BM, T.BN, T.SK, tile_kc(CFG, TAPS, X3, BDIR, NARROW), TAPS, STRIDE, RAGGED, X3, BDIR, RES, PADDED, WIN>;
     }
 }
 template <int CFG, int TAPS, size_t... F>
@@ -379,10 +379,10 @@
                    ? g_stamps + (size_t)(&op - &m->plan.convs[0]) * 4096 * 8 : nullptr;
 #endif
     const auto& table = kernel_table();
-    const auto it = table.find(KernKey(g.cfg, op.taps, op.stride, op.x3, op.bdir, g.ragged, g.fused, g.padded, g.windowed));
+    const auto it = table.find(KernKey(g.cfg, op.taps, op.stride, op.x3, op.bdir, g.ragged, g.fused, g.padded, g.windowed, g.narrow));
     if (it == table.end())
-        return fail(DAD_E_INVALID, "no kernel for %s (tile %d taps=%d stride=%d x3=%d bdir=%d ragged=%d res=%d)",
-                    op.name.c_str(), g.cfg, op.taps, op.stride, (int)op.x3, (int)op.bdir, (int)g.ragged, (int)g.fused);
+        return fail(DAD_E_INVALID, "no kernel for %s (tile %d taps=%d stride=%d x3=%d bdir=%d ragged=%d res=%d narrow=%d)",
+                    op.name.c_str(), g.cfg, op.taps, op.stride, (int)op.x3, (int)op.bdir, (int)g.ragged, (int)g.fused, (int)g.narrow);
     void* args[] = {&p};
     HIP_TRY(hipLaunchKernel((const void*)it->second, dim3(g.gx, g.gy, g.gz), dim3(g.threads), args,
                             g.lds_bytes, st));
@@ -1278,11 +1278,11 @@
         for (int taps = 1; taps <= kRegMaxTaps; ++taps)
             for (int stride = 1; stride <= 2; ++stride)
                 for (int f = 0; f < (1 << kRegFlags); ++f) {
-                    const bool x3 = f & 1, bdir = f & 2, ragged = f & 4, res = f & 8, padded = f & 16, win = f & 32;
-                    const bool have = t.count(KernKey(cfg, taps, stride, x3, bdir, ragged, res, padded, win)) != 0;
+                    const bool x3 = f & 1, bdir = f & 2, ragged = f & 4, res = f & 8, padded = f & 16, win = f & 32, narrow = f & 64;
+                    const bool have = t.count(KernKey(cfg, taps, stride, x3, bdir, ragged, res, padded, win, narrow)) != 0;
                     if (have != kernel_registered_f(cfg, taps, stride, f)) {
-                        fail(DAD_E_INVALID, "kernel table mismatch at tile %d taps=%d stride=%d x3=%d bdir=%d ragged=%d res=%d padded=%d windowed=%d (registry %d)",
-                             cfg, taps, stride, (int)x3, (int)bdir, (int)ragged, (int)res, (int)padded, (int)win, (int)have);
+                        fail(DAD_E_INVALID, "kernel table mismatch at tile %d taps=%d stride=%d x3=%d bdir=%d ragged=%d res=%d padded=%d windowed=%d narrow=%d (registry %d)",
+                             cfg, taps, stride, (int)x3, (int)bdir, (int)ragged, (int)res, (int)padded, (int)win, (int)narrow, (int)have);
                         return 0;
                     }
                     hits += have;
@@ -1374,6 +1374,23 @@
     return DAD_OK;
 }
 
+int dad_debug_forward_plan(dad_model* m, int32_t batch, int32_t* out, int32_t capacity, int32_t* needed_out) {
+    if (!m || batch <= 0 || capacity < 0 || (capacity > 0 && !out)) return fail(DAD_E_INVALID, "bad argument");
+    FwdPlan f;
+    const int rc = plan_forward(*m, false, batch, true, f);
+    if (rc != DAD_OK) return rc;
+    std::vector<int32_t> r = {(int32_t)f.launches.size(), DAD_FP_REC_INTS};
+    for (const FwdLaunch& l : f.launches) {
+        const LaunchGeom& g = l.g;
+        const int32_t rec[DAD_FP_REC_INTS] = {l.conv, g.cfg, g.kc, g.split.kslices, g.fused, g.ragged, g.narrow,
+                                              (int32_t)((long)g.gx * g.gy * g.gz)};
+        r.insert(r.end(), rec, rec + DAD_FP_REC_INTS);
+    }
+    if (needed_out) *needed_out = (int32_t)r.size();
+    std::copy(r.begin(), r.begin() + std::min<size_t>(r.size(), (size_t)capacity), out);
+    return DAD_OK;
+}
+
 int dad_debug_backward_plan(dad_model* m, int32_t batch, int32_t* out, int32_t capacity, int32_t* needed_out) {
     if (!m || batch <= 0 || capacity < 0 || (capacity > 0 && !out)) return fail(DAD_E_INVALID, "bad argument");
     if (!m->training) return fail(DAD_E_STATE, "dad_model_set_training(m, 1) has not been called");
diff --git a/dynamics_aware_diffusion_amd/csrc/host_plan.hpp b/dynamics_aware_diffusion_amd/csrc/host_plan.hpp
--- a/dynamics_aware_diffusion_amd/csrc/host_plan.hpp
+++ b/dynamics_aware_diffusion_amd/csrc/host_plan.hpp
@@ -117,8 +117,8 @@
            : (x3 && cfg_kc < 16 * sk)  ? 16 * sk
                                        : cfg_kc;
 }
-constexpr int tile_kc(int cfg, int taps, bool x3, bool bdir) {
-    return eff_kc(kTiles[cfg].KC, kTiles[cfg].BM, taps, kTiles[cfg].SK, x3, bdir, kTiles[cfg].BN);
+constexpr int tile_kc(int cfg, int taps, bool x3, bool bdir, bool narrow = false) {
+    return narrow ? 8 : eff_kc(kTiles[cfg].KC, kTiles[cfg].BM, taps, kTiles[cfg].SK, x3, bdir, kTiles[cfg].BN);
 }
 
 enum BwdSpace : int8_t { BSP_NONE, BSP_ACT, BSP_GRAD, BSP_X, BSP_DOUT, BSP_DX };
@@ -625,6 +625,11 @@
 }
 
 inline bool tile_valid(const ConvOp& op, int cfg);
+constexpr int kNarrowTile = 4;
+inline bool narrow_first(const ConvOp& op, int cfg) {
+    return cfg == kNarrowTile && op.cin0 + op.cin1 <= 8 && op.kc == 16 && !op.x3 && !op.bdir && !op.net_padded &&
+           op.stride == 1 && (op.taps == 3 || op.taps == 5 || op.taps == 7) && op.Lout <= kTiles[cfg].BN;
+}
 inline int check_tiles(const HostModel& m) {
     for (const ConvOp& op : m.plan.convs) {
         bool any = false;
@@ -802,6 +807,7 @@
     };
     if (op.kc == 8) return valid(3) ? 3 : -1;
     if (m.force_tile >= 0 && m.force_tile < kNumTiles && valid(m.force_tile)) return m.force_tile;
+    if (op.cin0 + op.cin1 <= 16 && !op.x3 && valid(kNarrowTile) && blocks(kNarrowTile) >= 224) return kNarrowTile;
     if (valid(2) && blocks(2) >= 512) return 2;
     if (valid(1) && blocks(1) >= 224) return 1;
     if (valid(0)) return 0;
@@ -876,6 +882,7 @@
 struct LaunchGeom {
     int cfg = -1;
     int kc = 0;
+    bool narrow = false;
     bool ragged = false;
     int threads = 0;
     size_t lds_bytes = 0;
@@ -901,16 +908,20 @@
     g = LaunchGeom();
     g.cfg = choose_tile(m, op, batch);
     if (g.cfg < 0) return;
-    g.kc = tile_kc(g.cfg, op.taps, op.x3, op.bdir);
+    g.narrow = narrow_first(op, g.cfg);
+    g.kc = tile_kc(g.cfg, op.taps, op.x3, op.bdir, g.narrow);
     g.split = plan_split(m, op, g.cfg, batch);
     g.fused = fused_at(m, op, g);
 }
 
 constexpr int kRegMaxTaps = 7;
-constexpr int kRegFlags = 6;
+constexpr int kRegFlags = 7;
 constexpr bool kernel_registered(int cfg, int taps, int stride, bool x3, bool bdir, bool ragged, bool res, bool padded = false,
-                                 bool windowed = false) {
+                                 bool windowed = false, bool narrow = false) {
     if (cfg < 0 || cfg >= kNumTiles) return false;
+    if (narrow)
+        return cfg == kNarrowTile && ragged && !x3 && !bdir && !padded && !windowed && stride == 1 &&
+               (taps == 3 || taps == 5 || taps == 7);
     if (windowed) {
         if (!kWinTiles[cfg] || !padded || x3 || bdir || res) return false;
         const bool odd = taps == 3 || taps == 5 || taps == 7 || taps == 1;
@@ -929,7 +940,7 @@
     return stride == 1 && (taps == 1 || taps == 2 || k357);
 }
 constexpr bool kernel_registered_f(int cfg, int taps, int stride, int f) {
-    return kernel_registered(cfg, taps, stride, f & 1, f & 2, f & 4, f & 8, f & 16, f & 32);
+    return kernel_registered(cfg, taps, stride, f & 1, f & 2, f & 4, f & 8, f & 16, f & 32, f & 64);
 }
 constexpr int count_registered() {
     int n = 0;
@@ -939,7 +950,7 @@
                 for (int f = 0; f < (1 << kRegFlags); ++f) n += kernel_registered_f(cfg, taps, stride, f);
     return n;
 }
-static_assert(count_registered() == 335, "the set of conv-GEMM kernels changed: kernel_registered");
+static_assert(count_registered() == 341, "the set of conv-GEMM kernels changed: kernel_registered");
 
 inline int plan_launch(const HostModel& m, const ConvOp& op, int batch, LaunchGeom& g) {
     choose_launch(m, op, batch, g);
@@ -951,7 +962,7 @@
                     op.name.c_str(), op.M, op.cout / 8, op.Lout);
     const TileCfg& t = kTiles[g.cfg];
     const int cin = op.cin0 + op.cin1;
-    g.ragged = (op.cin0 & 3) != 0 || (op.cin1 & 3) != 0 || op.cin0 % g.kc != 0 || cin % g.kc != 0;
+    g.ragged = g.narrow || (op.cin0 & 3) != 0 || (op.cin1 & 3) != 0 || op.cin0 % g.kc != 0 || cin % g.kc != 0;
     if (g.ragged && !(op.stride == 1 && (op.taps & 1) == 1))
         return fail(DAD_E_INVALID, "channel count %d+%d needs the general staging path, which exists "
                     "for stride-1 k-tap and 1x1 convs only", op.cin0, op.cin1);
@@ -968,7 +979,7 @@
                     op.name.c_str(), op.cin_pad, g.kc);
     g.windowed = op.Lout > t.BN;
     g.padded = op.net_padded || g.windowed;
-    if (!kernel_registered(g.cfg, op.taps, op.stride, op.x3, op.bdir, g.ragged, g.fused, g.padded, g.windowed))
+    if (!kernel_registered(g.cfg, op.taps, op.stride, op.x3, op.bdir, g.ragged, g.fused, g.padded, g.windowed, g.narrow))
         return fail(DAD_E_INVALID, "no kernel for %s (tile %d taps=%d stride=%d x3=%d bdir=%d ragged=%d res=%d padded=%d windowed=%d)",
                     op.name.c_str(), g.cfg, op.taps, op.stride, (int)op.x3, (int)op.bdir, (int)g.ragged, (int)g.fused, (int)g.padded,
                     (int)g.windowed);
diff --git a/dynamics_aware_diffusion_amd/csrc/pointwise.hpp b/dynamics_aware_diffusion_amd/csrc/pointwise.hpp
--- a/dynamics_aware_diffusion_amd/csrc/pointwise.hpp
+++ b/dynamics_aware_diffusion_amd/csrc/pointwise.hpp
@@ -79,8 +79,9 @@
 };
 
 
+constexpr int FINAL_KS = 4;
 template <int K>
-__device__ __forceinline__ void final_dots(const float* wrow0, const float* arow, int dim, int rstep, float* acc) {
+__device__ __forceinline__ void final_dots(const float* wrow0, const float* arow, int dim, int rstep, int sl, float* acc) {
     const float* wr[K];
     float a[K][4];
 #pragma unroll
@@ -88,11 +89,16 @@
         wr[k] = wrow0 + (long)k * rstep;
         a[k][0] = a[k][1] = a[k][2] = a[k][3] = 0.0f;
     }
-    for (int c = 0; c < dim; c += 4) {
+    const int dq = dim >> 2;
+    const int c0 = (((sl & 1) * (dq >> 1)) + (sl >> 1)) * 4;
+    const int w0 = (((sl & 1) * (dq >> 1)) + ((sl >> 1) ^ (sl & 1))) * 4;
+#pragma unroll 4
+    for (int i = 0; i < dq / FINAL_KS; ++i) {
+        const int c = c0 + 8 * i, cw = w0 + 8 * i;
         const float4 av = *reinterpret_cast<const float4*>(arow + c);
 #pragma unroll
         for (int k = 0; k < K; ++k) {
-            const float4 wv = *reinterpret_cast<const float4*>(wr[k] + c);
+            const float4 wv = *reinterpret_cast<const float4*>(wr[k] + cw);
             a[k][0] = fmaf(wv.x, av.x, a[k][0]); a[k][1] = fmaf(wv.y, av.y, a[k][1]);
             a[k][2] = fmaf(wv.z, av.z, a[k][2]); a[k][3] = fmaf(wv.w, av.w, a[k][3]);
         }
@@ -128,13 +134,19 @@
         const int j = ((lr / JG) * (int)gridDim.y + (int)blockIdx.y) * JG + lr % JG;
         float4 v = make_float4(0.f, 0.f, 0.f, 0.f);
         if (j < td) v = *reinterpret_cast<const float4*>(p.w + (long)j * dim + q * 4);
-        *reinterpret_cast<float4*>(wl + i * 4) = v;
+        const int qs = q < (dq >> 1) ? q : q ^ 1;
+        *reinterpret_cast<float4*>(wl + (lr * dq + qs) * 4) = v;
     }
     for (int i = threadIdx.x; i < td; i += blockDim.x) bl[i] = p.bias[i];
     __syncthreads();
 
-    const int col = threadIdx.x & (FINAL_COLS - 1);
-    const int jg = threadIdx.x / FINAL_COLS;
+    static_assert(FINAL_COLS == 32 && 256 % (FINAL_COLS * FINAL_KS) == 0, "two waves of 16 positions x 4 slices per column phase");
+    constexpr int NPH = 256 / (FINAL_COLS * FINAL_KS);
+    const int lane = threadIdx.x & 63;
+    const int wave = __builtin_amdgcn_readfirstlane(threadIdx.x >> 6);
+    const int col = (wave & 1) * 16 + (lane & 15);
+    const int sl = lane >> 4;
+    const int ph = wave >> 1;
     const long n = n0 + col;
     if (n >= N) return;
     const int b = (int)(n / p.H);
@@ -160,23 +172,33 @@
         p.x[idx] = xn;
     };
     constexpr int JB = 4;
-    const int jstep = JG * (int)gridDim.y;
-    for (int jb = (int)blockIdx.y * JG; jb < td; jb += JB * jstep) {
-        const int j0 = jb + jg;
-        const int live = min(JB, (td - 1 - jb) / jstep + 1);
-        float acc[JB], xv[JB];
-#pragma unroll
-        for (int k = 0; k < JB; ++k) xv[k] = p.x[n * td + min(j0 + k * jstep, td - 1)];
-        const float* wrow0 = wl + (long)(((jb / JG) / (int)gridDim.y) * JG + jg) * dim;
+    static_assert(JB <= FINAL_KS, "slice k finishes column k of a batch");
+    const int gy = (int)gridDim.y;
+    auto col_of = [&](int lr) { return ((lr / JG) * gy + (int)blockIdx.y) * JG + lr % JG; };
+    for (int lr0 = ph; lr0 < rows_local; lr0 += NPH * JB) {
+        int live = 0;
+#pragma unroll
+        for (int k = 0; k < JB; ++k) live += (lr0 + k * NPH < rows_local && col_of(lr0 + k * NPH) < td) ? 1 : 0;
+        if (live == 0) break;
+        const int jm = col_of(lr0 + sl * NPH);
+        const float xv = p.x[n * td + min(jm, td - 1)];
+        float acc[JB] = {0.0f, 0.0f, 0.0f, 0.0f};
+        const float* wrow0 = wl + (long)lr0 * dim;
         switch (live) {
-            case 1: final_dots<1>(wrow0, arow, dim, JG * dim, acc); break;
-            case 2: final_dots<2>(wrow0, arow, dim, JG * dim, acc); break;
-            case 3: final_dots<3>(wrow0, arow, dim, JG * dim, acc); break;
-            default: final_dots<4>(wrow0, arow, dim, JG * dim, acc); break;
-        }
-#pragma unroll
-        for (int k = 0; k < JB; ++k)
-            if (k < live && j0 + k * jstep < td) finish(j0 + k * jstep, acc[k], xv[k]);
+            case 1: final_dots<1>(wrow0, arow, dim, NPH * dim, sl, acc); break;
+            case 2: final_dots<2>(wrow0, arow, dim, NPH * dim, sl, acc); break;
+            case 3: final_dots<3>(wrow0, arow, dim, NPH * dim, sl, acc); break;
+            default: final_dots<4>(wrow0, arow, dim, NPH * dim, sl, acc); break;
+        }
+        float mine = 0.0f;
+#pragma unroll
+        for (int k = 0; k < JB; ++k) {
+            float v = acc[k];
+            v += __shfl_xor(v, 16, 64);
+            v += __shfl_xor(v, 32, 64);
+            mine = sl == k ? v : mine;
+        }
+        if (sl < live) finish(jm, mine, xv);
     }
 }
 
diff --git a/include/dad.h b/include/dad.h
--- a/include/dad.h
+++ b/include/dad.h
@@ -138,6 +138,17 @@
 int dad_debug_mish(const float* in, float* out, int64_t n, dad_stream_t stream);
 int dad_debug_kernel_table_consistent(void);
 int dad_debug_small_batch_plan(dad_model* m, int32_t batch, int32_t* launches_out, int32_t* wide_out);
+#define DAD_FP_HEADER 2
+#define DAD_FP_REC_CONV 0
+#define DAD_FP_REC_TILE 1
+#define DAD_FP_REC_KC 2
+#define DAD_FP_REC_KSLICES 3
+#define DAD_FP_REC_FUSED 4
+#define DAD_FP_REC_RAGGED 5
+#define DAD_FP_REC_NARROW 6
+#define DAD_FP_REC_BLOCKS 7
+#define DAD_FP_REC_INTS 8
+int dad_debug_forward_plan(dad_model* m, int32_t batch, int32_t* out, int32_t capacity, int32_t* needed_out);
 #define DAD_BP_WGRADS 0
 #define DAD_BP_MULTI 1
 #define DAD_BP_MAX_CHUNKS 2
```

Measured after the change: 3455 plans/s, median of 6. No clear change (+0.0%).
